# lars-uav/lars-image-processing

Hardware: AMD Instinct MI355X
Metric: Mpixels/sec NDVI+stats on 4096x4096 RGNir tiles; achieved HBM GB/s (higher is better)
Workload: dtype f32

## Files before the change

include/lars_hip.h:

```cpp
#ifndef LARS_HIP_H
#define LARS_HIP_H

#include <stddef.h>
#include <stdint.h>

#ifdef __cplusplus
extern "C" {
#endif

#define LARS_ABI_VERSION 1
#define LARS_HIST_BINS 50

typedef enum lars_status {
    LARS_OK = 0,
    LARS_ERR_INVALID = -1,
    LARS_ERR_NO_DEVICE = -2,
    LARS_ERR_HIP = -3,
    LARS_ERR_OOM = -4,
    LARS_ERR_RCCL = -5,
    LARS_ERR_UNSUPPORTED = -6
} lars_status;

#define LARS_U8  1
#define LARS_U16 2

#define LARS_NDVI  0
#define LARS_GNDVI 1
#define LARS_NDWI  2
#define LARS_MASK_NDVI  1u
#define LARS_MASK_GNDVI 2u
#define LARS_MASK_NDWI  4u
#define LARS_MASK_ALL   7u

#define LARS_F_STATS 1u
#define LARS_F_HIST  2u
#define LARS_F_SUMSQ 4u
#define LARS_F_RAW   8u

typedef struct lars_stats {
    double   sum;
    double   sumsq;
    uint64_t count;
    uint64_t above;
    uint64_t nans;
    double   min;
    double   max;
    double   threshold;
    uint32_t index_id;
    uint32_t reserved;
    uint64_t hist[LARS_HIST_BINS];
} lars_stats;

int         lars_abi_version(void);
const char *lars_last_error(void);
int         lars_device_count(int *count);
int         lars_set_device(int ordinal);
int         lars_get_device(int *ordinal);
int         lars_device_name(char *buf, size_t buflen);
int         lars_malloc(void **dptr, size_t bytes);
int         lars_free(void *dptr);
int         lars_memset(void *dptr, int value, size_t bytes, void *stream);
int         lars_memcpy_h2d(void *dst_dev, const void *src_host, size_t bytes);
int         lars_memcpy_d2h(void *dst_host, const void *src_dev, size_t bytes);
int         lars_memcpy_d2d(void *dst_dev, const void *src_dev, size_t bytes, void *stream);
int         lars_stream_create(void **stream);
int         lars_stream_destroy(void *stream);
int         lars_synchronize(void *stream);
int         lars_mem_info(size_t *free_bytes, size_t *total_bytes);
int         lars_shutdown(void);
int         lars_event_create(void **event);
int         lars_event_destroy(void *event);
int         lars_event_record(void *event, void *stream);
int         lars_event_elapsed_ms(void *start, void *stop, float *ms);
int         lars_stream_wait_event(void *stream, void *event);


int lars_d_channel_hist(const void *tiles, int64_t ntiles, int64_t npix, int channels,
                        int dtype, uint32_t *hist, void *stream);

int lars_d_wb_table(const uint32_t *hist, int64_t ntiles, int64_t npix, int dtype,
                    uint8_t *table, double *percentiles, int rgn_variant, void *stream);

size_t lars_wb_table_bytes(int dtype);

int lars_d_wb_prepare(const void *tiles, int64_t ntiles, int64_t npix, int channels, int dtype,
                      uint8_t *table, double *percentiles, int rgn_variant, void *stream);
int lars_u16_window_report(int64_t ntiles, uint32_t *flags, uint32_t *windows);

typedef struct lars_fused_args {
    const void    *tiles;
    int64_t        ntiles;
    int64_t        npix;
    int32_t        channels;
    int32_t        dtype;
    const uint8_t *wb_table;
    uint32_t       index_mask;
    uint32_t       flags;
    float         *out_index[3];
    uint8_t       *out_wb;
    uint8_t       *out_rgba[3];
    const uint8_t *cmap_lut[3];
    lars_stats    *stats;
    void          *stream;
} lars_fused_args;

int lars_d_fused(const lars_fused_args *args);
int lars_d_stats_begin(lars_stats *stats, int64_t ntiles, uint32_t index_mask, void *stream);
int lars_d_stats_end(lars_stats *stats, int64_t ntiles, uint32_t index_mask, int64_t npix, void *stream);

int lars_d_index_planes_f32(const float *red, const float *green, const float *nir,
                            int64_t n, int index_id, float *out, void *stream);

int lars_d_ndvi_f64(const void *img, int64_t npix, int channels, int dtype,
                    double *out, void *stream);

int lars_d_array_stats_f32(const float *x, int64_t n, float threshold, int want_hist,
                           lars_stats *out_dev, void *stream);
int lars_d_array_stats_f64(const double *x, int64_t n, double threshold, int want_hist,
                           lars_stats *out_dev, double *out_sumsqdev_dev, void *stream);

size_t lars_select_scratch_bytes(void);
int lars_d_median_pair_f32(const float *x, int64_t n, float *out_dev, void *scratch, void *stream);
int lars_d_median_pair_f64(const double *x, int64_t n, double *out_dev, void *scratch, void *stream);
int lars_d_median_pair_batch_f32(const float *x, int64_t n, int64_t items, int64_t stride, float *out_dev,
                                 void *scratch, void *stream);

int lars_d_quotient_select_hist(const void *tiles, int64_t ntiles, int64_t npix, int channels, int dtype,
                                const uint8_t *wb_table, uint32_t streams , int first,
                                const uint32_t bucket[4], uint64_t *hist, void *stream);
size_t lars_quotient_median_scratch_bytes(int64_t ntiles);
int lars_d_stats_medians(const lars_fused_args *a, float *out_pairs, void *scratch);
int lars_d_quotient_median_pairs(const void *tiles, int64_t ntiles, int64_t npix, int channels, int dtype,
                                 const uint8_t *wb_table, uint32_t streams ,
                                 float *out_pairs, void *scratch, void *stream);

size_t lars_joint_scratch_bytes(int64_t ntiles, int64_t npix, uint32_t index_mask);
int lars_d_stats_joint(const lars_fused_args *a, int white_balance, int rgn_variant, double *percentiles, uint32_t *hist,
                       float *out_pairs, void *scratch, size_t scratch_bytes);
int lars_joint_window_report(const void *scratch, int64_t ntiles, int64_t *windowed, int64_t *recounted);
int lars_joint_window_modes(const void *scratch, int64_t ntiles, int64_t counts[3]);

int lars_d_threshold_mask_f32(const float *x, int64_t n, float threshold, uint8_t *out_mask, void *stream);

int lars_d_colormap_f32(const float *x, int64_t n, const uint8_t *lut_rgba, uint8_t *out_rgba,
                        void *stream);
int lars_d_colormap_entry_f32(const float *x, int64_t n, uint8_t *out_entry, void *stream);

int lars_d_gray_c128(const uint8_t *img, int64_t npix, int channels, double *out_c128, void *stream);
size_t lars_phase_scratch_bytes(void);
int lars_d_phase_correlation(double *fixed_c128, double *moving_c128, int64_t h, int64_t w, int64_t *shift_dev,
                             void *scratch, void *stream);
int lars_d_shift_reflect_u8(const uint8_t *img, int64_t h, int64_t w, int channels, const int64_t *shift_dev,
                            uint8_t *out, void *stream);
int lars_d_diff_f32(const float *early, const float *late, int64_t n, float *out_diff, void *stream);
int lars_d_colormap_norm_f32(const float *x, int64_t n, float vmin, float vmax, const uint8_t *lut_rgba,
                             uint8_t *out_rgba, void *stream);

int lars_d_synth_u8(uint8_t *tiles, int64_t ntiles, int64_t first_tile, int64_t npix, int channels,
                    uint32_t seed, int profile, void *stream);

int lars_set_tuning(const char *key, int value);
int lars_get_tuning(const char *key, int *value);

#define LARS_BUILD_LAB_LAYOUT 1u
#define LARS_BUILD_IEEE_DIV 2u
#define LARS_BUILD_COUNT_MODE 4u
#define LARS_BUILD_STATS_GEOMETRY 8u
unsigned int lars_build_flags(void);

int lars_d_quot_selfcheck(uint32_t max_den, uint64_t *mismatches, uint32_t first_bad[2]);

int lars_stats_merge(const lars_stats *records, int64_t n, lars_stats *out);
int lars_d_stats_fold(const lars_stats *tile_records, int64_t ntiles, uint32_t index_mask, lars_stats *out, void *stream);


int lars_h_fix_white_balance(const void *img, int64_t h, int64_t w, int channels, int dtype,
                             int variant, uint8_t *out, double *percentiles );
int lars_h_fix_white_balance_f32(const float *img, int64_t h, int64_t w, int channels, uint8_t *out,
                                 double *percentiles );

int lars_h_calculate_index(const void *img, int64_t h, int64_t w, int channels, int dtype,
                           uint32_t index_mask, float *const out[3],
                           lars_stats *stats , int want_hist);

int lars_h_calculate_index_planes(const float *red, const float *green, const float *nir,
                                  int64_t n, int index_id, float *out);

int lars_h_ndvi_f64(const void *img, int64_t h, int64_t w, int channels, int dtype, double *out);

int lars_h_analyze_f32(const float *x, int64_t n, float threshold, int want_hist,
                       lars_stats *out, float median_pair[2]);
int lars_h_analyze_f64(const double *x, int64_t n, double threshold, int want_hist,
                       lars_stats *out, double median_pair[2], double *sumsqdev);

int lars_h_process_image(const void *img, int64_t h, int64_t w, int channels, int dtype,
                         int apply_wb, uint32_t index_mask, int want_hist,
                         uint8_t *out_wb, float *const out_index[3],
                         lars_stats *stats , float *medians ,
                         uint8_t *const out_rgba[3], const uint8_t *const cmap_lut[3]);

int lars_h_colormap_f32(const float *x, int64_t n, const uint8_t *lut_rgba, uint8_t *out_rgba);
int lars_h_threshold_mask_f32(const float *x, int64_t n, float threshold, uint8_t *out_mask);

int lars_h_resize_lanczos_u8(const uint8_t *img, int64_t h, int64_t w, int channels, int64_t new_h, int64_t new_w,
                             uint8_t *out);
int lars_h_thumbnail_u8(const uint8_t *img, int64_t h, int64_t w, int channels, int fx, int fy, const int reduce_box[4],
                        const float box[4], int64_t new_h, int64_t new_w, int vertical_first, uint8_t *out);

int lars_h_align_images(const uint8_t *fixed, const uint8_t *moving, int64_t h, int64_t w, int channels,
                        uint8_t *out_aligned, double shift[2]);
int lars_h_change_detection(const uint8_t *early, const uint8_t *late, int64_t h, int64_t w, int channels,
                            int wb_early, int wb_late, int align, int index_id,
                            float *out_early, float *out_late, float *out_diff,
                            uint8_t *out_rgba_diff, const uint8_t *lut_rgba, float vmin, float vmax,
                            uint8_t *out_aligned_late, double shift[2]);
int lars_h_colormap_norm_f32(const float *x, int64_t n, float vmin, float vmax, const uint8_t *lut_rgba,
                             uint8_t *out_rgba);

size_t lars_png_bound(int64_t h, int64_t w, int channels);
size_t lars_png_scratch_bytes(int64_t h, int64_t w, int channels);
int lars_d_encode_png_u8(const uint8_t *img, int64_t h, int64_t w, int channels, const uint8_t *palette_rgba, int palette_len,
                         uint8_t *out, size_t out_cap, int64_t *out_len_dev, void *scratch, void *stream);
int lars_h_encode_png_u8(const uint8_t *img, int64_t h, int64_t w, int channels, const uint8_t *palette_rgba, int palette_len,
                         uint8_t *out, size_t out_cap, int64_t *out_len);
int lars_h_process_image_png(const void *img, int64_t h, int64_t w, int channels, int dtype,
                             int apply_wb, uint32_t index_mask, int want_hist,
                             uint8_t *out_wb, float *const out_index[3],
                             lars_stats *stats , float *medians ,
                             const uint8_t *const cmap_lut[3], int png_mode,
                             uint8_t *const out_png[3], size_t png_cap, int64_t png_len[3]);

#define LARS_PNG_INFO_N 10
enum {
    LARS_PNG_INFO_WIDTH = 0,
    LARS_PNG_INFO_HEIGHT = 1,
    LARS_PNG_INFO_BIT_DEPTH = 2,
    LARS_PNG_INFO_COLOR_TYPE = 3,
    LARS_PNG_INFO_INTERLACE = 4,
    LARS_PNG_INFO_CHANNELS = 5,
    LARS_PNG_INFO_IDAT_BYTES = 6,
    LARS_PNG_INFO_IDAT_COUNT = 7,
    LARS_PNG_INFO_APNG = 8,
    LARS_PNG_INFO_SUPPORTED = 9
};
enum {
    LARS_PNGD_OK = 0,
    LARS_PNGD_CRC = 1,
    LARS_PNGD_ZLIB_HEADER = 2,
    LARS_PNGD_DEFLATE = 3,
    LARS_PNGD_FAR = 4,
    LARS_PNGD_SHORT = 5,
    LARS_PNGD_ADLER = 6,
    LARS_PNGD_FILTER = 7,
    LARS_PNGD_INTERNAL = 8
};
int lars_png_info(const uint8_t *file, int64_t len, int64_t info[LARS_PNG_INFO_N], int64_t *idat_table, int64_t idat_cap);
size_t lars_png_decode_scratch_bytes(int64_t h, int64_t w, int channels, int64_t idat_bytes, int64_t idat_count);
int lars_d_decode_png_u8(const uint8_t *file, const int64_t *idat_table, int64_t idat_count, int64_t idat_bytes, int64_t h,
                         int64_t w, int channels, uint8_t *out, int32_t *status_dev, void *scratch, void *stream);
int lars_h_decode_png_u8(const uint8_t *file, int64_t len, uint8_t *out, size_t out_cap);
int lars_h_thumbnail_png_u8(const uint8_t *file, int64_t len, int fx, int fy, const int reduce_box[4], const float box[4],
                            int64_t new_h, int64_t new_w, int vertical_first, uint8_t *out);

#define LARS_PNGX_PASS_N 10
enum {
    LARS_PNGX_PASS_X0 = 0,
    LARS_PNGX_PASS_Y0 = 1,
    LARS_PNGX_PASS_DX = 2,
    LARS_PNGX_PASS_DY = 3,
    LARS_PNGX_PASS_W = 4,
    LARS_PNGX_PASS_H = 5,
    LARS_PNGX_PASS_ROW_BYTES = 6,
    LARS_PNGX_PASS_OFFSET = 7,
    LARS_PNGX_PASS_BPP = 8,
    LARS_PNGX_PASS_INDEX = 9
};
int lars_png_out_format(int depth, int color_type, int *channels, int *itemsize);
int lars_png_layout(int64_t w, int64_t h, int depth, int color_type, int interlace, int64_t passes[7 * LARS_PNGX_PASS_N],
                    int64_t *npass, int64_t *need);
size_t lars_png_decode_ex_scratch_bytes(int64_t h, int64_t w, int depth, int color_type, int interlace, int64_t idat_bytes,
                                        int64_t idat_count);
int lars_d_decode_png_ex(const uint8_t *file, const int64_t *idat_table, int64_t idat_count, int64_t idat_bytes, int64_t h,
                         int64_t w, int depth, int color_type, int interlace, uint8_t *out, int32_t *status_dev, void *scratch,
                         void *stream);
int lars_h_decode_png_ex(const uint8_t *file, int64_t len, uint8_t *out, size_t out_cap);
int lars_h_thumbnail_png_ex(const uint8_t *file, int64_t len, int fx, int fy, const int reduce_box[4], const float box[4],
                            int64_t new_h, int64_t new_w, int vertical_first, uint8_t *out);

#define LARS_JPEG_INFO_N 16
#define LARS_JPEG_INFO_SAMPLING_STRIDE 2
enum {
    LARS_JPEG_INFO_WIDTH = 0,
    LARS_JPEG_INFO_HEIGHT = 1,
    LARS_JPEG_INFO_COMPONENTS = 2,
    LARS_JPEG_INFO_FRAME = 3,
    LARS_JPEG_INFO_PRECISION = 4,
    LARS_JPEG_INFO_H0 = 5,
    LARS_JPEG_INFO_V0 = 6,
    LARS_JPEG_INFO_RESTART_INTERVAL = 11,
    LARS_JPEG_INFO_ENTROPY_OFFSET = 12,
    LARS_JPEG_INFO_ENTROPY_BYTES = 13,
    LARS_JPEG_INFO_SUPPORTED = 14,
    LARS_JPEG_INFO_REASON = 15
};
enum {
    LARS_JPEG_REASON_NONE = 0,
    LARS_JPEG_REASON_PROGRESSIVE = 1,
    LARS_JPEG_REASON_FRAME = 2,
    LARS_JPEG_REASON_PRECISION = 3,
// ... 277 lines not shown
```

lars_image_processing_amd/_ffi.py:

```python
from __future__ import annotations

import contextlib
import ctypes as C
import os
import threading
from typing import NamedTuple

import numpy as np

_HERE = os.path.dirname(os.path.abspath(__file__))
LIB_PATH = os.environ.get("LARS_HIP_LIB", os.path.join(_HERE, "liblars_hip.so"))

HIST_BINS = 50
U8, U16 = 1, 2
NDVI, GNDVI, NDWI = 0, 1, 2
INDEX_IDS = {"NDVI": NDVI, "GNDVI": GNDVI, "NDWI": NDWI}
INDEX_NAMES = ("NDVI", "GNDVI", "NDWI")
F_STATS, F_HIST, F_SUMSQ, F_RAW = 1, 2, 4, 8
COMM_ID_BYTES = 128


class LarsError(RuntimeError):

    def __init__(self, code, message):
        super().__init__(f"liblars_hip error {code}: {message}")
        self.code = code


class Stats(C.Structure):
    _fields_ = [
        ("sum", C.c_double), ("sumsq", C.c_double),
        ("count", C.c_uint64), ("above", C.c_uint64), ("nans", C.c_uint64),
        ("min", C.c_double), ("max", C.c_double), ("threshold", C.c_double),
        ("index_id", C.c_uint32), ("reserved", C.c_uint32),
        ("hist", C.c_uint64 * HIST_BINS),
    ]


STATS_DTYPE = np.dtype([
    ("sum", "<f8"), ("sumsq", "<f8"), ("count", "<u8"), ("above", "<u8"), ("nans", "<u8"),
    ("min", "<f8"), ("max", "<f8"), ("threshold", "<f8"), ("index_id", "<u4"), ("reserved", "<u4"),
    ("hist", "<u8", (HIST_BINS,)),
])
assert STATS_DTYPE.itemsize == C.sizeof(Stats) == 472

REGION_DTYPE = np.dtype([("area", "<i8"), ("bbox", "<i4", (4,)), ("row_sum", "<u8"), ("col_sum", "<u8")])
assert REGION_DTYPE.itemsize == 40

RING_DTYPE = np.dtype([("label", "<i4"), ("key", "<i4"), ("start", "<i4"), ("count", "<i4"), ("area2", "<i8")])
assert RING_DTYPE.itemsize == 24


class Outlines(C.Structure):
    _fields_ = [
        ("rings", C.c_void_p), ("ring_capacity", C.c_int64), ("verts", C.c_void_p), ("vert_capacity", C.c_int64),
        ("n_rings", C.c_int64), ("n_vertices", C.c_int64), ("n_edges", C.c_int64),
    ]


class FusedArgs(C.Structure):
    _fields_ = [
        ("tiles", C.c_void_p), ("ntiles", C.c_int64), ("npix", C.c_int64),
        ("channels", C.c_int32), ("dtype", C.c_int32),
        ("wb_table", C.c_void_p), ("index_mask", C.c_uint32), ("flags", C.c_uint32),
        ("out_index", C.c_void_p * 3), ("out_wb", C.c_void_p),
        ("out_rgba", C.c_void_p * 3), ("cmap_lut", C.c_void_p * 3),
        ("stats", C.c_void_p), ("stream", C.c_void_p),
    ]


class PngInfo(NamedTuple):
    width: int
    height: int
    bit_depth: int
    color_type: int
    interlace: int
    channels: int
    idat_bytes: int
    idat_count: int
    apng: int
    supported: int

    @classmethod
    def array(cls):
        return (C.c_int64 * len(cls._fields))()


class JpegInfo(NamedTuple):
    width: int
    height: int
    components: int
    frame: int
    precision: int
    h0: int
    v0: int
    h1: int
    v1: int
    h2: int
    v2: int
    restart_interval: int
    entropy_offset: int
    entropy_bytes: int
    supported: int
    reason: int

    @classmethod
    def array(cls):
        return (C.c_int64 * len(cls._fields))()

    @property
    def sampling(self):
        return ((self.h0, self.v0), (self.h1, self.v1), (self.h2, self.v2))


class TiffInfo(NamedTuple):
    width: int
    height: int
    samples: int
    bits: int
    compression: int
    predictor: int
    planar: int
    big_endian: int
    photometric: int
    extra_samples: int
    tiled: int
    chunk_w: int
    chunk_h: int
    chunks: int
    supported: int
    reason: int

    @classmethod
    def array(cls):
        return (C.c_int64 * len(cls._fields))()


_P, _I, _I64, _U32, _SZ, _F, _D = C.c_void_p, C.c_int, C.c_int64, C.c_uint32, C.c_size_t, C.c_float, C.c_double
SIGNATURES = {
    "lars_abi_version": (_I, []),
    "lars_last_error": (C.c_char_p, []),
    "lars_device_count": (_I, [C.POINTER(_I)]),
    "lars_set_device": (_I, [_I]),
    "lars_get_device": (_I, [C.POINTER(_I)]),
    "lars_device_name": (_I, [C.c_char_p, _SZ]),
    "lars_malloc": (_I, [C.POINTER(_P), _SZ]),
    "lars_free": (_I, [_P]),
    "lars_memset": (_I, [_P, _I, _SZ, _P]),
    "lars_memcpy_h2d": (_I, [_P, _P, _SZ]),
    "lars_memcpy_d2h": (_I, [_P, _P, _SZ]),
    "lars_memcpy_d2d": (_I, [_P, _P, _SZ, _P]),
    "lars_stream_create": (_I, [C.POINTER(_P)]),
    "lars_stream_destroy": (_I, [_P]),
    "lars_synchronize": (_I, [_P]),
    "lars_shutdown": (_I, []),
    "lars_mem_info": (_I, [C.POINTER(_SZ), C.POINTER(_SZ)]),
    "lars_event_create": (_I, [C.POINTER(_P)]),
    "lars_event_destroy": (_I, [_P]),
    "lars_event_record": (_I, [_P, _P]),
    "lars_event_elapsed_ms": (_I, [_P, _P, C.POINTER(_F)]),
    "lars_stream_wait_event": (_I, [_P, _P]),
    "lars_d_channel_hist": (_I, [_P, _I64, _I64, _I, _I, _P, _P]),
    "lars_d_wb_table": (_I, [_P, _I64, _I64, _I, _P, _P, _I, _P]),
    "lars_wb_table_bytes": (_SZ, [_I]),
    "lars_d_wb_prepare": (_I, [_P, _I64, _I64, _I, _I, _P, _P, _I, _P]),
    "lars_u16_window_report": (_I, [_I64, _P, _P]),
    "lars_d_fused": (_I, [C.POINTER(FusedArgs)]),
    "lars_d_stats_begin": (_I, [_P, _I64, _U32, _P]),
    "lars_d_stats_end": (_I, [_P, _I64, _U32, _I64, _P]),
    "lars_d_index_planes_f32": (_I, [_P, _P, _P, _I64, _I, _P, _P]),
    "lars_d_ndvi_f64": (_I, [_P, _I64, _I, _I, _P, _P]),
    "lars_d_array_stats_f32": (_I, [_P, _I64, _F, _I, _P, _P]),
    "lars_d_array_stats_f64": (_I, [_P, _I64, _D, _I, _P, _P, _P]),
    "lars_select_scratch_bytes": (_SZ, []),
    "lars_d_median_pair_f32": (_I, [_P, _I64, _P, _P, _P]),
    "lars_d_median_pair_f64": (_I, [_P, _I64, _P, _P, _P]),
    "lars_d_median_pair_batch_f32": (_I, [_P, _I64, _I64, _I64, _P, _P, _P]),
    "lars_d_colormap_f32": (_I, [_P, _I64, _P, _P, _P]),
    "lars_d_colormap_entry_f32": (_I, [_P, _I64, _P, _P]),
    "lars_quotient_median_scratch_bytes": (_SZ, [_I64]),
    "lars_d_stats_medians": (_I, [C.POINTER(FusedArgs), _P, _P]),
    "lars_d_quotient_median_pairs": (_I, [_P, _I64, _I64, _I, _I, _P, _U32, _P, _P, _P]),
    "lars_joint_scratch_bytes": (_SZ, [_I64, _I64, _U32]),
    "lars_d_stats_joint": (_I, [C.POINTER(FusedArgs), _I, _I, _P, _P, _P, _P, _SZ]),
    "lars_joint_window_report": (_I, [_P, _I64, C.POINTER(_I64), C.POINTER(_I64)]),
    "lars_joint_window_modes": (_I, [_P, _I64, C.POINTER(_I64)]),
    "lars_h_tiff_lzw_decode": (_I, [_P, _I64, _P, _I64, C.POINTER(_I64)]),
    "lars_h_tiff_lzw_decode_chunks": (_I, [_P, _I64, _P, _P, _I64, _P, _I64, _P, _I]),
    "lars_d_quotient_select_hist": (_I, [_P, _I64, _I64, _I, _I, _P, _U32, _I, _P, _P, _P]),
    "lars_d_synth_u8": (_I, [_P, _I64, _I64, _I64, _I, _U32, _I, _P]),
    "lars_stats_merge": (_I, [_P, _I64, _P]),
    "lars_d_stats_fold": (_I, [_P, _I64, _U32, _P, _P]),
    "lars_build_flags": (C.c_uint, []),
    "lars_set_tuning": (_I, [C.c_char_p, _I]),
    "lars_get_tuning": (_I, [C.c_char_p, C.POINTER(_I)]),
    "lars_d_quot_selfcheck": (_I, [_U32, C.POINTER(C.c_uint64), C.POINTER(_U32 * 2)]),
    "lars_h_fix_white_balance": (_I, [_P, _I64, _I64, _I, _I, _I, _P, _P]),
    "lars_h_fix_white_balance_f32": (_I, [_P, _I64, _I64, _I, _P, _P]),
    "lars_h_calculate_index": (_I, [_P, _I64, _I64, _I, _I, _U32, C.POINTER(_P * 3), _P, _I]),
    "lars_h_calculate_index_planes": (_I, [_P, _P, _P, _I64, _I, _P]),
    "lars_h_ndvi_f64": (_I, [_P, _I64, _I64, _I, _I, _P]),
    "lars_h_analyze_f32": (_I, [_P, _I64, _F, _I, _P, _P]),
    "lars_h_analyze_f64": (_I, [_P, _I64, _D, _I, _P, _P, _P]),
    "lars_h_process_image": (_I, [_P, _I64, _I64, _I, _I, _I, _U32, _I, _P, C.POINTER(_P * 3), _P, _P,
                                  C.POINTER(_P * 3), C.POINTER(_P * 3)]),
    "lars_h_colormap_f32": (_I, [_P, _I64, _P, _P]),
    "lars_h_threshold_mask_f32": (_I, [_P, _I64, _F, _P]),
    "lars_d_threshold_mask_f32": (_I, [_P, _I64, _F, _P, _P]),
    "lars_h_colormap_norm_f32": (_I, [_P, _I64, _F, _F, _P, _P]),
    "lars_h_align_images": (_I, [_P, _P, _I64, _I64, _I, _P, _P]),
    "lars_h_change_detection": (_I, [_P, _P, _I64, _I64, _I, _I, _I, _I, _I, _P, _P, _P, _P, _P, _F, _F, _P, _P]),
    "lars_d_gray_c128": (_I, [_P, _I64, _I, _P, _P]),
    "lars_phase_scratch_bytes": (_SZ, []),
    "lars_d_phase_correlation": (_I, [_P, _P, _I64, _I64, _P, _P, _P]),
    "lars_d_shift_reflect_u8": (_I, [_P, _I64, _I64, _I, _P, _P, _P]),
    "lars_d_diff_f32": (_I, [_P, _P, _I64, _P, _P]),
    "lars_d_colormap_norm_f32": (_I, [_P, _I64, _F, _F, _P, _P, _P]),
    "lars_h_resize_lanczos_u8": (_I, [_P, _I64, _I64, _I, _I64, _I64, _P]),
    "lars_h_thumbnail_u8": (_I, [_P, _I64, _I64, _I, _I, _I, C.POINTER(_I), C.POINTER(_F), _I64, _I64, _I, _P]),
    "lars_png_bound": (_SZ, [_I64, _I64, _I]),
    "lars_png_scratch_bytes": (_SZ, [_I64, _I64, _I]),
    "lars_d_encode_png_u8": (_I, [_P, _I64, _I64, _I, _P, _I, _P, _SZ, _P, _P, _P]),
    "lars_h_encode_png_u8": (_I, [_P, _I64, _I64, _I, _P, _I, _P, _SZ, C.POINTER(_I64)]),
    "lars_h_process_image_png": (_I, [_P, _I64, _I64, _I, _I, _I, _U32, _I, _P, C.POINTER(_P * 3), _P, _P,
                                      C.POINTER(_P * 3), _I, C.POINTER(_P * 3), _SZ, _P]),
    "lars_png_info": (_I, [_P, _I64, _P, _P, _I64]),
    "lars_png_decode_scratch_bytes": (_SZ, [_I64, _I64, _I, _I64, _I64]),
    "lars_d_decode_png_u8": (_I, [_P, _P, _I64, _I64, _I64, _I64, _I, _P, _P, _P, _P]),
    "lars_h_decode_png_u8": (_I, [_P, _I64, _P, _SZ]),
    "lars_h_thumbnail_png_u8": (_I, [_P, _I64, _I, _I, C.POINTER(_I), C.POINTER(_F), _I64, _I64, _I, _P]),
    "lars_png_out_format": (_I, [_I, _I, C.POINTER(_I), C.POINTER(_I)]),
    "lars_png_layout": (_I, [_I64, _I64, _I, _I, _I, _P, C.POINTER(_I64), C.POINTER(_I64)]),
    "lars_png_decode_ex_scratch_bytes": (_SZ, [_I64, _I64, _I, _I, _I, _I64, _I64]),
    "lars_d_decode_png_ex": (_I, [_P, _P, _I64, _I64, _I64, _I64, _I, _I, _I, _P, _P, _P, _P]),
    "lars_h_decode_png_ex": (_I, [_P, _I64, _P, _SZ]),
    "lars_h_thumbnail_png_ex": (_I, [_P, _I64, _I, _I, C.POINTER(_I), C.POINTER(_F), _I64, _I64, _I, _P]),
    "lars_jpeg_info": (_I, [_P, _I64, _P]),
    "lars_jpeg_decode_scratch_bytes": (_SZ, [_P]),
    "lars_d_decode_jpeg_u8": (_I, [_P, _P, _P, _P, _P, _P, _P]),
    "lars_h_decode_jpeg_u8": (_I, [_P, _I64, _P, _SZ]),
    "lars_h_thumbnail_jpeg_u8": (_I, [_P, _I64, _I, _I, C.POINTER(_I), C.POINTER(_F), _I64, _I64, _I, _P]),
    "lars_jpeg_decode_scaled_scratch_bytes": (_SZ, [_P, _I]),
    "lars_d_decode_jpeg_scaled_u8": (_I, [_P, _P, _P, _I, _P, _P, _P, _P]),
    "lars_h_decode_jpeg_scaled_u8": (_I, [_P, _I64, _I, _P, _SZ]),
    "lars_h_thumbnail_jpeg_scaled_u8": (_I, [_P, _I64, _I, _I, _I, C.POINTER(_I), C.POINTER(_F), _I64, _I64, _I, _P]),
    "lars_tiff_info": (_I, [_P, _I64, _P, _P, _I64]),
    "lars_h_decode_tiff": (_I, [_P, _I64, _P, _SZ]),
    "lars_h_thumbnail_tiff_u8": (_I, [_P, _I64, _I, _I, C.POINTER(_I), C.POINTER(_F), _I64, _I64, _I, _P]),
    "lars_tiff_info_deflate": (_I, [_P, _I64, _P, _P, _I64]),
    "lars_h_decode_tiff_deflate": (_I, [_P, _I64, _P, _SZ]),
    "lars_h_thumbnail_tiff_deflate_u8": (_I, [_P, _I64, _I, _I, C.POINTER(_I), C.POINTER(_F), _I64, _I64, _I, _P]),
    "lars_tiff_bound": (_SZ, [_I64, _I64, _I, _I, _I64]),
    "lars_tiff_encode_scratch_bytes": (_SZ, [_I64, _I64, _I, _I, _I64]),
    "lars_d_encode_tiff": (_I, [_P, _I64, _I64, _I, _I, _I64, _I, _P, _SZ, _P, _P, _P, _P]),
    "lars_h_encode_tiff": (_I, [_P, _I64, _I64, _I, _I, _I64, _I, _P, _SZ, C.POINTER(_I64)]),
    "lars_tiff_f32_bound": (_SZ, [_I64, _I64, _I, _I64]),
    "lars_tiff_f32_encode_scratch_bytes": (_SZ, [_I64, _I64, _I, _I64]),
    "lars_d_encode_tiff_f32": (_I, [_P, _I64, _I64, _I, _I64, _I, _P, _SZ, _P, _P, _P, _P]),
    "lars_h_encode_tiff_f32": (_I, [_P, _I64, _I64, _I, _I64, _I, _P, _SZ, C.POINTER(_I64)]),
    "lars_h_process_image_tiff_f32": (_I, [_P, _I64, _I64, _I, _I, _I, _U32, _I, _P, C.POINTER(_P * 3), _P, _P,
                                           C.POINTER(_P * 3), C.POINTER(_P * 3), _I, _I64, C.POINTER(_P * 3), _SZ, _P]),
    "lars_tiff_deflate_bound": (_SZ, [_I64, _I64, _I, _I, _I64]),
    "lars_tiff_deflate_encode_scratch_bytes": (_SZ, [_I64, _I64, _I, _I, _I64]),
    "lars_d_encode_tiff_deflate": (_I, [_P, _I64, _I64, _I, _I, _I64, _I, _P, _SZ, _P, _P, _P, _P]),
    "lars_h_encode_tiff_deflate": (_I, [_P, _I64, _I64, _I, _I, _I64, _I, _P, _SZ, C.POINTER(_I64)]),
    "lars_tiff_float32_deflate_bound": (_SZ, [_I64, _I64, _I, _I64]),
    "lars_tiff_float32_deflate_encode_scratch_bytes": (_SZ, [_I64, _I64, _I, _I64]),
    "lars_d_encode_tiff_deflate_float32": (_I, [_P, _I64, _I64, _I, _I64, _I, _P, _SZ, _P, _P, _P, _P]),
    "lars_h_encode_tiff_deflate_float32": (_I, [_P, _I64, _I64, _I, _I64, _I, _P, _SZ, C.POINTER(_I64)]),
    "lars_h_process_image_tiff_float32": (_I, [_P, _I64, _I64, _I, _I, _I, _U32, _I, _P, C.POINTER(_P * 3), _P, _P,
                                                       C.POINTER(_P * 3), C.POINTER(_P * 3), _I, _I, _I64, C.POINTER(_P * 3), _SZ, _P]),
    "lars_d_valid_mask": (_I, [_P, _I64, _I, _I, _P, _I, _I, _I, _P, _P, _P]),
    "lars_d_masked_channel_hist": (_I, [_P, _I64, _I, _I, _P, _P, _P]),
    "lars_d_masked_fused": (_I, [C.POINTER(FusedArgs), _P, C.POINTER(_P * 3), _P]),
    "lars_h_valid_mask": (_I, [_P, _I64, _I64, _I, _I, _I, _I, _I, _P, C.POINTER(_I64)]),
    "lars_h_process_image_masked": (_I, [_P, _I64, _I64, _I, _I, _I, _U32, _I, _P, C.POINTER(_P * 3), _P, _P,
                                         C.POINTER(_P * 3), C.POINTER(_P * 3), _P, _I, _I, _I, C.POINTER(_I64),
                                         _I, _I, _I64, C.POINTER(_P * 3), _SZ, _P]),
    "lars_d_zone_count": (_I, [_P, _I, _P, _I64, _I64, _P, _P, _P]),
    "lars_d_zone_offsets": (_I, [_P, _I64, _P, _P, _P]),
    "lars_d_zone_scatter": (_I, [C.POINTER(_P * 3), _U32, _P, _I, _P, _I64, _I64, _P, _P, C.POINTER(_P * 3), _P]),
    "lars_d_zone_stats": (_I, [_P, _P, _P, _I64, _F, _I, _I64, _P, _P, _P]),
    "lars_h_zonal_stats_f32": (_I, [_P, _P, _I, _P, _I64, _I64, _I64, _F, _I, _P, _P, C.POINTER(_I64)]),
    "lars_h_process_image_zones": (_I, [_P, _I64, _I64, _I, _I, _I, _U32, _I, _P, C.POINTER(_P * 3), _P, _P,
                                        C.POINTER(_P * 3), C.POINTER(_P * 3), _P, _I, _I, _I, C.POINTER(_I64),
                                        _P, _I, _I64, _P, _P, C.POINTER(_I64)]),
    "lars_zone_rasterize_scratch_bytes": (_SZ, [_I64]),
    "lars_d_zone_rasterize": (_I, [_P, _I64, _P, _I64, _P, _I64, _I64, _I64, _P, _P, _P]),
    "lars_d_zone_labels_narrow": (_I, [_P, _I64, _I, _P, _P]),
    "lars_h_rasterize_zones": (_I, [_P, _I64, _P, _I64, _P, _I64, _I64, _I64, _I, _P]),
    "lars_h_zonal_stats_polygons_f32": (_I, [_P, _P, _I64, _P, _I64, _P, _I64, _P, _I64, _I64, _F, _I, _P, _P, _P, _I]),
    "lars_h_process_image_zones_polygons": (_I, [_P, _I64, _I64, _I, _I, _I, _U32, _I, _P, C.POINTER(_P * 3), _P, _P,
                                                 C.POINTER(_P * 3), C.POINTER(_P * 3), _P, _I, _I, _I, C.POINTER(_I64),
                                                 _P, _I64, _P, _I64, _P, _I64, _P, _P, _P, _I]),
    "lars_region_label_scratch_bytes": (_SZ, [_I64, _I64]),
    "lars_d_region_label": (_I, [_P, _I64, _I64, _I, _I64, _P, _P, _I64, _P, _P, _P]),
    "lars_d_region_mask_f32": (_I, [_P, _P, _P, _I64, _F, _I, _P, _P]),
    "lars_h_label_regions": (_I, [_P, _I64, _I64, _I, _I64, _I, _P, C.POINTER(_I), _P, _I64, C.POINTER(_I64)]),
    "lars_h_zonal_stats_regions_f32": (_I, [_P, _P, _I, _F, _I, _I64, _P, _I64, _I64, _F, _I, _I64, _P, _P, _P, C.POINTER(_I64), _P, _I,
                                            C.POINTER(_I)]),
    "lars_h_process_image_regions": (_I, [_P, _I64, _I64, _I, _I, _I, _U32, _I, _P, C.POINTER(_P * 3), _P, _P,
                                          C.POINTER(_P * 3), C.POINTER(_P * 3), _P, _I, _I, _I, C.POINTER(_I64),
                                          _P, _I, _I, _F, _I, _I64, _I64, _P, _P, _P, C.POINTER(_I64), _P, _I, C.POINTER(_I)]),
    "lars_region_outline_scratch_bytes": (_SZ, [_I64, _I64, _I64]),
    "lars_d_region_outline_count": (_I, [_P, _I64, _I64, _P, _P]),
    "lars_d_region_outline": (_I, [_P, _I64, _I64, _I, _I64, _I64, _P, _I64, _P, _I64, _P, _P, _P]),
    "lars_h_region_outlines": (_I, [_P, _I64, _I64, _I, _I64, _I, _P, C.POINTER(_I), _P, _I64, C.POINTER(_I64), C.POINTER(Outlines)]),
    "lars_h_zonal_stats_regions_outlines_f32": (_I, [_P, _P, _I, _F, _I, _I64, _P, _I64, _I64, _F, _I, _I64, _P, _P, _P, C.POINTER(_I64), _P, _I,
                                                     C.POINTER(_I), C.POINTER(Outlines)]),
    "lars_h_process_image_regions_outlines": (_I, [_P, _I64, _I64, _I, _I, _I, _U32, _I, _P, C.POINTER(_P * 3), _P, _P,
                                                   C.POINTER(_P * 3), C.POINTER(_P * 3), _P, _I, _I, _I, C.POINTER(_I64),
                                                   _P, _I, _I, _F, _I, _I64, _I64, _P, _P, _P, C.POINTER(_I64), _P, _I, C.POINTER(_I),
                                                   C.POINTER(Outlines)]),
    "lars_jpeg_bound": (_SZ, [_I64, _I64, _I, _I]),
    "lars_jpeg_header": (_I64, [_I64, _I64, _I, _I, _I, _P, _SZ]),
    "lars_jpeg_encode_scratch_bytes": (_SZ, [_I64, _I64, _I, _I]),
    "lars_d_encode_jpeg_u8": (_I, [_P, _I64, _I64, _I, _I, _I, _P, _SZ, _P, _P, _P]),
    "lars_h_encode_jpeg_u8": (_I, [_P, _I64, _I64, _I, _I, _I, _P, _SZ, C.POINTER(_I64)]),
    "lars_comm_available": (_I, []),
    "lars_comm_unique_id": (_I, [_P]),
# ... 158 lines not shown
```

lars_image_processing_amd/batch.py:

```python
from __future__ import annotations

import ctypes as C
import os

import numpy as np

from . import _ffi
from . import arena as _arena
from ._ffi import FusedArgs, INDEX_IDS, INDEX_NAMES, STATS_DTYPE, DeviceBuffer, DeviceSlice
from .arena import arena_placements

MAX_TILES_PER_LAUNCH = 65535


_STATS_ROUTE = os.environ.get("LARS_STATS_ROUTE", "auto")


def set_stats_route(route):
    global _STATS_ROUTE
    if route not in ("auto", "joint", "classic"):
        raise ValueError("route must be auto, joint or classic")
    _STATS_ROUTE = route


def get_stats_route():
    return _STATS_ROUTE


def index_mask(indices):
    mask = 0
    for t in indices:
        mask |= 1 << INDEX_IDS[t]
    return mask


def joint_serves(code, channels, ntiles, npix):
    return code == _ffi.U8 and channels in (3, 4) and (ntiles == 1 or npix % 4 == 0)


def plan_process(code, channels, ntiles, npix, indices, white_balance, hist, medians, sumsq, route,
                 outputs=False, wb_plane=False, reuse=False):
    if route not in ("auto", "joint", "classic"):
        raise ValueError(f"route must be auto, joint or classic, not {route!r}")
    if reuse and not outputs and route == "joint":
        raise ValueError("route='joint' derives the tables from its own counts: it cannot honour recompute_tables=False")
    one_read = route != "classic" and not reuse and joint_serves(code, channels, ntiles, npix) and bool(indices)
    if one_read and not outputs:
        return "measure" if route == "auto" and not medians and not sumsq else "one-read"
    if route == "joint" and not outputs:
        raise ValueError("route='joint' serves uint8 tiles with 3 or 4 channels (4-byte aligned) only")
    if one_read and not wb_plane and (medians or hist or select_streams(indices) in (1, 2)):
        return "one-read+planes"
    if medians and code == _ffi.U8 and channels == 3 and npix * 6 < (1 << 30) and (ntiles == 1 or npix % 4 == 0):
        return "select" if not outputs and index_mask(indices) in (1, 2, 4, 7) else "per-pixel+select"
    return "per-pixel+radix" if medians else "per-pixel"


def channels_of(indices, whole_image=False):
    if whole_image:
        return {0, 1, 2}
    need = set()
    for t in indices:
        need |= {2, 0} if t == "NDVI" else {2, 1}
    return need


def shard_range(ntiles, rank, world):
    base, rem = divmod(int(ntiles), int(world))
    start = rank * base + min(rank, rem)
    return start, start + base + (1 if rank < rem else 0)


class TileBatch:

    def __init__(self, ntiles, h, w, channels=3, dtype=np.uint8, first_tile=0):
        self.ntiles, self.h, self.w, self.channels = int(ntiles), int(h), int(w), int(channels)
        self.dtype = np.dtype(dtype)
        self.code = _ffi.dtype_code(self.dtype)
        if self.code is None:
            raise TypeError("tiles must be uint8 or uint16")
        if self.ntiles < 1 or self.ntiles > MAX_TILES_PER_LAUNCH:
            raise ValueError(f"1 <= ntiles <= {MAX_TILES_PER_LAUNCH} per batch")
        self.first_tile = int(first_tile)
        self.npix = self.h * self.w
        self.nvalues = 256 if self.code == _ffi.U8 else 65536
        self.table_bytes = int(_ffi.load().lars_wb_table_bytes(self.code))
        self.tile_bytes = self.npix * self.channels * self.dtype.itemsize
        self.tiles = DeviceBuffer(self.ntiles * self.tile_bytes)
        self.hist = None
        self.table = None
        self.percentiles = None
        self._table_channels = set()
        self._hist_channels = set()
        self._rgn_variant = 0
        self._joint_scratch = None
        self._joint_tiles = self.ntiles
        self._selq = None
        self.last_route = None

    @classmethod
    def from_host(cls, array, first_tile=0):
        arr = np.ascontiguousarray(array)
        if arr.ndim != 4 or arr.shape[3] < 3:
            raise ValueError("expected [ntiles, H, W, C>=3]")
        b = cls(arr.shape[0], arr.shape[1], arr.shape[2], arr.shape[3], arr.dtype, first_tile)
        b.tiles.upload(arr)
        return b

    @classmethod
    def synthetic(cls, ntiles, h, w, seed=1234, profile="uniform", first_tile=0, channels=3):
        b = cls(ntiles, h, w, channels, np.uint8, first_tile)
        _ffi.call("lars_d_synth_u8", C.c_void_p(b.tiles.ptr), b.ntiles, b.first_tile, b.npix, b.channels,
                  int(seed) & 0xFFFFFFFF, {"uniform": 0, "vegetation": 1}[profile], None)
        _ffi.call("lars_synchronize", None)
        return b

    def host_tiles(self, start=0, count=None):
        count = self.ntiles - start if count is None else count
        return self.tiles.download(self.dtype, (count, self.h, self.w, self.channels), start * self.tile_bytes)

    def compute_wb_tables(self, stream=None, rgn_variant=0):
        if self.table is None:
            self.table = DeviceBuffer(self.ntiles * self.table_bytes)
            self.percentiles = DeviceBuffer(self.ntiles * 3 * 2 * 8)
        if self.code == _ffi.U8:
            if self.hist is None:
                self.hist = DeviceBuffer(self.ntiles * 3 * 256 * 4)
            _ffi.call("lars_d_channel_hist", C.c_void_p(self.tiles.ptr), self.ntiles, self.npix, self.channels,
                      self.code, C.c_void_p(self.hist.ptr), stream)
            _ffi.call("lars_d_wb_table", C.c_void_p(self.hist.ptr), self.ntiles, self.npix, self.code,
                      C.c_void_p(self.table.ptr), C.c_void_p(self.percentiles.ptr), int(rgn_variant), stream)
        else:
            _ffi.call("lars_d_wb_prepare", C.c_void_p(self.tiles.ptr), self.ntiles, self.npix, self.channels,
                      self.code, C.c_void_p(self.table.ptr), C.c_void_p(self.percentiles.ptr), int(rgn_variant), stream)
        self._table_channels = {0, 1, 2}
        self._hist_channels = {0, 1, 2} if self.code == _ffi.U8 else set()
        self._rgn_variant = int(rgn_variant)
        return self

    def u16_window_report(self):
        if self.code != _ffi.U16:
            raise _ffi.LarsError(-1, "lars_u16_window_report: a uint8 batch's pre-pass does not take the value-window route")
        flags = np.zeros(self.ntiles, np.uint32)
        windows = np.zeros((self.ntiles, 3, 4), np.uint32)
        _ffi.call("lars_u16_window_report", self.ntiles, _ffi.ptr(flags), _ffi.ptr(windows))
        return flags, windows

    def _need_channels(self, partial):
        if self.table is None:
            raise RuntimeError("compute_wb_tables() first")
        if not partial and self._table_channels != {0, 1, 2}:
            missing = sorted({0, 1, 2} - self._table_channels)
            raise RuntimeError(f"white-balance tables of channel(s) {missing} are not valid: the last pass computed only the "
                               f"channels its indices read (compute_wb_tables() for all three, or partial=True)")

    def host_tables(self, partial=False):
        self._need_channels(partial)
        blob = self.table.download(np.uint8, (self.ntiles, self.table_bytes))
        return np.ascontiguousarray(blob[:, :3 * self.nvalues]).reshape(self.ntiles, 3, self.nvalues)

    def host_percentiles(self, partial=False):
        self._need_channels(partial)
        return self.percentiles.download(np.float64, (self.ntiles, 3, 2))

    def host_hist(self, partial=False):
        self._need_channels(partial)
        if self.hist is None or (not partial and self._hist_channels != {0, 1, 2}):
            missing = sorted({0, 1, 2} - self._hist_channels)
            raise RuntimeError(f"channel histograms of channel(s) {missing} are not valid: the last one-read pass was not asked for them "
                               f"(compute_wb_tables(), or run_joint(..., channel_hist=True); partial=True hands out what there is)")
        return self.hist.download(np.uint32, (self.ntiles, 3, 256))

    def make_outputs(self, indices=INDEX_NAMES, index=False, wb=False, rgba=False, ring=None, placement_trials=None, arena="auto",
                     pick="fastest"):
        outs = BatchOutputs(self, indices, index, wb, rgba, ring, allocate=False)
        nplanes = len(outs._index_ids) + len(outs._rgba_ids)
        plan = _arena.plan_arena(nplanes, outs.plane_bytes, outs.slots * self.npix * 4, arena, placement_trials, pick)
        if plan.kind != "search":
            if plan.kind == "packed":
                outs.adopt_arena(DeviceBuffer(nplanes * outs.plane_bytes))
            outs.arena_report = _arena.unsearched_report(plan)
            return outs

        def free_bytes():
            free_b, total_b = C.c_size_t(), C.c_size_t()
            _ffi.call("lars_mem_info", C.byref(free_b), C.byref(total_b))
            return free_b.value

        stats = self.new_stats()
        try:
            found = _arena.search(outs, plan, pick, alloc=DeviceBuffer, free_bytes=free_bytes,
                                  probe=lambda placement, warm_ms: self._probe_arena(outs, indices, stats, warm_ms),
                                  synchronize=lambda: _ffi.call("lars_synchronize", None))
        finally:
            stats.free()
        outs.placement_ms, outs.arena_report = _arena.report(found)
        return outs

    def _probe_arena(self, outs, indices, stats, warm_ms=_arena.ARENA_WARM_MS):
        count = min(outs.slots, self.ntiles)
        starts = list(range(0, self.ntiles, count))
        if len(starts) > 16:
            starts = [starts[int(round(i * (len(starts) - 1) / 15.0))] for i in range(16)]
        mask = index_mask(indices)
        wb_on = self.table is not None
        launches = [self.fused_args(indices, wb_on, stats, False, outs, None, st, min(count, self.ntiles - st), raw=True) for st in starts]
        while len(launches) < 4:
            launches = launches + launches
        ev = [C.c_void_p(), C.c_void_p()]
        for e in ev:
            _ffi.call("lars_event_create", C.byref(e))
        ms = C.c_float(0)

        def one_pass():
            _ffi.call("lars_event_record", ev[0], None)
            for a in launches:
                self.run_fused(a)
            _ffi.call("lars_event_record", ev[1], None)
            _ffi.call("lars_event_elapsed_ms", ev[0], ev[1], C.byref(ms))
            return float(ms.value)

        try:
            _ffi.call("lars_d_stats_begin", C.c_void_p(stats.ptr), self.ntiles, mask, None)
            warmed, passes = 0.0, 0
            while warmed < warm_ms and passes < 8:
                warmed += one_pass()
                passes += 1
            timed = one_pass()
            _ffi.call("lars_d_stats_end", C.c_void_p(stats.ptr), self.ntiles, mask, self.npix, None)
            _ffi.call("lars_synchronize", None)
        finally:
            for e in ev:
                _ffi.call("lars_event_destroy", e)
        return timed / len(launches)

    def fused_args(self, indices=INDEX_NAMES, white_balance=True, stats=None, hist=False, outputs=None,
                   stream=None, tile_start=0, tile_count=None, sumsq=False, raw=False):
        tile_count = self.ntiles - tile_start if tile_count is None else tile_count
        a = FusedArgs()
        a.tiles = self.tiles.ptr + tile_start * self.tile_bytes
        a.ntiles, a.npix, a.channels, a.dtype = tile_count, self.npix, self.channels, self.code
        if white_balance:
            if self.table is None:
                raise RuntimeError("compute_wb_tables() first")
            a.wb_table = self.table.ptr + tile_start * self.table_bytes
        a.index_mask = index_mask(indices)
        a.flags = ((_ffi.F_STATS if stats is not None else 0) | (_ffi.F_HIST if (stats is not None and hist) else 0) |
                   (_ffi.F_SUMSQ if (stats is not None and sumsq) else 0) | (_ffi.F_RAW if (stats is not None and raw) else 0))
        if stats is not None:
            a.stats = stats.ptr + tile_start * 3 * STATS_DTYPE.itemsize
        if outputs is not None:
            slot = tile_start % outputs.slots
            if slot + tile_count > outputs.slots:
                raise ValueError("tile range wraps the output ring")
            for k in range(3):
                if outputs.index[k] is not None:
                    a.out_index[k] = outputs.index[k].ptr + slot * self.npix * 4
                if outputs.rgba[k] is not None:
                    a.out_rgba[k] = outputs.rgba[k].ptr + slot * self.npix * 4
                    a.cmap_lut[k] = outputs.luts[k].ptr
            if outputs.wb is not None:
                a.out_wb = outputs.wb.ptr + slot * self.npix * self.channels
        a.stream = stream
        return a

    def new_stats(self):
        return DeviceBuffer(self.ntiles * 3 * STATS_DTYPE.itemsize)

    def fold_stats(self, stats, indices=INDEX_NAMES, out=None, stream=None):
        if out is None:
            out = DeviceBuffer(3 * STATS_DTYPE.itemsize)
            out.zero(stream)
        _ffi.call("lars_d_stats_fold", C.c_void_p(stats.ptr), self.ntiles, index_mask(indices), C.c_void_p(out.ptr), stream)
        return out

    def run_fused_chunks(self, indices, white_balance, stats, hist, outputs, stream=None, sumsq=False, launch_events=None):
        chunk = self.ntiles if outputs is None else outputs.slots
        if chunk >= self.ntiles:
            if launch_events:
                _ffi.call("lars_event_record", launch_events[0], stream)
            self.run_fused(self.fused_args(indices, white_balance, stats, hist, outputs, stream, sumsq=sumsq))
            if launch_events and len(launch_events) > 1:
                _ffi.call("lars_event_record", launch_events[1], stream)
            return 1
        mask = index_mask(indices)
        if stats is not None:
            _ffi.call("lars_d_stats_begin", C.c_void_p(stats.ptr), self.ntiles, mask, stream)
        launches = 0
        if launch_events:
            _ffi.call("lars_event_record", launch_events[0], stream)
        for start in range(0, self.ntiles, chunk):
            count = min(chunk, self.ntiles - start)
            self.run_fused(self.fused_args(indices, white_balance, stats, hist, outputs, stream, start, count, sumsq=sumsq,
                                           raw=stats is not None))
            launches += 1
            if launch_events and launches < len(launch_events):
                _ffi.call("lars_event_record", launch_events[launches], stream)
        if stats is not None:
            _ffi.call("lars_d_stats_end", C.c_void_p(stats.ptr), self.ntiles, mask, self.npix, stream)
        return launches

    def run_fused(self, args):
        _ffi.call("lars_d_fused", C.byref(args))

    def can_joint(self):
        return joint_serves(self.code, self.channels, self.ntiles, self.npix)

    def run_joint(self, indices, white_balance, stats, hist=False, sumsq=False, pairs=None, stream=None, rgn_variant=0,
                  tile_count=None, channel_hist=False):
        mask = index_mask(indices)
        need = int(_ffi.load().lars_joint_scratch_bytes(self.ntiles, self.npix, mask))
        if self._joint_scratch is None or self._joint_scratch.nbytes < need:
            if self._joint_scratch is not None:
                _ffi.call("lars_synchronize", stream)
                self._joint_scratch.free()
            self._joint_scratch = DeviceBuffer(need)
        if white_balance:
            if self.table is None:
                self.table = DeviceBuffer(self.ntiles * self.table_bytes)
                self.percentiles = DeviceBuffer(self.ntiles * 3 * 2 * 8)
                self.table.zero(stream)
                self.percentiles.zero(stream)
            if channel_hist and self.hist is None:
                self.hist = DeviceBuffer(self.ntiles * 3 * 256 * 4)
                self.hist.zero(stream)
                self._hist_channels = set()
            if tile_count is None or int(tile_count) == self.ntiles:
                keep = self._table_channels if int(rgn_variant) == self._rgn_variant else set()
                self._table_channels = keep | channels_of(indices)
                self._rgn_variant = int(rgn_variant)
                if channel_hist:
                    self._hist_channels = self._hist_channels | channels_of(indices)
            else:
                self._table_channels = set()
                self._hist_channels = set()
        a = FusedArgs()
        a.tiles = self.tiles.ptr
        a.ntiles, a.npix, a.channels, a.dtype = (self.ntiles if tile_count is None else int(tile_count)), self.npix, self.channels, self.code
        a.wb_table = self.table.ptr if white_balance else None
        a.index_mask = mask
        a.flags = _ffi.F_STATS | (_ffi.F_HIST if hist else 0) | (_ffi.F_SUMSQ if sumsq else 0)
        a.stats = stats.ptr
        a.stream = stream
        self._joint_tiles = int(a.ntiles)
        _ffi.call("lars_d_stats_joint", C.byref(a), 1 if white_balance else 0, int(rgn_variant),
                  C.c_void_p(self.percentiles.ptr) if white_balance else None,
                  C.c_void_p(self.hist.ptr) if white_balance and channel_hist else None,
                  C.c_void_p(pairs.ptr) if pairs is not None else None, C.c_void_p(self._joint_scratch.ptr), self._joint_scratch.nbytes)

    def joint_window_report(self):
        w, r = C.c_int64(0), C.c_int64(0)
        if self._joint_scratch is None:
            return 0, 0
        _ffi.call("lars_joint_window_report", C.c_void_p(self._joint_scratch.ptr), self._joint_tiles, C.byref(w), C.byref(r))
        return int(w.value), int(r.value)

    def joint_window_modes(self):
        if self._joint_scratch is None:
            return 0, 0, 0
        counts = (C.c_int64 * 3)()
        _ffi.call("lars_joint_window_modes", C.c_void_p(self._joint_scratch.ptr), self._joint_tiles, counts)
        return int(counts[0]), int(counts[1]), int(counts[2])

    def check_joint(self, stream=None):
        _ffi.call("lars_synchronize", stream)
        if self._joint_scratch is not None and int(self._joint_scratch.download(np.uint32, (1,))[0]):
            raise RuntimeError("lars_d_stats_joint: a workgroup's hand-over list overflowed (a chunk of more than 2^24 pixels?)")

    def pick_stats_route(self, indices, white_balance=True, sample=256, min_pixels=1 << 29):
        key = (tuple(sorted(INDEX_IDS[t] for t in indices)), bool(white_balance))
        cache = self.__dict__.setdefault("_route_cache", {})
        if key in cache:
            return cache[key]
        sample = min(int(sample), self.ntiles)
        if sample * self.npix < int(min_pixels) or self.channels != 3:
            cache[key] = "joint"
            return "joint"
        saved = (self.table, self.percentiles, self.hist, set(self._table_channels), self._rgn_variant, set(self._hist_channels))
        self.table = self.percentiles = self.hist = None
        self._table_channels = set()
        self._hist_channels = set()
        ev = [C.c_void_p() for _ in range(3)]
        for e in ev:
            _ffi.call("lars_event_create", C.byref(e))
        stats = self.new_stats()
        ms = {}
        try:
            for _ in range(2):
                _ffi.call("lars_event_record", ev[0], None)
                self.run_joint(indices, white_balance, stats, tile_count=sample)
                _ffi.call("lars_event_record", ev[1], None)
                if white_balance:
                    if self.hist is None:
                        self.hist = DeviceBuffer(self.ntiles * 3 * 256 * 4)
                    _ffi.call("lars_d_channel_hist", C.c_void_p(self.tiles.ptr), sample, self.npix, self.channels, self.code,
                              C.c_void_p(self.hist.ptr), None)
                    _ffi.call("lars_d_wb_table", C.c_void_p(self.hist.ptr), sample, self.npix, self.code, C.c_void_p(self.table.ptr),
                              C.c_void_p(self.percentiles.ptr), 0, None)
                self.run_fused(self.fused_args(indices, white_balance, stats, False, None, None, 0, sample))
                _ffi.call("lars_event_record", ev[2], None)
                t = C.c_float(0)
                _ffi.call("lars_event_elapsed_ms", ev[0], ev[1], C.byref(t)); ms["joint"] = t.value
                _ffi.call("lars_event_elapsed_ms", ev[1], ev[2], C.byref(t)); ms["classic"] = t.value
            self.check_joint()
        finally:
            _ffi.call("lars_synchronize", None)
            for e in ev:
                _ffi.call("lars_event_destroy", e)
            stats.free()
            for buf in (self.table, self.percentiles, self.hist):
                if buf is not None:
                    buf.free()
            self.table, self.percentiles, self.hist, self._table_channels, self._rgn_variant, self._hist_channels = saved
        cache[key] = "joint" if ms["joint"] <= ms["classic"] else "classic"
        self._route_ms = dict(ms)
        return cache[key]

    def process(self, indices=INDEX_NAMES, white_balance=True, hist=False, outputs=None, stream=None,
                recompute_tables=True, medians=False, sumsq=False, route=None, rgn_variant=None, channel_hist=False):
        route = _STATS_ROUTE if route is None else route
        variant = 0 if rgn_variant is None else int(rgn_variant)
        wb_plane = outputs is not None and outputs.wb is not None
        reuse = (white_balance and not recompute_tables and self.table is not None
                 and channels_of(indices, wb_plane) <= self._table_channels and (rgn_variant is None or variant == self._rgn_variant))

        def plan(r):
            return plan_process(self.code, self.channels, self.ntiles, self.npix, indices, white_balance, hist, medians, sumsq, r,
                                outputs is not None, wb_plane, reuse)

        taken = plan(route)
        if taken == "measure":
            taken = plan(self.pick_stats_route(indices, white_balance))
        self.last_route = taken
        if taken in ("one-read", "one-read+planes"):
            return self._run_one_read(indices, white_balance, hist, sumsq, medians, outputs, stream, variant, channel_hist)
        if white_balance and not reuse:
            self.compute_wb_tables(stream, rgn_variant=variant)
        stats = self.new_stats()
        stats.zero(stream)
        run = {"select": self._run_select, "per-pixel+select": self._run_fused_select, "per-pixel": self._run_fused,
               "per-pixel+radix": self._run_fused_radix}[taken]
        return run(indices, white_balance, stats, hist, sumsq, outputs, stream)

    def _records(self, stats):
        rec = stats.download(STATS_DTYPE, (self.ntiles, 3))
        stats.free()
        return rec

    def _run_one_read(self, indices, white_balance, hist, sumsq, medians, outputs, stream, variant, channel_hist):
        stats = self.new_stats()
        stats.zero(stream)
        pairs = DeviceBuffer(self.ntiles * 4 * 4) if medians else None
        self.run_joint(indices, white_balance, stats, hist, sumsq, pairs, stream, rgn_variant=variant, channel_hist=channel_hist)
        if outputs is not None:
            self.run_fused_chunks(indices, white_balance, None, False, outputs, stream)
        self.check_joint(stream)
        rec = self._records(stats)
        if not medians:
            return rec
        med = self._medians_from_pairs(pairs.download(np.float32, (self.ntiles, 2, 2)), indices)
        pairs.free()
        return rec, med

    def _run_select(self, indices, white_balance, stats, hist, sumsq, outputs, stream):
        args = self.fused_args(indices, white_balance, stats, hist, None, stream, sumsq=sumsq)
        med = self._per_tile_select(indices, stream, lambda pairs, scratch: _ffi.call("lars_d_stats_medians", C.byref(args), pairs, scratch))
        return self._records(stats), med

    def _run_fused_select(self, indices, white_balance, stats, hist, sumsq, outputs, stream):
        self.run_fused_chunks(indices, white_balance, stats, hist, outputs, stream, sumsq)
        med = self.tile_medians(indices, white_balance, stream)
        return self._records(stats), med

    def _run_fused(self, indices, white_balance, stats, hist, sumsq, outputs, stream):
        self.run_fused_chunks(indices, white_balance, stats, hist, outputs, stream, sumsq)
        _ffi.call("lars_synchronize", stream)
        return self._records(stats)

    def _run_fused_radix(self, indices, white_balance, stats, hist, sumsq, outputs, stream):
        own_outputs = None
        if outputs is None or any(outputs.index[INDEX_IDS[t]] is None for t in indices):
            own_outputs = outputs = self.make_outputs(indices=indices, index=True, ring=min(self.ntiles, 16), arena="plain")
        pairs = DeviceBuffer(self.ntiles * 3 * 2 * 4)
        pairs.zero(stream)
        sel = DeviceBuffer(outputs.slots * int(_ffi.load().lars_select_scratch_bytes()))
        for start in range(0, self.ntiles, outputs.slots):
            count = min(outputs.slots, self.ntiles - start)
            self.run_fused(self.fused_args(indices, white_balance, stats, hist, outputs, stream, start, count, sumsq=sumsq))
            for t in indices:
                k = INDEX_IDS[t]
                _ffi.call("lars_d_median_pair_batch_f32", C.c_void_p(outputs.index[k].ptr), self.npix, count, self.npix,
                          C.c_void_p(pairs.ptr + (k * self.ntiles + start) * 8), C.c_void_p(sel.ptr), stream)
        _ffi.call("lars_synchronize", stream)
        rec = self._records(stats)
        med = pair_medians(pairs.download(np.float32, (3, self.ntiles, 2)), indices, per_index=True)
        pairs.free()
        sel.free()
        if own_outputs is not None:
            own_outputs.free()
        return rec, med

    def free(self):
        for b in (self.tiles, self.hist, self.table, self.percentiles, self._joint_scratch, self._selq):
            if b is not None:
                b.free()

    def tile_medians(self, indices=INDEX_NAMES, white_balance=True, stream=None):
        if white_balance and (self.table is None or not channels_of(indices) <= self._table_channels):
            raise RuntimeError("compute_wb_tables() first")
        return self._per_tile_select(indices, stream, lambda pairs, scratch: _ffi.call(
            "lars_d_quotient_median_pairs", C.c_void_p(self.tiles.ptr), self.ntiles, self.npix, self.channels, self.code,
            C.c_void_p(self.table.ptr) if white_balance else None, select_streams(indices), pairs, scratch, stream))

    def _per_tile_select(self, indices, stream, launch):
        pairs = DeviceBuffer(self.ntiles * 4 * 4)
        scratch = DeviceBuffer(int(_ffi.load().lars_quotient_median_scratch_bytes(self.ntiles)))
        launch(C.c_void_p(pairs.ptr), C.c_void_p(scratch.ptr))
        _ffi.call("lars_synchronize", stream)
        med = self._medians_from_pairs(pairs.download(np.float32, (self.ntiles, 2, 2)), indices)
        pairs.free()
        scratch.free()
        return med

    def _medians_from_pairs(self, pairs, indices):
        med = pair_medians(pairs, indices)
        if any(np.isnan(med[:, INDEX_IDS[t]]).any() for t in indices):
            raise RuntimeError("exact median select did not settle (values outside the uint8 quotient domain?)")
        return med

    def select_histogram(self, first, buckets, white_balance=True, stream=None, streams=3):
        if self.code != _ffi.U8 or self.channels != 3:
            raise TypeError("exact batch medians need uint8 tiles with 3 channels")
        if white_balance and self.table is None:
            raise RuntimeError("compute_wb_tables() first")
        if self._selq is None:
            self._selq = DeviceBuffer(2 * 2 * SELECT_BINS * 8)
        self._selq.zero(stream)
        b = np.ascontiguousarray(np.asarray(buckets, dtype=np.int64) & 0xFFFFFFFF, dtype=np.uint32).reshape(4)
        _ffi.call("lars_d_quotient_select_hist", C.c_void_p(self.tiles.ptr), self.ntiles, self.npix, self.channels, self.code,
                  C.c_void_p(self.table.ptr) if white_balance else None, int(streams), int(first), _ffi.ptr(b),
                  C.c_void_p(self._selq.ptr), stream)
        _ffi.call("lars_synchronize", stream)
        return self._selq.download(np.uint64, (2, 2, SELECT_BINS))

    def global_medians(self, indices=INDEX_NAMES, white_balance=True, comm=None, recompute_tables=False):
        if white_balance and (recompute_tables or self.table is None or not channels_of(indices) <= self._table_channels):
            self.compute_wb_tables()
        n_local = self.ntiles * self.npix
        streams = select_streams(indices)
        values = select_order_statistics(lambda first, buckets: self.select_histogram(first, buckets, white_balance, None, streams),
                                         n_local, comm, streams)
        return medians_from_pairs(values, indices)


class BatchOutputs:

    def __init__(self, batch, indices, index, wb, rgba, ring=None, allocate=True):
        from .api import colormap_lut, _colormap_for
        self.slots = batch.ntiles if not ring else min(int(ring), batch.ntiles)
        self.index, self.rgba, self.luts = [None] * 3, [None] * 3, [None] * 3
        self.batch = batch
        self.plane_bytes = (self.slots * batch.npix * 4 + 255) & ~255
        self._index_ids = sorted(INDEX_IDS[t] for t in indices) if index else []
        self._rgba_ids = sorted(INDEX_IDS[t] for t in indices) if rgba else []
        self.arena = None
        self.arena2 = None
        self.arena_report = None
        if allocate and (self._index_ids or self._rgba_ids):
            self.adopt_arena(DeviceBuffer((len(self._index_ids) + len(self._rgba_ids)) * self.plane_bytes))
        for t in indices:
            k = INDEX_IDS[t]
            if rgba:
                self.luts[k] = DeviceBuffer(1024)
                self.luts[k].upload(colormap_lut(_colormap_for(t)))
        self.wb = DeviceBuffer(self.slots * batch.npix * batch.channels) if wb else None

    def adopt(self, buffers, placement):
        placement = tuple((int(i), int(o)) for i, o in placement)
        assert len(placement) == len(self._index_ids) + len(self._rgba_ids)
        used = list(dict.fromkeys(i for i, _ in placement))
        assert len(used) <= 2
        for i in used:
            inside = sorted(o for a, o in placement if a == i)
            assert all(o % 256 == 0 and o + self.plane_bytes <= buffers[i].nbytes for o in inside)
            assert all(b - a >= self.plane_bytes for a, b in zip(inside, inside[1:])), "planes overlap"
        self.arena = buffers[used[0]] if used else None
        self.arena2 = buffers[used[1]] if len(used) > 1 else None
        self.plane_offsets = tuple(o for _, o in placement)
        slices = [DeviceSlice(buffers[i], o, self.plane_bytes) for i, o in placement]
        for j, k in enumerate(self._index_ids):
            self.index[k] = slices[j]
        for j, k in enumerate(self._rgba_ids):
            self.rgba[k] = slices[len(self._index_ids) + j]

    def adopt_arena(self, arena, offsets=None):
        if offsets is None:
            offsets = _arena.packed(len(self._index_ids) + len(self._rgba_ids), self.plane_bytes)
        self.adopt([arena], [(0, o) for o in offsets])

    def adopt_two_arenas(self, arena, offsets, arena2, offsets2):
        self.adopt([arena, arena2], [(0, o) for o in offsets] + [(1, o) for o in offsets2])

    def forget_planes(self):
        self.index, self.rgba, self.arena, self.arena2 = [None] * 3, [None] * 3, None, None

    def host_index(self, index_type, slot=0, count=1):
        k = INDEX_IDS[index_type]
        b = self.batch
        return self.index[k].download(np.float32, (count, b.h, b.w), slot * b.npix * 4)

    def host_rgba(self, index_type, slot=0, count=1):
        k = INDEX_IDS[index_type]
        b = self.batch
        return self.rgba[k].download(np.uint8, (count, b.h, b.w, 4), slot * b.npix * 4)

    def host_wb(self, slot=0, count=1):
        b = self.batch
        return self.wb.download(np.uint8, (count, b.h, b.w, b.channels), slot * b.npix * b.channels)

    def free(self):
        for b in self.index + self.rgba + self.luts + [self.wb, self.arena, self.arena2]:
            if b is not None:
                b.free()
        self.forget_planes()


def merge_records(records):
    rec = np.ascontiguousarray(records, dtype=STATS_DTYPE).reshape(-1)
    out = np.zeros(1, dtype=STATS_DTYPE)
    _ffi.call("lars_stats_merge", _ffi.ptr(rec), rec.size, _ffi.ptr(out))
    return out[0]


def summarize(record):
    count = int(record["count"])
    mean = float(record["sum"]) / count
    sumsq = float(record["sumsq"])
    have_sq = sumsq != 0.0 or (float(record["min"]) == 0.0 and float(record["max"]) == 0.0)
    var = max(sumsq / count - mean * mean, 0.0)
    return {
        "count": count,
        "mean": mean,
        "std": var ** 0.5 if have_sq else None,
        "min": float(record["min"]),
        "max": float(record["max"]),
        "coverage": int(record["above"]) / count * 100.0,
        "hist": np.array(record["hist"], dtype=np.int64),
    }


def local_fold(tile_records, indices=INDEX_NAMES):
    out = np.zeros(3, dtype=STATS_DTYPE)
    for t in indices:
        k = INDEX_IDS[t]
        out[k] = merge_records(tile_records[:, k])
    return out
# ... 166 lines not shown
```

lars_image_processing_amd/csrc/common.h:

```cpp
#pragma once
#include <hip/hip_runtime.h>
#include <stdint.h>
#include <stdio.h>
#include <string>

#include "host_common.h"

namespace lars {


#define LARS_HIP_TRY(expr)                                                          \
    do {                                                                            \
        hipError_t _e = (expr);                                                     \
        if (_e != hipSuccess)                                                       \
            return ::lars::fail(_e == hipErrorOutOfMemory ? LARS_ERR_OOM : LARS_ERR_HIP, \
                                "%s failed: %s (%s:%d)", #expr, hipGetErrorString(_e), \
                                __FILE__, __LINE__);                                \
    } while (0)

struct ThreadCtx {
    int device = -1;
    hipStream_t stream = nullptr;
    void *ws = nullptr;
    size_t ws_bytes = 0;
    void *scratch = nullptr;
    size_t scratch_bytes = 0;
    void *outline = nullptr;
    size_t outline_bytes = 0;
    int64_t u16_win_tiles = 0;
};

int ensure_ctx(ThreadCtx **out);
int ws_reserve(ThreadCtx *c, size_t bytes);
int scratch_reserve(ThreadCtx *c, size_t bytes);
int outline_reserve(ThreadCtx *c, size_t bytes);

struct Carver {
    char *base;
    size_t off = 0;
    explicit Carver(void *b) : base(static_cast<char *>(b)) {}
    template <typename T>
    T *take(size_t count)
    {
        off = (off + 255) & ~(size_t)255;
        T *p = base ? reinterpret_cast<T *>(base + off) : nullptr;
        off += count * sizeof(T);
        return p;
    }
    size_t bytes() const { return (off + 255) & ~(size_t)255; }
};

template <typename Plan>
int ws_plan(ThreadCtx *c, Plan &&plan)
{
    Carver size(nullptr);
    plan(size);
    LARS_TRY(ws_reserve(c, size.bytes() + 256));
    Carver cv(c->ws);
    plan(cv);
    return LARS_OK;
}
inline hipStream_t pick_stream(ThreadCtx *c, void *stream) {
    return stream ? reinterpret_cast<hipStream_t>(stream) : c->stream;
}

#define LARS_FX_SCALE 4294967296.0
#define LARS_FX_INV (1.0 / 4294967296.0)

struct StatsAccView {
    unsigned long long sum_fx;
    unsigned long long sumsq_fx;
    unsigned long long count;
    unsigned long long above;
    unsigned long long nans;
    unsigned long long min_key;
    unsigned long long max_key;
    double threshold;
    unsigned int index_id;
    unsigned int reserved;
    unsigned long long hist[LARS_HIST_BINS];
};
static_assert(sizeof(StatsAccView) == sizeof(lars_stats), "accumulator view must alias lars_stats");

__host__ __device__ inline unsigned int f32_key(float x) {
    unsigned int b = __builtin_bit_cast(unsigned int, x);
    return (b & 0x80000000u) ? ~b : (b | 0x80000000u);
}
__host__ __device__ inline float key_f32(unsigned int k) {
    unsigned int b = (k & 0x80000000u) ? (k & 0x7FFFFFFFu) : ~k;
    return __builtin_bit_cast(float, b);
}
__host__ __device__ inline unsigned long long f64_key(double x) {
    unsigned long long b = __builtin_bit_cast(unsigned long long, x);
    return (b >> 63) ? ~b : (b | 0x8000000000000000ull);
}
__host__ __device__ inline double key_f64(unsigned long long k) {
    unsigned long long b = (k >> 63) ? (k & 0x7FFFFFFFFFFFFFFFull) : ~k;
    return __builtin_bit_cast(double, b);
}

__host__ __device__ inline double hist_edge_f64(int i) {
    return i >= LARS_HIST_BINS ? 1.0 : (double)i * (2.0 / 50.0) + (-1.0);
}

#define LARS_U16_THR_OFFSET 196608
#define LARS_U16_PAR_OFFSET (196608 + 3 * 260 * 4)
#define LARS_U16_BLOB_BYTES (196608 + 4096)

int launch_check(const char *what);
void align_release();

struct Tuning {
    int fused_impl = 0;
    int hist_impl = 2;
    int nt_stores = 0;
    int blocks_per_tile = 0;
    int load_policy = 0;
    int selq_window = 1;
    int selq_list_wgs = 0;
    int last_fused_kernel = 0;
    int u16_hist_impl = 5;
    int out_stride_planes = 0;
    int joint_depth = 6;
    int joint_win_depth = 15;
    int jpeg_subseq_bits = 512;
    int jpeg_last_rounds = 0;
    int tiff_strip_bytes = 65536;
    int deflate_matching = 0;
    int joint_window = 1;
    int zone_split_pixels = 131072;
};
Tuning &tuning();
inline bool stream_loads_nt(bool kernel_default_nt)
{
    const int k = tuning().load_policy;
    return k == 0 ? kernel_default_nt : k == 2;
}

struct FusedParams;
#ifndef LARS_V2_STATS_THREADS
#define LARS_V2_STATS_THREADS 1024
#endif
#ifndef LARS_V2_STATS_WAVES
#define LARS_V2_STATS_WAVES 8
#endif
int fused_v2_threads(bool any_out);
void fused_v2_launch(unsigned mask, bool wb, int stats, bool nt, dim3 grid, hipStream_t s, const FusedParams &P);
void chan_hist_v2_launch(const uint8_t *tiles, long long npix, unsigned int *hist, dim3 grid, hipStream_t s, int channels = 3);
int selq_pass_launch(const uint8_t *tiles, const uint8_t *wb_table, long long ntiles, long long npix, int first,
                     const unsigned int bucket[4], unsigned long long *hist, hipStream_t s, unsigned streams);
size_t selq_tile_scratch_bytes(long long ntiles);
int selq_tile_medians_launch(const uint8_t *tiles, const uint8_t *wb_table, long long ntiles, long long npix, float *out_pairs,
                             void *scratch, hipStream_t s, bool first_pass_done, unsigned streams, bool windowed = false);
int selq_tile_prepare(void *scratch, long long ntiles, long long npix, hipStream_t s, unsigned int streams);
unsigned int *selq_tile_hist32(void *scratch, long long ntiles);
void fused_v2_sel_launch(unsigned mask, bool wb, int stats, dim3 grid, hipStream_t s, const FusedParams &P);
int blocks_per_tile(long long work_items, long long ntiles, int threads = 256, long long target_total = 8192);
void stats_init_launch(lars_stats *stats, long long nrec, unsigned int mask, hipStream_t s);
void stats_finalize_launch(lars_stats *stats, long long nrec, unsigned int mask, long long npix, hipStream_t s);
int quot_check_launch(unsigned int max_den, unsigned long long *mismatches_dev, unsigned int *first_bad_dev, hipStream_t s);

}
```

lars_image_processing_amd/csrc/device_common.h:

```cpp
#pragma once
#include "common.h"
#include "stream_load.h"

namespace lars {

struct FusedParams {
    const void *tiles;
    long long npix;
    int channels;
    const uint8_t *wb_table;
    float *out_index[3];
    uint8_t *out_wb;
    uint8_t *out_rgba[3];
    const uint8_t *cmap_lut[3];
    lars_stats *stats;
    unsigned int mask;
    unsigned int flags;
    unsigned int *sel_hist;
    const unsigned int *sel_win;
    unsigned int *sel_win_hist;
    unsigned int *sel_below;
#ifdef LARS_LAB_LAYOUT
    long long out_tile_stride;
#endif
};

struct Acc {
    float mn, mx;
    double sum, sumsq;
    unsigned int above;
};
__device__ inline void acc_init(Acc &a) { a.mn = __builtin_inff(); a.mx = -__builtin_inff(); a.sum = 0; a.sumsq = 0; a.above = 0; }

__device__ inline float norm_diff(float a, float b)
{
    const float s = a + b;
    const float d = a - b;
#ifdef LARS_IEEE_DIV
    return d / (s == 0.0f ? 1.0f : s);
#else
    const float den = fmaxf(s, 1.0f);
    const float r = __builtin_amdgcn_rcpf(den);
    const float q0 = d * r;
    const float e = __builtin_fmaf(-q0, den, d);
    return __builtin_fmaf(e, r, q0);
#endif
}

#define LARS_HIST_CELLS 65
template <typename T>
struct HistCell {
    T edge;
    long long base;
};
template <>
struct HistCell<float> {
    float edge;
    int base;
};
template <typename T>
__device__ inline void hist_cells_init(HistCell<T> *cells, int tid)
{
    if (tid < LARS_HIST_CELLS) {
        const T lo = (T)tid / (T)32 - (T)1, hi = (T)(tid + 1) / (T)32 - (T)1;
        int below = 0;
        T inside = (T)__builtin_inf();
        for (int i = 0; i < LARS_HIST_BINS; ++i) {
            const T e = (T)hist_edge_f64(i);
            if (e < lo) ++below;
            else if (e < hi) inside = e;
        }
        cells[tid].edge = inside;
        cells[tid].base = below - 1;
    }
}
template <typename T>
__device__ inline int hist_bin_cell(T x, const HistCell<T> *cells)
{
    const int c = (int)__builtin_fma(x, (T)32, (T)32);
    const HistCell<T> e = cells[c];
    return (int)e.base + (x >= e.edge ? 1 : 0);
}
__device__ inline int hist_bin_f32(float x, const HistCell<float> *cells)
{
    const int c = (int)__builtin_fmaf(x, 32.0f, 32.0f);
    const HistCell<float> e = cells[c];
    return e.base + (x >= e.edge ? 1 : 0);
}

__device__ inline unsigned int cmap_index(float x)
{
    const float s = (x + 1.0f) * 128.0f;
    int i = (int)s;
    i = i < 0 ? 0 : (i > 255 ? 255 : i);
    return (unsigned)i;
}


__device__ inline unsigned int wb_level(int v, double p_lo, double p_hi, int rgn_variant)
{
    double x = (double)v;
    if (rgn_variant) x = fmin(fmax(x, p_lo), p_hi);
    double y = (x - p_lo) / (p_hi - p_lo) * 255.0;
    if (y != y) return 0u;
    y = y < 0.0 ? 0.0 : (y > 255.0 ? 255.0 : y);
    return rgn_variant ? (unsigned int)(int)y : (unsigned int)(int)(float)y;
}

__device__ inline void u16_fill_blob(uint8_t *blob, int c, double p_lo, double p_hi, int rgn_variant,
                                     unsigned int *s_thr, int tid)
{
    for (int k = tid; k < 260; k += 256) s_thr[k] = 65536u;
    __syncthreads();
    uint8_t *out = blob + (long long)c * 65536;
    unsigned int prev = tid == 0 ? 0u : wb_level(tid * 256 - 1, p_lo, p_hi, rgn_variant);
    for (int j = 0; j < 256; ++j) {
        const int v = tid * 256 + j;
        const unsigned int o = wb_level(v, p_lo, p_hi, rgn_variant);
        out[v] = (uint8_t)o;
        for (unsigned int k = prev + 1; k <= o; ++k) s_thr[k] = (unsigned)v;
        prev = o > prev ? o : prev;
    }
    __syncthreads();
    unsigned int *thr = reinterpret_cast<unsigned int *>(blob + LARS_U16_THR_OFFSET) + c * 260;
    for (int k = tid; k < 260; k += 256) thr[k] = k == 0 ? 0u : (k >= 256 ? 65536u : s_thr[k]);
    if (tid == 0) {
        double *par = reinterpret_cast<double *>(blob + LARS_U16_PAR_OFFSET) + c * 2;
        const double span = p_hi - p_lo;
        par[0] = p_lo;
        par[1] = span > 0.0 ? 255.0 / span : 1e300;
    }
}

}
```

lars_image_processing_amd/csrc/fused.hip:

```cpp
#include <string.h>

#include "common.h"
#include "device_common.h"
#include "fused_device.h"
#include "wg_device.h"

namespace lars {

__global__ __launch_bounds__(256) void k_chan_hist_u8c3(const uint8_t *__restrict__ tiles,
                                                        long long npix, unsigned int *__restrict__ hist)
{
    __shared__ unsigned int s_h[4][3 * 256];
    const int tid = threadIdx.x;
    const int wave = tid >> 6;
    for (int i = tid; i < 4 * 768; i += 256) (&s_h[0][0])[i] = 0;
    __syncthreads();

    const long long tile = blockIdx.y;
    const uint8_t *base = tiles + tile * npix * 3;
    const long long nquads = npix >> 2;
    unsigned int *h = s_h[wave];
    for (long long q = (long long)blockIdx.x * 256 + tid; q < nquads; q += (long long)gridDim.x * 256) {
        const unsigned int *p = reinterpret_cast<const unsigned int *>(base + q * 12);
        unsigned int w0 = p[0], w1 = p[1], w2 = p[2];
        atomicAdd(&h[0 * 256 + (w0 & 0xFF)], 1u);
        atomicAdd(&h[1 * 256 + ((w0 >> 8) & 0xFF)], 1u);
        atomicAdd(&h[2 * 256 + ((w0 >> 16) & 0xFF)], 1u);
        atomicAdd(&h[0 * 256 + (w0 >> 24)], 1u);
        atomicAdd(&h[1 * 256 + (w1 & 0xFF)], 1u);
        atomicAdd(&h[2 * 256 + ((w1 >> 8) & 0xFF)], 1u);
        atomicAdd(&h[0 * 256 + ((w1 >> 16) & 0xFF)], 1u);
        atomicAdd(&h[1 * 256 + (w1 >> 24)], 1u);
        atomicAdd(&h[2 * 256 + (w2 & 0xFF)], 1u);
        atomicAdd(&h[0 * 256 + ((w2 >> 8) & 0xFF)], 1u);
        atomicAdd(&h[1 * 256 + ((w2 >> 16) & 0xFF)], 1u);
        atomicAdd(&h[2 * 256 + (w2 >> 24)], 1u);
    }
    if (blockIdx.x == 0 && tid < (int)(npix & 3)) {
        const uint8_t *p = base + (nquads * 4 + tid) * 3;
        atomicAdd(&h[p[0]], 1u);
        atomicAdd(&h[256 + p[1]], 1u);
        atomicAdd(&h[512 + p[2]], 1u);
    }
    __syncthreads();
    unsigned int *gh = hist + tile * 768;
    for (int i = tid; i < 768; i += 256) {
        unsigned int v = s_h[0][i] + s_h[1][i] + s_h[2][i] + s_h[3][i];
        if (v) atomicAdd(&gh[i], v);
    }
}

template <typename PIX, int NVAL>
__global__ __launch_bounds__(256) void k_chan_hist_generic(const PIX *__restrict__ tiles, long long npix,
                                                           int channels, unsigned int *__restrict__ hist)
{
    const long long tile = blockIdx.y;
    const PIX *base = tiles + tile * npix * channels;
    unsigned int *gh = hist + tile * 3 * (long long)NVAL;
    if (NVAL == 256) {
        __shared__ unsigned int s_h[3 * 256];
        for (int i = threadIdx.x; i < 768; i += 256) s_h[i] = 0;
        __syncthreads();
        for (long long i = (long long)blockIdx.x * 256 + threadIdx.x; i < npix; i += (long long)gridDim.x * 256) {
            const PIX *p = base + i * channels;
            atomicAdd(&s_h[(unsigned)p[0]], 1u);
            atomicAdd(&s_h[256 + (unsigned)p[1]], 1u);
            atomicAdd(&s_h[512 + (unsigned)p[2]], 1u);
        }
        __syncthreads();
        for (int i = threadIdx.x; i < 768; i += 256)
            if (s_h[i]) atomicAdd(&gh[i], s_h[i]);
    } else {
        for (long long i = (long long)blockIdx.x * 256 + threadIdx.x; i < npix; i += (long long)gridDim.x * 256) {
            const PIX *p = base + i * channels;
            atomicAdd(&gh[(unsigned)p[0]], 1u);
            atomicAdd(&gh[NVAL + (unsigned)p[1]], 1u);
            atomicAdd(&gh[2 * NVAL + (unsigned)p[2]], 1u);
        }
    }
}

template <int NVAL>
__global__ __launch_bounds__(256) void k_wb_table(const unsigned int *__restrict__ hist, long long npix,
                                                  uint8_t *__restrict__ table, double *__restrict__ pcts,
                                                  int rgn_variant)
{
    constexpr int PER = NVAL / 256;
    __shared__ unsigned long long s_scan[4];
    __shared__ double s_val[4];
    __shared__ double s_p[2];
    __shared__ unsigned int s_thr[NVAL == 256 ? 4 : 260];

    const int tid = threadIdx.x;
    const long long slot = (long long)blockIdx.y * 3 + blockIdx.x;
    const unsigned int *h = hist + slot * NVAL;

    unsigned long long local = 0;
    for (int j = 0; j < PER; ++j) local += h[tid * PER + j];
    const unsigned long long before = wg_exscan<256>(local, s_scan);

    const double nm1 = (double)(npix - 1);
    double tq[2];
    long long rank[4];
    for (int k = 0; k < 2; ++k) {
        const double q = (k == 0 ? 2.0 : 98.0) / 100.0;
        const double vi = nm1 * q;
        const double fl = floor(vi);
        long long lo = (long long)fl;
        long long hi = lo + 1;
        if (hi > npix - 1) hi = npix - 1;
        rank[2 * k] = lo;
        rank[2 * k + 1] = hi;
        tq[k] = vi - fl;
    }
    unsigned long long cum = before;
    for (int j = 0; j < PER; ++j) {
        const unsigned long long c = h[tid * PER + j];
        if (c) {
            for (int r = 0; r < 4; ++r)
                if ((unsigned long long)rank[r] >= cum && (unsigned long long)rank[r] < cum + c)
                    s_val[r] = (double)(tid * PER + j);
        }
        cum += c;
    }
    __syncthreads();
    if (tid < 2) {
        const double a = s_val[2 * tid], b = s_val[2 * tid + 1], t = tq[tid];
        const double d = b - a;
        double r = a + d * t;
        if (t >= 0.5) r = b - d * (1.0 - t);
        s_p[tid] = r;
        if (pcts) pcts[slot * 2 + tid] = r;
    }
    __syncthreads();
    const double p_lo = s_p[0], p_hi = s_p[1];
    if (NVAL == 256) {
        uint8_t *out = table + slot * 256;
        out[tid] = (uint8_t)wb_level(tid, p_lo, p_hi, rgn_variant);
    } else {
        u16_fill_blob(table + (long long)blockIdx.y * LARS_U16_BLOB_BYTES, (int)blockIdx.x, p_lo, p_hi, rgn_variant, s_thr, tid);
    }
}

__global__ void k_stats_init(lars_stats *stats, long long nrec, unsigned int mask)
{
    const long long i = (long long)blockIdx.x * blockDim.x + threadIdx.x;
    if (i >= nrec) return;
    const int k = (int)(i % 3);
    if (!((mask >> k) & 1u)) return;
    StatsAccView *a = reinterpret_cast<StatsAccView *>(stats + i);
    a->sum_fx = 0; a->sumsq_fx = 0; a->count = 0; a->above = 0; a->nans = 0;
    a->min_key = ~0ull; a->max_key = 0ull;
    a->threshold = (k == LARS_NDWI) ? 0.0 : (double)0.2f;
    a->index_id = (unsigned)k; a->reserved = 0;
    for (int b = 0; b < LARS_HIST_BINS; ++b) a->hist[b] = 0;
}

__global__ void k_stats_finalize(lars_stats *stats, long long nrec, unsigned int mask, long long npix)
{
    const long long i = (long long)blockIdx.x * blockDim.x + threadIdx.x;
    if (i >= nrec) return;
    const int k = (int)(i % 3);
    if (!((mask >> k) & 1u)) return;
    StatsAccView *a = reinterpret_cast<StatsAccView *>(stats + i);
    const long long s = (long long)a->sum_fx, s2 = (long long)a->sumsq_fx;
    const unsigned long long mnk = a->min_key, mxk = a->max_key;
    lars_stats *o = stats + i;
    o->sum = (double)s * LARS_FX_INV;
    o->sumsq = (double)s2 * LARS_FX_INV;
    o->count = (uint64_t)npix;
    o->min = key_f64(mnk);
    o->max = key_f64(mxk);
}

__global__ __launch_bounds__(256) void k_stats_fold(const lars_stats *__restrict__ rec, long long ntiles, unsigned int mask,
                                                    lars_stats *__restrict__ out)
{
    const int k = blockIdx.x;
    if (!((mask >> k) & 1u)) return;
    __shared__ double s_sum[256], s_sq[256];
    __shared__ double s_mn[4], s_mx[4];
    __shared__ unsigned long long s_cnt[4][3];
    const int tid = threadIdx.x;
    double sum = 0.0, sq = 0.0;
    double mn = __builtin_inf(), mx = -__builtin_inf();
    unsigned long long cnt = 0, above = 0, nans = 0;
    __shared__ unsigned long long s_hist[LARS_HIST_BINS];
    if (tid < LARS_HIST_BINS) s_hist[tid] = 0ull;
    __syncthreads();
    for (long long t = tid; t < ntiles; t += 256) {
        const unsigned long long *h = reinterpret_cast<const unsigned long long *>(rec[t * 3 + k].hist);
        unsigned long long v[LARS_HIST_BINS];
#pragma unroll
        for (int b = 0; b < LARS_HIST_BINS; ++b) v[b] = h[b];
#pragma unroll
        for (int b = 0; b < LARS_HIST_BINS; ++b)
            if (v[b]) atomicAdd(&s_hist[b], v[b]);
    }
    for (long long base = 0; base < ntiles; base += 256) {
        const long long t = base + tid;
        if (t < ntiles) {
            const lars_stats *r = rec + t * 3 + k;
            s_sum[tid] = r->sum; s_sq[tid] = r->sumsq;
            cnt += r->count; above += r->above; nans += r->nans;
            mn = fmin(mn, r->min); mx = fmax(mx, r->max);
        }
        __syncthreads();
        const int n = (int)(ntiles - base < 256 ? ntiles - base : 256);
        if (tid == 0) {
            int i = 0;
            if (base == 0) { sum = s_sum[0]; sq = s_sq[0]; i = 1; }
            for (; i < n && (i & 7); ++i) { sum += s_sum[i]; sq += s_sq[i]; }
            for (; i + 8 <= n; i += 8) {
                double a[8], b[8];
#pragma unroll
                for (int j = 0; j < 8; ++j) { a[j] = s_sum[i + j]; b[j] = s_sq[i + j]; }
#pragma unroll
                for (int j = 0; j < 8; ++j) { sum += a[j]; sq += b[j]; }
            }
            for (; i < n; ++i) { sum += s_sum[i]; sq += s_sq[i]; }
        }
        __syncthreads();
    }
    for (int off = 32; off >= 1; off >>= 1) {
        cnt += __shfl_xor(cnt, off); above += __shfl_xor(above, off); nans += __shfl_xor(nans, off);
        mn = fmin(mn, __shfl_xor(mn, off)); mx = fmax(mx, __shfl_xor(mx, off));
    }
    if ((tid & 63) == 0) {
        const int w = tid >> 6;
        s_cnt[w][0] = cnt; s_cnt[w][1] = above; s_cnt[w][2] = nans; s_mn[w] = mn; s_mx[w] = mx;
    }
    __syncthreads();
    lars_stats *o = out + k;
    if (tid == 0) {
        o->sum = sum; o->sumsq = sq;
        o->count = s_cnt[0][0] + s_cnt[1][0] + s_cnt[2][0] + s_cnt[3][0];
        o->above = s_cnt[0][1] + s_cnt[1][1] + s_cnt[2][1] + s_cnt[3][1];
        o->nans = s_cnt[0][2] + s_cnt[1][2] + s_cnt[2][2] + s_cnt[3][2];
        o->min = fmin(fmin(s_mn[0], s_mn[1]), fmin(s_mn[2], s_mn[3]));
        o->max = fmax(fmax(s_mx[0], s_mx[1]), fmax(s_mx[2], s_mx[3]));
        o->threshold = rec[k].threshold; o->index_id = rec[k].index_id; o->reserved = rec[k].reserved;
    }
    if (tid < LARS_HIST_BINS) o->hist[tid] = s_hist[tid];
}

__device__ inline void acc_flush(Acc a, StatsAccView *rec, double (*s_red)[4], int tid)
{
    for (int off = 32; off >= 1; off >>= 1) {
        a.mn = fminf(a.mn, __shfl_xor(a.mn, off));
        a.mx = fmaxf(a.mx, __shfl_xor(a.mx, off));
        a.sum += __shfl_xor(a.sum, off);
        a.sumsq += __shfl_xor(a.sumsq, off);
        a.above += __shfl_xor(a.above, off);
    }
    const int wave = tid >> 6, lane = tid & 63;
    __syncthreads();
    if (lane == 0) {
        s_red[0][wave] = a.sum;
        s_red[1][wave] = a.sumsq;
        s_red[2][wave] = (double)a.above;
        s_red[3][wave] = __builtin_bit_cast(double, ((unsigned long long)f32_key(a.mx) << 32) | f32_key(a.mn));
    }
    __syncthreads();
    if (tid == 0) {
        double sum = 0, sumsq = 0, above = 0;
        unsigned int mnk = 0xFFFFFFFFu, mxk = 0;
        for (int w = 0; w < 4; ++w) {
            sum += s_red[0][w];
            sumsq += s_red[1][w];
            above += s_red[2][w];
            const unsigned long long kk = __builtin_bit_cast(unsigned long long, s_red[3][w]);
            const unsigned int kmn = (unsigned int)kk, kmx = (unsigned int)(kk >> 32);
            mnk = kmn < mnk ? kmn : mnk;
            mxk = kmx > mxk ? kmx : mxk;
        }
        atomicAdd(&rec->sum_fx, (unsigned long long)__double2ll_rn(sum * LARS_FX_SCALE));
        atomicAdd(&rec->sumsq_fx, (unsigned long long)__double2ll_rn(sumsq * LARS_FX_SCALE));
        atomicAdd(&rec->above, (unsigned long long)above);
        atomicMin(&rec->min_key, f64_key((double)key_f32(mnk)));
        atomicMax(&rec->max_key, f64_key((double)key_f32(mxk)));
    }
}


template <typename PIX, unsigned MASK, bool WB, int STATS, int CH = 3, int POLICY = LOAD_PLAIN>
__global__ __launch_bounds__(256)
__attribute__((amdgpu_waves_per_eu(1, (sizeof(PIX) == 1 && CH == 3 && MASK != 0u && STATS <= 1) ? 3 : 8))) void k_fused_u8c3(FusedParams P)
{
    constexpr bool U16 = sizeof(PIX) == 2;
    static_assert(CH == 3 || (CH == 4 && !U16), "4-channel fast path: uint8 tiles");
    __shared__ uint8_t s_lut[U16 ? 16 : 3 * 256];
    __shared__ unsigned int s_thr[U16 ? 3 * 260 : 4];
    __shared__ double s_par[U16 ? 6 : 1];
    constexpr int HIST_COPIES = 16;
    __shared__ unsigned int s_hist_all[HIST_COPIES * 3 * LARS_HIST_BINS];
    __shared__ HistCell<float> s_edges[LARS_HIST_CELLS];
    __shared__ double s_red[4][4];

    const int tid = threadIdx.x;
    unsigned int *const s_hist = s_hist_all + (tid & (HIST_COPIES - 1));
    const unsigned int bx = blockIdx.x, gx = gridDim.x;
    const long long tile = blockIdx.y;
    const long long npix = P.npix;
    const PIX *base = static_cast<const PIX *>(P.tiles) + tile * npix * CH;

    if (WB) {
        if (U16) {
            const uint8_t *blob = P.wb_table + tile * LARS_U16_BLOB_BYTES;
            const unsigned int *thr = reinterpret_cast<const unsigned int *>(blob + LARS_U16_THR_OFFSET);
            const double *par = reinterpret_cast<const double *>(blob + LARS_U16_PAR_OFFSET);
            for (int i = tid; i < 3 * 260; i += 256) s_thr[i] = thr[i];
            if (tid < 6) s_par[tid] = par[tid];
        } else {
            const uint8_t *t = P.wb_table + tile * 768;
            for (int i = tid; i < 768; i += 256) s_lut[i] = t[i];
        }
    }
    if (STATS >= 2) {
        for (int i = tid; i < HIST_COPIES * 3 * LARS_HIST_BINS; i += 256) s_hist_all[i] = 0;
        hist_cells_init<float>(s_edges, tid);
    }
    if (WB || STATS >= 2) __syncthreads();

    auto wb_map = [&](unsigned int v, int c) -> unsigned int {
        if (!U16) return s_lut[c * 256 + v];
        const double y = ((double)v - s_par[2 * c]) * s_par[2 * c + 1];
        int g = (int)y;
        g = g < 0 ? 0 : (g > 255 ? 255 : g);
        const unsigned int *t = s_thr + c * 260;
        g += (v >= t[g + 1] ? 1 : 0) - (v < t[g] ? 1 : 0);
        return (unsigned int)g;
    };

    Acc acc[3];
    acc_init(acc[0]); acc_init(acc[1]); acc_init(acc[2]);

#ifdef LARS_LAB_LAYOUT
    const long long ots = P.out_tile_stride;
#else
    const long long ots = npix;
#endif
    float *const oi0 = P.out_index[0] ? P.out_index[0] + tile * ots : nullptr;
    float *const oi1 = P.out_index[1] ? P.out_index[1] + tile * ots : nullptr;
    float *const oi2 = P.out_index[2] ? P.out_index[2] + tile * ots : nullptr;
    uint8_t *const owb = P.out_wb ? P.out_wb + tile * npix * CH : nullptr;
    uint8_t *const oc0 = P.out_rgba[0] ? P.out_rgba[0] + tile * npix * 4 : nullptr;
    uint8_t *const oc1 = P.out_rgba[1] ? P.out_rgba[1] + tile * npix * 4 : nullptr;
    uint8_t *const oc2 = P.out_rgba[2] ? P.out_rgba[2] + tile * npix * 4 : nullptr;
    const unsigned int *lut0 = reinterpret_cast<const unsigned int *>(P.cmap_lut[0]);
    const unsigned int *lut1 = reinterpret_cast<const unsigned int *>(P.cmap_lut[1]);
    const unsigned int *lut2 = reinterpret_cast<const unsigned int *>(P.cmap_lut[2]);

    const long long nquads = npix >> 2;
    const bool nt_st = (P.flags & 0x20000000u) != 0;
    __amdgpu_buffer_rsrc_t rsrc16;
    if (U16) rsrc16 = __builtin_amdgcn_make_buffer_rsrc(const_cast<PIX *>(base), 0, (int)(nquads * 24), 0x00020000);
    constexpr int NW = U16 ? 6 : 3;

    auto load_quad = [&](long long q, unsigned int (&w)[NW]) {
        if (U16) {
            const unsigned int off = (unsigned int)q * 24u;
            const fu32x4 a4 = stream_load_b128<POLICY>(rsrc16, off, 0);
            const fu32x2 a2 = stream_load_b64<POLICY>(rsrc16, off + 16u, 0);
            w[0] = a4.x; w[1] = a4.y; w[2] = a4.z; w[NW - 3] = a4.w; w[NW - 2] = a2.x; w[NW - 1] = a2.y;
        } else if (CH == 4) {
            const sl_u32x3 a = rgba_quad_to_rgb(
                stream_load_ptr<POLICY>(reinterpret_cast<const sl_u32x4 *>(reinterpret_cast<const uint8_t *>(base) + q * 16)));
            w[0] = a.x; w[1] = a.y; w[2] = a.z;
        } else {
            const unsigned int *p = reinterpret_cast<const unsigned int *>(reinterpret_cast<const uint8_t *>(base) + q * 12);
            w[0] = stream_load_ptr<POLICY>(p); w[1] = stream_load_ptr<POLICY>(p + 1); w[2] = stream_load_ptr<POLICY>(p + 2);
        }
    };
    auto do_quad = [&](long long q, const unsigned int (&w)[NW]) {
        unsigned int b[12];
        if (U16) {
#pragma unroll
            for (int i = 0; i < 6; ++i) { b[2 * i] = w[i % NW] & 0xFFFFu; b[2 * i + 1] = w[i % NW] >> 16; }
        } else {
            const unsigned int w0 = w[0], w1 = w[1], w2 = w[2];
            const unsigned int t[12] = {w0 & 0xFF, (w0 >> 8) & 0xFF, (w0 >> 16) & 0xFF, w0 >> 24,
                                        w1 & 0xFF, (w1 >> 8) & 0xFF, (w1 >> 16) & 0xFF, w1 >> 24,
                                        w2 & 0xFF, (w2 >> 8) & 0xFF, (w2 >> 16) & 0xFF, w2 >> 24};
#pragma unroll
            for (int i = 0; i < 12; ++i) b[i] = t[i];
        }
        if (WB) {
            const bool need_r = (MASK & 1u) || owb, need_g = (MASK & 6u) || owb;
#pragma unroll
            for (int i = 0; i < 12; ++i)
                if (i % 3 == 2 || (i % 3 == 0 && need_r) || (i % 3 == 1 && need_g)) b[i] = wb_map(b[i], i % 3);
            if (owb && CH == 4) {
                *reinterpret_cast<uint4 *>(owb + q * 16) = make_uint4(b[0] | (b[1] << 8) | (b[2] << 16), b[3] | (b[4] << 8) | (b[5] << 16),
                                                                      b[6] | (b[7] << 8) | (b[8] << 16), b[9] | (b[10] << 8) | (b[11] << 16));
            } else if (owb) {
                unsigned int *o = reinterpret_cast<unsigned int *>(owb + q * 12);
                o[0] = b[0] | (b[1] << 8) | (b[2] << 16) | (b[3] << 24);
                o[1] = b[4] | (b[5] << 8) | (b[6] << 16) | (b[7] << 24);
                o[2] = b[8] | (b[9] << 8) | (b[10] << 16) | (b[11] << 24);
            }
        }
        float v0[4], v1[4], v2[4];
#pragma unroll
        for (int px = 0; px < 4; ++px) {
            v0[px] = v1[px] = v2[px] = 0.0f;
            pixel_math<MASK, STATS, false, !U16, HIST_COPIES>((float)b[3 * px], (float)b[3 * px + 1], (float)b[3 * px + 2], 0u,
                                                            v0[px], v1[px], v2[px], acc, s_hist, s_edges);
        }
        if ((MASK & 1u) && oi0) store_plane4(oi0 + q * 4, v0, nt_st);
        if ((MASK & 2u) && oi1) store_plane4(oi1 + q * 4, v1, nt_st);
        if ((MASK & 4u) && oi2) store_plane4(oi2 + q * 4, v2, nt_st);
        if ((MASK & 1u) && oc0)
            *reinterpret_cast<uint4 *>(oc0 + q * 16) = make_uint4(lut0[cmap_index(v0[0])], lut0[cmap_index(v0[1])],
                                                                  lut0[cmap_index(v0[2])], lut0[cmap_index(v0[3])]);
        if ((MASK & 2u) && oc1)
            *reinterpret_cast<uint4 *>(oc1 + q * 16) = make_uint4(lut1[cmap_index(v1[0])], lut1[cmap_index(v1[1])],
                                                                  lut1[cmap_index(v1[2])], lut1[cmap_index(v1[3])]);
        if ((MASK & 4u) && oc2)
            *reinterpret_cast<uint4 *>(oc2 + q * 16) = make_uint4(lut2[cmap_index(v2[0])], lut2[cmap_index(v2[1])],
                                                                  lut2[cmap_index(v2[2])], lut2[cmap_index(v2[3])]);
    };

    constexpr int RUN = (!U16 && CH == 3 && MASK == 7u && STATS == 1) ? 16 : (U16 && MASK == 1u && STATS <= 1) ? 8 : 4;
    const long long nsteps = (nquads + 64 * RUN - 1) / (64 * RUN);
    const long long wstride = (long long)gx * 4;
    const unsigned int lane = (unsigned int)tid & 63u;
    for (long long st = (long long)bx * 4 + (tid >> 6); st < nsteps; st += wstride) {
        const long long q0 = st * (64 * RUN) + lane;
        unsigned int w[RUN][NW];
        if (st * (64 * RUN) + 64 * RUN <= nquads) {
#pragma unroll
            for (int j = 0; j < RUN; ++j) load_quad(q0 + 64 * j, w[j]);
            __builtin_amdgcn_sched_barrier(0);
#pragma unroll
            for (int j = 0; j < RUN; ++j) {
                do_quad(q0 + 64 * j, w[j]);
                __builtin_amdgcn_sched_barrier(0);
            }
        } else {
            for (int j = 0; j < RUN; ++j) {
                const long long q = q0 + 64 * j;
                if (q < nquads) { load_quad(q, w[0]); do_quad(q, w[0]); }
            }
        }
    }
    if (bx == 0 && tid < (int)(npix & 3)) {
        const long long i = nquads * 4 + tid;
        unsigned int r = base[i * CH], g = base[i * CH + 1], n = base[i * CH + 2];
        if (WB) { r = wb_map(r, 0); g = wb_map(g, 1); n = wb_map(n, 2); }
        if (WB && owb) {
            owb[i * CH] = (uint8_t)r; owb[i * CH + 1] = (uint8_t)g; owb[i * CH + 2] = (uint8_t)n;
            if (CH == 4) owb[i * CH + 3] = 0;
        }
        float a = 0, bq = 0, c = 0;
        pixel_math<MASK, STATS, false, !U16, HIST_COPIES>((float)r, (float)g, (float)n, 0u, a, bq, c, acc, s_hist, s_edges);
        if ((MASK & 1u) && oi0) oi0[i] = a;
        if ((MASK & 2u) && oi1) oi1[i] = bq;
        if ((MASK & 4u) && oi2) oi2[i] = c;
        if ((MASK & 1u) && oc0) reinterpret_cast<unsigned int *>(oc0)[i] = lut0[cmap_index(a)];
        if ((MASK & 2u) && oc1) reinterpret_cast<unsigned int *>(oc1)[i] = lut1[cmap_index(bq)];
        if ((MASK & 4u) && oc2) reinterpret_cast<unsigned int *>(oc2)[i] = lut2[cmap_index(c)];
    }

    if (STATS >= 1) {
        StatsAccView *rec = reinterpret_cast<StatsAccView *>(P.stats + tile * 3);
#pragma unroll
        for (int k = 0; k < 3; ++k)
            if ((MASK & (1u << k)) && (P.mask & (1u << k))) acc_flush(acc[k], rec + k, s_red, tid);
        if (STATS >= 2) {
            __syncthreads();
            for (int i = tid; i < 3 * LARS_HIST_BINS; i += 256) {
                const int k = i / LARS_HIST_BINS;
                unsigned int v = 0;
#pragma unroll
                for (int c = 0; c < HIST_COPIES; ++c) v += s_hist_all[i * HIST_COPIES + ((c + i) & (HIST_COPIES - 1))];
                if ((MASK & (1u << k)) && (P.mask & (1u << k)) && v) atomicAdd(&rec[k].hist[i - k * LARS_HIST_BINS], (unsigned long long)v);
            }
        }
    }
}

template <typename PIX, int NVAL>
__global__ __launch_bounds__(256) void k_fused_generic(FusedParams P)
{
    __shared__ unsigned int s_hist[3 * LARS_HIST_BINS];
    __shared__ HistCell<float> s_edges[LARS_HIST_CELLS];
    __shared__ double s_red[4][4];

    const int tid = threadIdx.x;
    const long long tile = blockIdx.y;
    const long long npix = P.npix;
    const int C = P.channels;
    const unsigned mask = P.mask;
    const bool stats = P.flags & (LARS_F_STATS | LARS_F_HIST | LARS_F_SUMSQ);
    const bool hist = P.flags & (LARS_F_HIST | LARS_F_SUMSQ);
    const bool sumsq = P.flags & LARS_F_SUMSQ;
    const PIX *base = static_cast<const PIX *>(P.tiles) + tile * npix * C;
    const uint8_t *tab = P.wb_table ? P.wb_table + tile * (NVAL == 256 ? 768ll : (long long)LARS_U16_BLOB_BYTES) : nullptr;

    for (int i = tid; i < 3 * LARS_HIST_BINS; i += 256) s_hist[i] = 0;
    hist_cells_init<float>(s_edges, tid);
    __syncthreads();

    Acc acc[3];
    acc_init(acc[0]); acc_init(acc[1]); acc_init(acc[2]);
    float *const oi0 = P.out_index[0] ? P.out_index[0] + tile * npix : nullptr;
    float *const oi1 = P.out_index[1] ? P.out_index[1] + tile * npix : nullptr;
    float *const oi2 = P.out_index[2] ? P.out_index[2] + tile * npix : nullptr;
    uint8_t *const owb = P.out_wb ? P.out_wb + tile * npix * C : nullptr;
    unsigned int *const oc0 = P.out_rgba[0] ? reinterpret_cast<unsigned int *>(P.out_rgba[0]) + tile * npix : nullptr;
    unsigned int *const oc1 = P.out_rgba[1] ? reinterpret_cast<unsigned int *>(P.out_rgba[1]) + tile * npix : nullptr;
    unsigned int *const oc2 = P.out_rgba[2] ? reinterpret_cast<unsigned int *>(P.out_rgba[2]) + tile * npix : nullptr;
    const unsigned int *lut0 = reinterpret_cast<const unsigned int *>(P.cmap_lut[0]);
    const unsigned int *lut1 = reinterpret_cast<const unsigned int *>(P.cmap_lut[1]);
    const unsigned int *lut2 = reinterpret_cast<const unsigned int *>(P.cmap_lut[2]);

    for (long long i = (long long)blockIdx.x * 256 + tid; i < npix; i += (long long)gridDim.x * 256) {
        const PIX *p = base + i * C;
        unsigned int r = p[0], g = p[1], n = p[2];
        if (tab) {
            r = tab[r]; g = tab[NVAL + g]; n = tab[2 * NVAL + n];
            if (owb) {
                uint8_t *o = owb + i * C;
                o[0] = (uint8_t)r; o[1] = (uint8_t)g; o[2] = (uint8_t)n;
                for (int c = 3; c < C; ++c) o[c] = 0;
            }
        }
        float a = 0, b = 0, c = 0;
        if (stats) {
            if (sumsq) pixel_math<7u, 3, true>((float)r, (float)g, (float)n, mask, a, b, c, acc, s_hist, s_edges);
            else if (hist) pixel_math<7u, 2, true>((float)r, (float)g, (float)n, mask, a, b, c, acc, s_hist, s_edges);
            else pixel_math<7u, 1, true>((float)r, (float)g, (float)n, mask, a, b, c, acc, s_hist, s_edges);
        } else {
            pixel_math<7u, 0, true>((float)r, (float)g, (float)n, mask, a, b, c, acc, s_hist, s_edges);
        }
        if ((mask & 1u) && oi0) oi0[i] = a;
        if ((mask & 2u) && oi1) oi1[i] = b;
        if ((mask & 4u) && oi2) oi2[i] = c;
        if ((mask & 1u) && oc0) oc0[i] = lut0[cmap_index(a)];
        if ((mask & 2u) && oc1) oc1[i] = lut1[cmap_index(b)];
        if ((mask & 4u) && oc2) oc2[i] = lut2[cmap_index(c)];
    }
    if (stats) {
        StatsAccView *rec = reinterpret_cast<StatsAccView *>(P.stats + tile * 3);
        for (int k = 0; k < 3; ++k)
            if (mask & (1u << k)) acc_flush(acc[k], rec + k, s_red, tid);
        if (hist) {
            __syncthreads();
            for (int i = tid; i < 3 * LARS_HIST_BINS; i += 256) {
                const int k = i / LARS_HIST_BINS;
                if ((mask & (1u << k)) && s_hist[i])
                    atomicAdd(&rec[k].hist[i - k * LARS_HIST_BINS], (unsigned long long)s_hist[i]);
            }
        }
    }
}

__device__ inline unsigned int mix32(unsigned int x)
{
    x ^= x >> 16; x *= 0x7FEB352Du; x ^= x >> 15; x *= 0x846CA68Bu; x ^= x >> 16;
    return x;
}
__device__ inline unsigned int veg_byte(unsigned int v, int ch)
{
    return ch == 0 ? 20u + (v * 3u) / 8u : ch == 1 ? 40u + v / 2u : ch == 2 ? 60u + (v * 3u) / 4u : v;
}

__global__ __launch_bounds__(256) void k_synth_u8(uint8_t *tiles, long long first_tile, long long nbytes,
                                                  int channels, unsigned int seed, int profile)
{
    const long long tile_local = blockIdx.y;
    const unsigned int salt = (unsigned int)(first_tile + tile_local) * 0x9E3779B9u;
    uint8_t *base = tiles + tile_local * nbytes;
    const long long nwords = (nbytes + 3) >> 2;
    for (long long k = (long long)blockIdx.x * 256 + threadIdx.x; k < nwords; k += (long long)gridDim.x * 256) {
        unsigned int w = mix32(mix32((unsigned int)k + seed) ^ salt);
        if (profile == 1) {
            unsigned int o = 0;
            for (int j = 0; j < 4; ++j) {
                const int ch = (int)((k * 4 + j) % channels);
                o |= (veg_byte((w >> (8 * j)) & 0xFF, ch) & 0xFF) << (8 * j);
            }
            w = o;
        }
        const long long off = k * 4;
        if (off + 4 <= nbytes && ((reinterpret_cast<uintptr_t>(base + off) & 3) == 0)) {
            *reinterpret_cast<unsigned int *>(base + off) = w;
        } else {
            for (int j = 0; j < 4 && off + j < nbytes; ++j) base[off + j] = (uint8_t)(w >> (8 * j));
        }
    }
}

}

using namespace lars;

namespace lars {
int blocks_per_tile(long long work_items, long long ntiles, int threads, long long target_total)
{
    long long want = (target_total * 256 / threads + ntiles - 1) / ntiles;
    if (tuning().blocks_per_tile > 0) want = tuning().blocks_per_tile;
    long long cap = work_items / ((long long)threads * 16);
    if (cap < 1) cap = 1;
    if (want > cap && tuning().blocks_per_tile <= 0) want = cap;
    const long long hard = (work_items + threads - 1) / threads;
    if (want > hard) want = hard;
    if (want < 1) want = 1;
    if (want > 65535) want = 65535;
    return (int)want;
}
}

extern "C" int lars_d_channel_hist(const void *tiles, int64_t ntiles, int64_t npix, int channels, int dtype,
                                   uint32_t *hist, void *stream)
{
    ThreadCtx *c;
    LARS_TRY(ensure_ctx(&c));
    if (!tiles || !hist || ntiles <= 0 || npix <= 0 || channels < 3)
        return fail(LARS_ERR_INVALID, "lars_d_channel_hist: bad arguments");
    if (ntiles > 65535) return fail(LARS_ERR_INVALID, "lars_d_channel_hist: ntiles > 65535 per call");
    hipStream_t s = pick_stream(c, stream);
    const int nval = dtype == LARS_U8 ? 256 : 65536;
    if (dtype != LARS_U8 && dtype != LARS_U16) return fail(LARS_ERR_INVALID, "lars_d_channel_hist: dtype");
    LARS_HIP_TRY(hipMemsetAsync(hist, 0, (size_t)ntiles * 3 * nval * sizeof(uint32_t), s));
    const bool fast = dtype == LARS_U8 && channels == 3 && (ntiles == 1 || (npix & 3) == 0) &&
                      ((reinterpret_cast<uintptr_t>(tiles) & 3) == 0);
    const bool fast4 = dtype == LARS_U8 && channels == 4 && (reinterpret_cast<uintptr_t>(tiles) & 15) == 0 &&
                       (ntiles == 1 || (npix & 3) == 0) && (long long)npix * 4 < (1ll << 30);
    if ((fast && tuning().hist_impl != 1 && (long long)npix * 3 < (1ll << 30)) || fast4) {
        long long want = tuning().blocks_per_tile > 0 ? tuning().blocks_per_tile : (1024 + ntiles - 1) / ntiles;
        const long long cap = (npix / 4 + 1023) / 1024;
        if (want > cap) want = cap;
        if (want < 1) want = 1;
        dim3 grid((unsigned)want, (unsigned)ntiles);
        chan_hist_v2_launch(static_cast<const uint8_t *>(tiles), (long long)npix, hist, grid, s, channels);
    } else if (fast) {
        dim3 grid(blocks_per_tile(npix / 4 + 1, ntiles), (unsigned)ntiles);
        hipLaunchKernelGGL(k_chan_hist_u8c3, grid, dim3(256), 0, s, static_cast<const uint8_t *>(tiles),
                           (long long)npix, hist);
    } else if (dtype == LARS_U8) {
        dim3 grid(blocks_per_tile(npix, ntiles), (unsigned)ntiles);
        hipLaunchKernelGGL((k_chan_hist_generic<uint8_t, 256>), grid, dim3(256), 0, s,
                           static_cast<const uint8_t *>(tiles), (long long)npix, channels, hist);
    } else {
        dim3 grid(blocks_per_tile(npix, ntiles), (unsigned)ntiles);
        hipLaunchKernelGGL((k_chan_hist_generic<uint16_t, 65536>), grid, dim3(256), 0, s,
                           static_cast<const uint16_t *>(tiles), (long long)npix, channels, hist);
    }
    return launch_check("lars_d_channel_hist");
}

extern "C" int lars_d_wb_table(const uint32_t *hist, int64_t ntiles, int64_t npix, int dtype, uint8_t *table,
                               double *percentiles, int rgn_variant, void *stream)
{
    ThreadCtx *c;
    LARS_TRY(ensure_ctx(&c));
    if (!hist || !table || ntiles <= 0 || npix <= 0) return fail(LARS_ERR_INVALID, "lars_d_wb_table: bad arguments");
    if (ntiles > 65535) return fail(LARS_ERR_INVALID, "lars_d_wb_table: ntiles > 65535 per call");
    hipStream_t s = pick_stream(c, stream);
    dim3 grid(3, (unsigned)ntiles);
    if (dtype == LARS_U8)
        hipLaunchKernelGGL((k_wb_table<256>), grid, dim3(256), 0, s, hist, (long long)npix, table, percentiles, rgn_variant);
    else if (dtype == LARS_U16)
        hipLaunchKernelGGL((k_wb_table<65536>), grid, dim3(256), 0, s, hist, (long long)npix, table, percentiles, rgn_variant);
    else
        return fail(LARS_ERR_INVALID, "lars_d_wb_table: dtype");
    return launch_check("lars_d_wb_table");
}

template <typename PIX, unsigned MASK, bool WB, int CH, int POLICY>
static void launch_fast_stats(int stats_mode, dim3 grid, hipStream_t s, const FusedParams &P)
{
    if (stats_mode == 0) hipLaunchKernelGGL((k_fused_u8c3<PIX, MASK, WB, 0, CH, POLICY>), grid, dim3(256), 0, s, P);
    else if (stats_mode == 1) hipLaunchKernelGGL((k_fused_u8c3<PIX, MASK, WB, 1, CH, POLICY>), grid, dim3(256), 0, s, P);
    else if (stats_mode == 3) hipLaunchKernelGGL((k_fused_u8c3<PIX, MASK, WB, 3, CH, POLICY>), grid, dim3(256), 0, s, P);
    else hipLaunchKernelGGL((k_fused_u8c3<PIX, MASK, WB, 2, CH, POLICY>), grid, dim3(256), 0, s, P);
}
template <typename PIX, unsigned MASK, int CH, int POLICY>
static void launch_fast_wb(bool wb, int stats_mode, dim3 grid, hipStream_t s, const FusedParams &P)
{
    if (wb) launch_fast_stats<PIX, MASK, true, CH, POLICY>(stats_mode, grid, s, P);
    else launch_fast_stats<PIX, MASK, false, CH, POLICY>(stats_mode, grid, s, P);
}
template <typename PIX, int CH, int POLICY>
static void launch_fast_policy(unsigned mask, bool wb, int stats_mode, dim3 grid, hipStream_t s, const FusedParams &P)
{
    switch (mask) {
    case 0u: hipLaunchKernelGGL((k_fused_u8c3<PIX, 0u, true, 0, CH, POLICY>), grid, dim3(256), 0, s, P); break;
    case 1u: launch_fast_wb<PIX, 1u, CH, POLICY>(wb, stats_mode, grid, s, P); break;
    case 2u: launch_fast_wb<PIX, 2u, CH, POLICY>(wb, stats_mode, grid, s, P); break;
    case 4u: launch_fast_wb<PIX, 4u, CH, POLICY>(wb, stats_mode, grid, s, P); break;
    default: launch_fast_wb<PIX, 7u, CH, POLICY>(wb, stats_mode, grid, s, P); break;
    }
}
template <typename PIX, int CH = 3>
static void launch_fast(unsigned mask, bool wb, int stats_mode, dim3 grid, hipStream_t s, const FusedParams &P, bool default_nt = false)
{
    if (stream_loads_nt(default_nt)) launch_fast_policy<PIX, CH, LOAD_NT>(mask, wb, stats_mode, grid, s, P);
    else launch_fast_policy<PIX, CH, LOAD_PLAIN>(mask, wb, stats_mode, grid, s, P);
}

extern "C" int lars_d_fused(const lars_fused_args *a)
{
    ThreadCtx *c;
    LARS_TRY(ensure_ctx(&c));
    if (!a || !a->tiles || a->ntiles <= 0 || a->npix <= 0 || a->channels < 3)
        return fail(LARS_ERR_INVALID, "lars_d_fused: bad arguments");
    if (a->ntiles > 65535) return fail(LARS_ERR_INVALID, "lars_d_fused: ntiles > 65535 per call");
    if (a->dtype != LARS_U8 && a->dtype != LARS_U16) return fail(LARS_ERR_INVALID, "lars_d_fused: dtype");
    const unsigned mask = a->index_mask & LARS_MASK_ALL;
    if (a->index_mask & ~LARS_MASK_ALL) return fail(LARS_ERR_INVALID, "lars_d_fused: unknown index bits in mask");
    const int stats_mode = (a->flags & LARS_F_SUMSQ) ? 3 : (a->flags & LARS_F_HIST) ? 2 : (a->flags & LARS_F_STATS) ? 1 : 0;
    if (stats_mode && !a->stats) return fail(LARS_ERR_INVALID, "lars_d_fused: stats requested but stats == NULL");
    if (a->out_wb && !a->wb_table) return fail(LARS_ERR_INVALID, "lars_d_fused: out_wb needs wb_table");
    for (int k = 0; k < 3; ++k)
        if (a->out_rgba[k] && !a->cmap_lut[k]) return fail(LARS_ERR_INVALID, "lars_d_fused: out_rgba needs cmap_lut");
    if (mask == 0 && !a->out_wb) return fail(LARS_ERR_INVALID, "lars_d_fused: nothing to do");
    hipStream_t s = pick_stream(c, a->stream);

    FusedParams P;
    P.tiles = a->tiles; P.npix = a->npix; P.channels = a->channels; P.wb_table = a->wb_table;
    for (int k = 0; k < 3; ++k) {
        const bool on = (mask >> k) & 1u;
        P.out_index[k] = on ? a->out_index[k] : nullptr;
        P.out_rgba[k] = on ? a->out_rgba[k] : nullptr;
        P.cmap_lut[k] = a->cmap_lut[k];
    }
    P.out_wb = a->out_wb; P.stats = a->stats; P.mask = mask; P.sel_hist = nullptr; P.sel_win = nullptr; P.sel_win_hist = nullptr; P.sel_below = nullptr;
    P.flags = (a->flags & 7u) | (tuning().nt_stores ? 0x20000000u : 0u);
#ifdef LARS_LAB_LAYOUT
    P.out_tile_stride = a->npix * (tuning().out_stride_planes > 1 ? tuning().out_stride_planes : 1);
#endif

    const long long nrec = a->ntiles * 3;
    const bool raw = (a->flags & LARS_F_RAW) != 0;
    if (stats_mode && !raw)
        hipLaunchKernelGGL(k_stats_init, dim3((unsigned)((nrec + 255) / 256)), dim3(256), 0, s, a->stats, nrec, mask);

    const bool aligned = (reinterpret_cast<uintptr_t>(a->tiles) & 3) == 0 &&
                         (!a->out_wb || (reinterpret_cast<uintptr_t>(a->out_wb) & 3) == 0) &&
                         (!P.out_index[0] || (reinterpret_cast<uintptr_t>(P.out_index[0]) & 15) == 0) &&
                         (!P.out_index[1] || (reinterpret_cast<uintptr_t>(P.out_index[1]) & 15) == 0) &&
                         (!P.out_index[2] || (reinterpret_cast<uintptr_t>(P.out_index[2]) & 15) == 0) &&
                         (!P.out_rgba[0] || (reinterpret_cast<uintptr_t>(P.out_rgba[0]) & 15) == 0) &&
                         (!P.out_rgba[1] || (reinterpret_cast<uintptr_t>(P.out_rgba[1]) & 15) == 0) &&
                         (!P.out_rgba[2] || (reinterpret_cast<uintptr_t>(P.out_rgba[2]) & 15) == 0);
    const unsigned tmask = (mask == 3u || mask == 5u || mask == 6u) ? 7u : mask;
    const bool ch_ok = a->channels == 3 || (a->channels == 4 && a->dtype == LARS_U8 && (reinterpret_cast<uintptr_t>(a->tiles) & 15) == 0 &&
                                            (!a->out_wb || (reinterpret_cast<uintptr_t>(a->out_wb) & 15) == 0));
    const bool fast = ch_ok && aligned && (a->ntiles == 1 || (a->npix & 3) == 0);
    const bool any_out = P.out_wb || P.out_index[0] || P.out_index[1] || P.out_index[2] || P.out_rgba[0] ||
                         P.out_rgba[1] || P.out_rgba[2];
    int impl = tuning().fused_impl;
    if (impl == 0) impl = (any_out && mask != 0u) ? 1 : 2;
    const bool small_tile = (long long)a->npix * 6 < (1ll << 30);
    int &ran = tuning().last_fused_kernel;
    if (fast && a->dtype == LARS_U8 && a->channels == 3 && impl >= 2 && small_tile) {
        dim3 grid(blocks_per_tile(a->npix / 4 + 1, a->ntiles, fused_v2_threads(any_out || mask == 0u)), (unsigned)a->ntiles);
        fused_v2_launch(tmask, a->wb_table != nullptr, stats_mode, tuning().nt_stores != 0, grid, s, P);
        ran = 2;
    } else if (fast && a->dtype == LARS_U8 && a->channels == 4) {
        dim3 grid(blocks_per_tile(a->npix / 4 + 1, a->ntiles, 256, 32768), (unsigned)a->ntiles);
        launch_fast<uint8_t, 4>(tmask, a->wb_table != nullptr, stats_mode, grid, s, P);
        ran = 5;
    } else if (fast && a->dtype == LARS_U8) {
        dim3 grid(blocks_per_tile(a->npix / 4 + 1, a->ntiles, 256, 32768), (unsigned)a->ntiles);
        const bool three_planes_stats = tmask == 7u && stats_mode == 1 && a->wb_table && P.out_index[0] && P.out_index[1] && P.out_index[2];
        launch_fast<uint8_t>(tmask, a->wb_table != nullptr, stats_mode, grid, s, P, three_planes_stats);
        ran = 1;
    } else if (fast && a->dtype == LARS_U16 && small_tile) {
        dim3 grid(blocks_per_tile(a->npix / 4 + 1, a->ntiles, 256, 32768), (unsigned)a->ntiles);
        launch_fast<uint16_t>(tmask, a->wb_table != nullptr, stats_mode, grid, s, P);
        ran = 3;
    } else {
        dim3 grid(blocks_per_tile(a->npix, a->ntiles), (unsigned)a->ntiles);
        if (a->dtype == LARS_U8) hipLaunchKernelGGL((k_fused_generic<uint8_t, 256>), grid, dim3(256), 0, s, P);
        else hipLaunchKernelGGL((k_fused_generic<uint16_t, 65536>), grid, dim3(256), 0, s, P);
        ran = 4;
    }
    if (stats_mode && !raw)
        hipLaunchKernelGGL(k_stats_finalize, dim3((unsigned)((nrec + 255) / 256)), dim3(256), 0, s, a->stats, nrec, mask,
                           (long long)a->npix);
    return launch_check("lars_d_fused");
}

extern "C" int lars_d_stats_begin(lars_stats *stats, int64_t ntiles, uint32_t index_mask, void *stream)
{
    ThreadCtx *c;
    LARS_TRY(ensure_ctx(&c));
    if (!stats || ntiles <= 0 || (index_mask & ~LARS_MASK_ALL)) return fail(LARS_ERR_INVALID, "lars_d_stats_begin: bad arguments");
    stats_init_launch(stats, ntiles * 3, index_mask & LARS_MASK_ALL, pick_stream(c, stream));
    return launch_check("lars_d_stats_begin");
}
extern "C" int lars_d_stats_end(lars_stats *stats, int64_t ntiles, uint32_t index_mask, int64_t npix, void *stream)
{
    ThreadCtx *c;
    LARS_TRY(ensure_ctx(&c));
    if (!stats || ntiles <= 0 || npix <= 0 || (index_mask & ~LARS_MASK_ALL)) return fail(LARS_ERR_INVALID, "lars_d_stats_end: bad arguments");
    stats_finalize_launch(stats, ntiles * 3, index_mask & LARS_MASK_ALL, (long long)npix, pick_stream(c, stream));
    return launch_check("lars_d_stats_end");
}

extern "C" int lars_d_stats_fold(const lars_stats *tile_records, int64_t ntiles, uint32_t index_mask, lars_stats *out, void *stream)
{
    ThreadCtx *c;
    LARS_TRY(ensure_ctx(&c));
    if (!tile_records || !out || ntiles <= 0 || !(index_mask & LARS_MASK_ALL) || (index_mask & ~LARS_MASK_ALL))
        return fail(LARS_ERR_INVALID, "lars_d_stats_fold: bad arguments");
    hipLaunchKernelGGL(k_stats_fold, dim3(3), dim3(256), 0, pick_stream(c, stream), tile_records, (long long)ntiles,
                       index_mask & LARS_MASK_ALL, out);
    return launch_check("lars_d_stats_fold");
}

extern "C" int lars_d_synth_u8(uint8_t *tiles, int64_t ntiles, int64_t first_tile, int64_t npix, int channels,
                               uint32_t seed, int profile, void *stream)
{
    ThreadCtx *c;
    LARS_TRY(ensure_ctx(&c));
    if (!tiles || ntiles <= 0 || npix <= 0 || channels < 1 || ntiles > 65535)
        return fail(LARS_ERR_INVALID, "lars_d_synth_u8: bad arguments");
    hipStream_t s = pick_stream(c, stream);
    const long long nbytes = (long long)npix * channels;
    dim3 grid(blocks_per_tile((nbytes + 3) / 4, ntiles), (unsigned)ntiles);
    hipLaunchKernelGGL(k_synth_u8, grid, dim3(256), 0, s, tiles, (long long)first_tile, nbytes, channels, seed, profile);
    return launch_check("lars_d_synth_u8");
}

namespace lars {
void stats_init_launch(lars_stats *stats, long long nrec, unsigned int mask, hipStream_t s)
{
    hipLaunchKernelGGL(k_stats_init, dim3((unsigned)((nrec + 255) / 256)), dim3(256), 0, s, stats, nrec, mask);
}
void stats_finalize_launch(lars_stats *stats, long long nrec, unsigned int mask, long long npix, hipStream_t s)
{
    hipLaunchKernelGGL(k_stats_finalize, dim3((unsigned)((nrec + 255) / 256)), dim3(256), 0, s, stats, nrec, mask, npix);
}
}
```

lars_image_processing_amd/csrc/fused_v2.hip:

```cpp
#include <string.h>

#include <type_traits>

#include "v2_device.h"

namespace lars {

__global__ __launch_bounds__(256) void k_quot_check(unsigned int max_den, unsigned long long *mismatches,
                                                    unsigned int *first_bad)
{
    unsigned long long bad = 0;
    for (unsigned int den = blockIdx.x + 1; den <= max_den; den += gridDim.x) {
        const float fd = (float)den;
        for (long long num = -(long long)den + threadIdx.x; num <= (long long)den; num += 256) {
            const float fn = (float)num;
            const float want = fn / fd;
            const float got = exact_quot(fn, fd);
            if (__builtin_bit_cast(unsigned int, want) != __builtin_bit_cast(unsigned int, got)) {
                if (!bad) { first_bad[0] = den; first_bad[1] = (unsigned int)(int)num; }
                ++bad;
            }
        }
    }
    if (bad) atomicAdd(mismatches, bad);
}

template <int CH, int POLICY = LOAD_PLAIN>
__global__ __launch_bounds__(1024) void k_chan_hist_u8c3_v2(const uint8_t *__restrict__ tiles, long long npix,
                                                            unsigned int *__restrict__ hist)
{
    __shared__ unsigned int s_h[3 * 256 * 32];
    const int tid = threadIdx.x;
    for (int i = tid; i < 3 * 256 * 32; i += 1024) s_h[i] = 0;
    __syncthreads();

    const long long tile = blockIdx.y;
    const uint8_t *base = tiles + tile * npix * CH;
    const long long nquads = npix >> 2;
    const unsigned int lane_off = (tid & 31) << 2;
    char *hb = reinterpret_cast<char *>(s_h);
#define HADD(word, shift, ch)                                                                          \
    atomicAdd(reinterpret_cast<unsigned int *>(hb + (ch) * 32768 + ((((word) >> (shift)) & 0xFFu) << 7) + lane_off), 1u)
    const long long step = (long long)gridDim.x * 1024;
    const long long q0 = (long long)blockIdx.x * 1024 + tid;
    const long long niter = (nquads + step - 1) / step;
#define HQUAD(a0, a1, a2)                                                                              \
    HADD(a0, 0, 0); HADD(a0, 8, 1); HADD(a0, 16, 2); HADD(a0, 24, 0);                                 \
    HADD(a1, 0, 1); HADD(a1, 8, 2); HADD(a1, 16, 0); HADD(a1, 24, 1);                                 \
    HADD(a2, 0, 2); HADD(a2, 8, 0); HADD(a2, 16, 1); HADD(a2, 24, 2);
    if (niter > 0 && CH == 4) {
        const __amdgpu_buffer_rsrc_t rsrc =
            __builtin_amdgcn_make_buffer_rsrc(const_cast<uint8_t *>(base), 0, (int)(nquads * 16), 0x00020000);
        const unsigned int voff = (unsigned int)q0 * 16u;
        const unsigned int step_b = (unsigned int)step * 16u;
        sl_u32x4 w[4];
#define HQUAD4(p)                                                                                       \
        {                                                                                               \
            const u32x3 a = rgba_quad_to_rgb(p);                                                        \
            HQUAD(a.x, a.y, a.z)                                                                        \
        }
#pragma unroll
        for (int k = 0; k < 4; ++k) w[k] = stream_load_b128<POLICY>(rsrc, voff, (unsigned)k * step_b);
        long long it = 0;
        unsigned int soff = 4u * step_b;
        for (; it + 4 <= niter - 1; it += 4) {
#pragma unroll
            for (int k = 0; k < 4; ++k) {
                HQUAD4(w[k])
                __builtin_amdgcn_sched_barrier(0);
                w[k] = stream_load_b128<POLICY>(rsrc, voff, soff + (unsigned)k * step_b);
                __builtin_amdgcn_sched_barrier(0);
            }
            soff += 4u * step_b;
        }
#pragma unroll
        for (int k = 0; k < 4; ++k) {
            if (it + k < niter && q0 + (it + k) * step < nquads) { HQUAD4(w[k]) }
        }
#undef HQUAD4
    } else if (niter > 0) {
        const __amdgpu_buffer_rsrc_t rsrc =
            __builtin_amdgcn_make_buffer_rsrc(const_cast<uint8_t *>(base), 0, (int)(nquads * 12), 0x00020000);
        const unsigned int voff = (unsigned int)q0 * 12u;
        const unsigned int step_b = (unsigned int)step * 12u;
        u32x3 w[4];
#pragma unroll
        for (int k = 0; k < 4; ++k) w[k] = stream_load_b96<POLICY>(rsrc, voff, (unsigned)k * step_b);
        long long it = 0;
        unsigned int soff = 4u * step_b;
        for (; it + 4 <= niter - 1; it += 4) {
#pragma unroll
            for (int k = 0; k < 4; ++k) {
                HQUAD(w[k].x, w[k].y, w[k].z)
                __builtin_amdgcn_sched_barrier(0);
                w[k] = stream_load_b96<POLICY>(rsrc, voff, soff + (unsigned)k * step_b);
                __builtin_amdgcn_sched_barrier(0);
            }
            soff += 4u * step_b;
        }
#pragma unroll
        for (int k = 0; k < 4; ++k) {
            if (it + k < niter && q0 + (it + k) * step < nquads) { HQUAD(w[k].x, w[k].y, w[k].z) }
        }
    }
#undef HQUAD
    if (blockIdx.x == 0 && tid < (int)(npix & 3)) {
        const uint8_t *p = base + (nquads * 4 + tid) * CH;
        HADD((unsigned)p[0], 0, 0); HADD((unsigned)p[1], 0, 1); HADD((unsigned)p[2], 0, 2);
    }
#undef HADD
    __syncthreads();
    if (tid < 768) {
        const unsigned int *row = s_h + tid * 32;
        unsigned int v = 0;
        for (int j = 0; j < 32; ++j) v += row[(j + tid) & 31];
        if (v) atomicAdd(&hist[tile * 768 + tid], v);
    }
}

typedef float f32x4 __attribute__((ext_vector_type(4)));
template <bool NT>
__device__ inline void store4(float *dst, float a, float b, float c, float d)
{
    f32x4 v = {a, b, c, d};
    if (NT) __builtin_nontemporal_store(v, reinterpret_cast<f32x4 *>(dst));
    else *reinterpret_cast<f32x4 *>(dst) = v;
}

struct WaveAcc {
    float mn, mx;
    double sum, sumsq;
};

#define V2_HIST_COPIES 16
#define V2_HIST_SHIFT 6
#define V2_HIST_ROWS 51
#define V2_HIST_WORDS (3 * V2_HIST_ROWS * V2_HIST_COPIES)
#define V2_WIN_ROW (64 + SELQ_WIN_SLOTS + 64)

__device__ inline void count_gt(unsigned int &counter, float x, float thr)
{
    unsigned int c;
    asm volatile("v_cmp_lt_f32 vcc, %1, %2\n\ts_bcnt1_i32_b64 %0, vcc" : "=s"(c) : "s"(thr), "v"(x) : "vcc", "scc");
    counter += c;
}
__device__ inline void count_lt(unsigned int &counter, float x, float thr)
{
    unsigned int c;
    asm volatile("v_cmp_gt_f32 vcc, %1, %2\n\ts_bcnt1_i32_b64 %0, vcc" : "=s"(c) : "s"(thr), "v"(x) : "vcc", "scc");
    counter += c;
}

__device__ inline void count4_gt(unsigned int &counter, const float (&x)[4], float thr)
{
    unsigned int c;
    asm volatile("v_cmp_lt_f32 vcc, %1, %2\n\ts_bcnt1_i32_b64 %0, vcc\n\t"
                 "v_cmp_lt_f32 vcc, %1, %3\n\ts_bcnt1_i32_b64 vcc_lo, vcc\n\ts_add_u32 %0, %0, vcc_lo\n\t"
                 "v_cmp_lt_f32 vcc, %1, %4\n\ts_bcnt1_i32_b64 vcc_lo, vcc\n\ts_add_u32 %0, %0, vcc_lo\n\t"
                 "v_cmp_lt_f32 vcc, %1, %5\n\ts_bcnt1_i32_b64 vcc_lo, vcc\n\ts_add_u32 %0, %0, vcc_lo"
                 : "=&s"(c) : "s"(thr), "v"(x[0]), "v"(x[1]), "v"(x[2]), "v"(x[3]) : "vcc", "scc");
    counter += c;
}
__device__ inline void count4_lt(unsigned int &counter, const float (&x)[4], float thr)
{
    unsigned int c;
    asm volatile("v_cmp_gt_f32 vcc, %1, %2\n\ts_bcnt1_i32_b64 %0, vcc\n\t"
                 "v_cmp_gt_f32 vcc, %1, %3\n\ts_bcnt1_i32_b64 vcc_lo, vcc\n\ts_add_u32 %0, %0, vcc_lo\n\t"
                 "v_cmp_gt_f32 vcc, %1, %4\n\ts_bcnt1_i32_b64 vcc_lo, vcc\n\ts_add_u32 %0, %0, vcc_lo\n\t"
                 "v_cmp_gt_f32 vcc, %1, %5\n\ts_bcnt1_i32_b64 vcc_lo, vcc\n\ts_add_u32 %0, %0, vcc_lo"
                 : "=&s"(c) : "s"(thr), "v"(x[0]), "v"(x[1]), "v"(x[2]), "v"(x[3]) : "vcc", "scc");
    counter += c;
}

template <int STATS, bool COUNT = true>
__device__ inline void push(WaveAcc &a, unsigned int &above, float x, float thr)
{
    a.mn = fminf(a.mn, x);
    a.mx = fmaxf(a.mx, x);
    const double xd = (double)x;
    a.sum += xd;
    if (STATS >= 3) a.sumsq += xd * xd;
    if (COUNT) count_gt(above, x, thr);
}
// ... 180 lines not shown
                if (STATS >= 2) hist_add(x, 1.0f, hb1);
                if (oi1) oi1[i] = x;
                if (oc1) reinterpret_cast<unsigned int *>(oc1)[i] = lut1[cmap_index(x)];
            }
            if (WANT_NDWI) {
                const float w = 0.0f - x;
                if (STATS >= 2) hist_add(x, -1.0f, hb2);
                if (oi2) oi2[i] = w;
                if (oc2) reinterpret_cast<unsigned int *>(oc2)[i] = lut2[cmap_index(w)];
            }
        }
    }

    if (STATS >= 2 || SEL) asm volatile("s_waitcnt lgkmcnt(0)" ::: "memory");
    if (RED_ALIASES_TABLE) __syncthreads();
    if (STATS >= 1) {
        for (int off = 32; off >= 1; off >>= 1) {
            if (WANT_NDVI) {
                acc_v.mn = fminf(acc_v.mn, __shfl_xor(acc_v.mn, off)); acc_v.mx = fmaxf(acc_v.mx, __shfl_xor(acc_v.mx, off));
                acc_v.sum += __shfl_xor(acc_v.sum, off);
                if (STATS >= 3) acc_v.sumsq += __shfl_xor(acc_v.sumsq, off);
            }
            if (NEED_G) {
                acc_g.mn = fminf(acc_g.mn, __shfl_xor(acc_g.mn, off)); acc_g.mx = fmaxf(acc_g.mx, __shfl_xor(acc_g.mx, off));
                acc_g.sum += __shfl_xor(acc_g.sum, off);
                if (STATS >= 3) acc_g.sumsq += __shfl_xor(acc_g.sumsq, off);
            }
        }
        const int wave = tid >> 6;
        double *row = s_red + wave * 16;
        if (lane == 0) {
            row[0] = acc_v.sum; row[1] = acc_v.sumsq; row[2] = (double)acc_v.mn; row[3] = (double)acc_v.mx; row[4] = (double)above_v;
            row[5] = acc_g.sum; row[6] = acc_g.sumsq; row[7] = (double)acc_g.mn; row[8] = (double)acc_g.mx;
            row[9] = (double)above_g; row[10] = (double)above_w;
        }
        __syncthreads();
        if (tid < 11) {
            const bool is_min = tid == 2 || tid == 7, is_max = tid == 3 || tid == 8;
            double t = s_red[tid];
#pragma unroll 1
            for (int w = 1; w < NWAVES; ++w) {
                const double o = s_red[w * 16 + tid];
                t = is_min ? fmin(t, o) : is_max ? fmax(t, o) : t + o;
            }
            s_red[tid] = t;
        }
        __syncthreads();
        if (tid == 0) {
            double t[11];
            for (int j = 0; j < 11; ++j) t[j] = s_red[j];
            StatsAccView *rec = reinterpret_cast<StatsAccView *>(P.stats + tile * 3);
            if (WANT_NDVI && (P.mask & 1u)) {
                atomicAdd(&rec[0].sum_fx, (unsigned long long)__double2ll_rn(t[0] * LARS_FX_SCALE));
                if (STATS >= 3) atomicAdd(&rec[0].sumsq_fx, (unsigned long long)__double2ll_rn(t[1] * LARS_FX_SCALE));
                atomicAdd(&rec[0].above, (unsigned long long)t[4]);
                atomicMin(&rec[0].min_key, f64_key(t[2]));
                atomicMax(&rec[0].max_key, f64_key(t[3]));
            }
            if (WANT_GNDVI && (P.mask & 2u)) {
                atomicAdd(&rec[1].sum_fx, (unsigned long long)__double2ll_rn(t[5] * LARS_FX_SCALE));
                if (STATS >= 3) atomicAdd(&rec[1].sumsq_fx, (unsigned long long)__double2ll_rn(t[6] * LARS_FX_SCALE));
                atomicAdd(&rec[1].above, (unsigned long long)t[9]);
                atomicMin(&rec[1].min_key, f64_key(t[7]));
                atomicMax(&rec[1].max_key, f64_key(t[8]));
            }
            if (WANT_NDWI && (P.mask & 4u)) {
                atomicAdd(&rec[2].sum_fx, (unsigned long long)__double2ll_rn((0.0 - t[5]) * LARS_FX_SCALE));
                if (STATS >= 3) atomicAdd(&rec[2].sumsq_fx, (unsigned long long)__double2ll_rn(t[6] * LARS_FX_SCALE));
                atomicAdd(&rec[2].above, (unsigned long long)t[10]);
                atomicMin(&rec[2].min_key, f64_key(0.0 - t[8]));
                atomicMax(&rec[2].max_key, f64_key(0.0 - t[7]));
            }
        }
        if (STATS >= 2) {
            __syncthreads();
            StatsAccView *rec = reinterpret_cast<StatsAccView *>(P.stats + tile * 3);
            if (tid < 3 * LARS_HIST_BINS) {
                const int k = tid / LARS_HIST_BINS;
                if ((MASK & (1u << k)) && (P.mask & (1u << k))) {
                    const int b = tid - k * LARS_HIST_BINS;
                    const unsigned int *rowh = s_hist + (k * V2_HIST_ROWS + b) * V2_HIST_COPIES;
                    unsigned int v = 0;
                    const int nwords = (b == LARS_HIST_BINS - 1) ? 2 * V2_HIST_COPIES : V2_HIST_COPIES;
                    for (int j = 0; j < nwords; ++j) v += rowh[j];
                    if (v) atomicAdd(&rec[k].hist[b], (unsigned long long)v);
                }
            }
        }
        if (SEL == 1) {
            unsigned int *h = P.sel_hist + tile * (4 * SELQ_BINS);
            for (int i = tid; i < 2 * SELQ_BINS; i += NTHR) {
                const unsigned int v = s_sel[i];
                if (v) atomicAdd(&h[(i >> 11) * (2 * SELQ_BINS) + (i & (SELQ_BINS - 1))], v);
            }
        }
        if (SEL == 2) {
            for (int i = tid; i < 2 * V2_WIN_ROW; i += NTHR) {
                const unsigned int v = s_win[i];
                if (!v) continue;
                const int stream = i / V2_WIN_ROW, w = i % V2_WIN_ROW;
                if (w < 64) atomicAdd(&P.sel_below[tile * 2 + stream], v);
                else if (w < 64 + SELQ_WIN_SLOTS) atomicAdd(&P.sel_win_hist[(tile * 2 + stream) * SELQ_WIN_SLOTS + (w - 64)], v);
            }
        }
    }
}


}

using namespace lars;

namespace lars {


void fused_v2_sel_launch(unsigned mask, bool wb, int stats, dim3 grid, hipStream_t s, const FusedParams &P)
{
    const int what = (P.sel_win && stats == 1) ? 0 : stats >= 3 ? 3 : stats == 2 ? 2 : 1;
    with_constant<1u, 2u, 4u, 7u>((int)mask, [&](auto M) {
        with_constant<false, true>(wb, [&](auto W) {
            with_constant<0, 1, 2, 3>(what, [&](auto X) {
                constexpr int STATS = decltype(X)::value ? decltype(X)::value : 1, SEL = decltype(X)::value ? 1 : 2;
                hipLaunchKernelGGL((k_fused_v2<decltype(M)::value, decltype(W)::value, STATS, false, false, SEL>), grid,
                                   dim3(V2Block<false>::threads), 0, s, P);
            });
        });
    });
}

int fused_v2_threads(bool any_out) { return any_out ? V2Block<true>::threads : V2Block<false>::threads; }

void fused_v2_launch(unsigned mask, bool wb, int stats, bool nt, dim3 grid, hipStream_t s, const FusedParams &P)
{
    const bool out = P.out_wb || P.out_index[0] || P.out_index[1] || P.out_index[2] || P.out_rgba[0] || P.out_rgba[1] ||
                     P.out_rgba[2];
    if (mask == 0u) {
        hipLaunchKernelGGL((k_fused_v2<0u, true, 0, true, false>), grid, dim3(V2Block<true>::threads), 0, s, P);
        return;
    }
    const int planes = !out ? 0 : nt ? 2 : 1;
    with_constant<1u, 2u, 4u, 7u>((int)mask, [&](auto M) {
        with_constant<false, true>(wb, [&](auto W) {
            with_constant<0, 1, 2, 3>(stats, [&](auto S) {
                with_constant<0, 1, 2>(planes, [&](auto O) {
                    constexpr bool OUT = decltype(O)::value != 0, NT = decltype(O)::value == 2;
                    hipLaunchKernelGGL((k_fused_v2<decltype(M)::value, decltype(W)::value, decltype(S)::value, OUT, NT>), grid,
                                       dim3(V2Block<OUT>::threads), 0, s, P);
                });
            });
        });
    });
}

void chan_hist_v2_launch(const uint8_t *tiles, long long npix, unsigned int *hist, dim3 grid, hipStream_t s, int channels)
{
    const bool nt = stream_loads_nt(true);
    if (channels == 4 && nt) hipLaunchKernelGGL((k_chan_hist_u8c3_v2<4, LOAD_NT>), grid, dim3(1024), 0, s, tiles, npix, hist);
    else if (channels == 4) hipLaunchKernelGGL((k_chan_hist_u8c3_v2<4, LOAD_PLAIN>), grid, dim3(1024), 0, s, tiles, npix, hist);
    else if (nt) hipLaunchKernelGGL((k_chan_hist_u8c3_v2<3, LOAD_NT>), grid, dim3(1024), 0, s, tiles, npix, hist);
    else hipLaunchKernelGGL((k_chan_hist_u8c3_v2<3, LOAD_PLAIN>), grid, dim3(1024), 0, s, tiles, npix, hist);
}

int quot_check_launch(unsigned int max_den, unsigned long long *mismatches_dev, unsigned int *first_bad_dev, hipStream_t s)
{
    hipLaunchKernelGGL(k_quot_check, dim3(2048), dim3(256), 0, s, max_den, mismatches_dev, first_bad_dev);
    return launch_check("k_quot_check");
}

}
```

lars_image_processing_amd/csrc/runtime.cpp:

```cpp
#include <stdarg.h>
#include <stdlib.h>
#include <string.h>
#include <cmath>

#include "common.h"

namespace lars {

static thread_local ThreadCtx g_ctx;

static void release_ctx(ThreadCtx *c)
{
    if (c->device < 0) return;
    if (hipSetDevice(c->device) != hipSuccess) { c->device = -1; return; }
    align_release();
    if (c->stream) { hipStreamSynchronize(c->stream); hipStreamDestroy(c->stream); c->stream = nullptr; }
    if (c->ws) { hipFree(c->ws); c->ws = nullptr; c->ws_bytes = 0; }
    if (c->scratch) { hipFree(c->scratch); c->scratch = nullptr; c->scratch_bytes = 0; }
    if (c->outline) { hipFree(c->outline); c->outline = nullptr; c->outline_bytes = 0; }
    c->u16_win_tiles = 0;
    c->device = -1;
}
struct CtxGuard {
    ~CtxGuard() { release_ctx(&g_ctx); }
};
static thread_local CtxGuard g_ctx_guard;

static int bind_device(ThreadCtx *c, int ordinal)
{
    int count = 0;
    hipError_t e = hipGetDeviceCount(&count);
    if (e != hipSuccess || count <= 0)
        return fail(LARS_ERR_NO_DEVICE, "no HIP device available (%s); liblars_hip has no CPU fallback",
                    e == hipSuccess ? "device count 0" : hipGetErrorString(e));
    if (ordinal < 0 || ordinal >= count) return fail(LARS_ERR_INVALID, "device ordinal %d out of range [0,%d)", ordinal, count);
    hipDeviceProp_t prop;
    LARS_HIP_TRY(hipGetDeviceProperties(&prop, ordinal));
    if (strncmp(prop.gcnArchName, "gfx950", 6) != 0)
        return fail(LARS_ERR_NO_DEVICE, "device %d is %s; liblars_hip is built for gfx950 (MI355X) only", ordinal,
                    prop.gcnArchName);
    LARS_HIP_TRY(hipSetDevice(ordinal));
    if (c->stream) { hipStreamDestroy(c->stream); c->stream = nullptr; }
    if (c->ws) { hipFree(c->ws); c->ws = nullptr; c->ws_bytes = 0; }
    if (c->scratch) { hipFree(c->scratch); c->scratch = nullptr; c->scratch_bytes = 0; }
    if (c->outline) { hipFree(c->outline); c->outline = nullptr; c->outline_bytes = 0; }
    c->u16_win_tiles = 0;
    LARS_HIP_TRY(hipStreamCreateWithFlags(&c->stream, hipStreamNonBlocking));
    c->device = ordinal;
    (void)&g_ctx_guard;
    return LARS_OK;
}

int ensure_ctx(ThreadCtx **out)
{
    ThreadCtx *c = &g_ctx;
    if (c->device < 0) LARS_TRY(bind_device(c, 0));
    else LARS_HIP_TRY(hipSetDevice(c->device));
    *out = c;
    return LARS_OK;
}

static int reserve(void **p, size_t *have, size_t bytes, hipStream_t s)
{
    if (bytes <= *have) return LARS_OK;
    if (*p) {
        LARS_HIP_TRY(hipStreamSynchronize(s));
        LARS_HIP_TRY(hipFree(*p));
        *p = nullptr; *have = 0;
    }
    size_t want = bytes + (bytes >> 3);
    want = (want + 0xFFFFF) & ~(size_t)0xFFFFF;
    hipError_t e = hipMalloc(p, want);
    if (e != hipSuccess) {
        *p = nullptr;
        return fail(LARS_ERR_OOM, "hipMalloc(%zu) for the library workspace failed: %s", want, hipGetErrorString(e));
    }
    *have = want;
    return LARS_OK;
}
int ws_reserve(ThreadCtx *c, size_t bytes) { return reserve(&c->ws, &c->ws_bytes, bytes, c->stream); }
int scratch_reserve(ThreadCtx *c, size_t bytes)
{
    c->u16_win_tiles = 0;
    return reserve(&c->scratch, &c->scratch_bytes, bytes, c->stream);
}

int outline_reserve(ThreadCtx *c, size_t bytes) { return reserve(&c->outline, &c->outline_bytes, bytes, c->stream); }

static Tuning g_tuning;
Tuning &tuning() { return g_tuning; }

struct Knob {
    const char *name;
    int Tuning::*field;
    enum Access { SET, READ_ONLY, LAB_LAYOUT } access;
    bool (*allowed)(int);
    const char *domain;
};
#ifdef LARS_LAB_LAYOUT
static const bool kLabLayout = true;
#else
static const bool kLabLayout = false;
#endif
static const Knob KNOBS[] = {
    {"fused_impl", &Tuning::fused_impl, Knob::SET, nullptr, nullptr},
    {"hist_impl", &Tuning::hist_impl, Knob::SET, nullptr, nullptr},
    {"nt_stores", &Tuning::nt_stores, Knob::SET, nullptr, nullptr},
    {"blocks_per_tile", &Tuning::blocks_per_tile, Knob::SET, nullptr, nullptr},
    {"load_policy", &Tuning::load_policy, Knob::SET, [](int v) { return v >= 0 && v <= 2; }, "0 .. 2"},
    {"selq_window", &Tuning::selq_window, Knob::SET, nullptr, nullptr},
    {"selq_list_wgs", &Tuning::selq_list_wgs, Knob::SET, nullptr, nullptr},
    {"joint_depth", &Tuning::joint_depth, Knob::SET, [](int v) { return v == 4 || v == 6 || v == 8 || v == 12; }, "4, 6, 8 or 12"},
    {"joint_window", &Tuning::joint_window, Knob::SET, [](int v) { return v >= 0 && v <= 5; }, "0 .. 5"},
    {"joint_win_depth", &Tuning::joint_win_depth, Knob::SET, [](int v) { return v == 4 || v == 5 || v == 6 || v == 12 || v == 15; }, "4, 5, 6, 12 or 15"},
    {"out_stride_planes", &Tuning::out_stride_planes, Knob::LAB_LAYOUT, nullptr, nullptr},
    {"u16_hist_impl", &Tuning::u16_hist_impl, Knob::SET, [](int v) { return v == 5 || v == 1 || v == 3; }, "5, 1 or 3"},
    {"jpeg_subseq_bits", &Tuning::jpeg_subseq_bits, Knob::SET, [](int v) { return v >= 32 && v <= 65536; }, "32 .. 65536"},
    {"tiff_strip_bytes", &Tuning::tiff_strip_bytes, Knob::SET, [](int v) { return v >= 1 && v <= (1 << 30); }, "1 .. 1073741824"},
    {"deflate_matching", &Tuning::deflate_matching, Knob::SET, [](int v) { return v == 0 || v == 1; }, "0 or 1"},
    {"zone_split_pixels", &Tuning::zone_split_pixels, Knob::SET, [](int v) { return v >= 64 && v <= (1 << 30); }, "64 .. 1073741824"},
    {"last_fused_kernel", &Tuning::last_fused_kernel, Knob::READ_ONLY, nullptr, nullptr},
    {"jpeg_last_rounds", &Tuning::jpeg_last_rounds, Knob::READ_ONLY, nullptr, nullptr},
};
static const Knob *find_knob(const char *key)
{
    for (const Knob &k : KNOBS)
        if (!strcmp(key, k.name)) return &k;
    return nullptr;
}

int launch_check(const char *what)
{
    hipError_t e = hipGetLastError();
    if (e != hipSuccess) return fail(LARS_ERR_HIP, "%s: kernel launch failed: %s", what, hipGetErrorString(e));
    return LARS_OK;
}

}

using namespace lars;

extern "C" {


int lars_device_count(int *count)
{
    if (!count) return fail(LARS_ERR_INVALID, "lars_device_count: NULL");
    int n = 0;
    hipError_t e = hipGetDeviceCount(&n);
    if (e != hipSuccess) { *count = 0; return fail(LARS_ERR_NO_DEVICE, "hipGetDeviceCount: %s", hipGetErrorString(e)); }
    *count = n;
    return LARS_OK;
}

int lars_set_device(int ordinal) { return bind_device(&g_ctx, ordinal); }

int lars_get_device(int *ordinal)
{
    ThreadCtx *c;
    LARS_TRY(ensure_ctx(&c));
    if (ordinal) *ordinal = c->device;
    return LARS_OK;
}

int lars_device_name(char *buf, size_t buflen)
{
    ThreadCtx *c;
    LARS_TRY(ensure_ctx(&c));
    hipDeviceProp_t prop;
    LARS_HIP_TRY(hipGetDeviceProperties(&prop, c->device));
    snprintf(buf, buflen, "%s (%s, %d CUs, %.1f GiB)", prop.name, prop.gcnArchName, prop.multiProcessorCount,
             (double)prop.totalGlobalMem / (1024.0 * 1024.0 * 1024.0));
    return LARS_OK;
}

int lars_malloc(void **dptr, size_t bytes)
{
    ThreadCtx *c;
    LARS_TRY(ensure_ctx(&c));
    if (!dptr) return fail(LARS_ERR_INVALID, "lars_malloc: NULL");
    const hipError_t e = hipMalloc(dptr, bytes ? bytes : 1);
    if (e != hipSuccess) { *dptr = nullptr; return fail(LARS_ERR_OOM, "hipMalloc(%zu): %s", bytes, hipGetErrorString(e)); }
    return LARS_OK;
}
int lars_free(void *dptr)
{
    if (!dptr) return LARS_OK;
    ThreadCtx *c;
    LARS_TRY(ensure_ctx(&c));
    LARS_HIP_TRY(hipFree(dptr));
    return LARS_OK;
}
int lars_memset(void *dptr, int value, size_t bytes, void *stream)
{
    ThreadCtx *c;
    LARS_TRY(ensure_ctx(&c));
    LARS_HIP_TRY(hipMemsetAsync(dptr, value, bytes, pick_stream(c, stream)));
    return LARS_OK;
}
int lars_memcpy_h2d(void *dst, const void *src, size_t bytes)
{
    ThreadCtx *c;
    LARS_TRY(ensure_ctx(&c));
    LARS_HIP_TRY(hipMemcpyAsync(dst, src, bytes, hipMemcpyHostToDevice, c->stream));
    LARS_HIP_TRY(hipStreamSynchronize(c->stream));
    return LARS_OK;
}
int lars_memcpy_d2h(void *dst, const void *src, size_t bytes)
{
    ThreadCtx *c;
    LARS_TRY(ensure_ctx(&c));
    LARS_HIP_TRY(hipMemcpyAsync(dst, src, bytes, hipMemcpyDeviceToHost, c->stream));
    LARS_HIP_TRY(hipStreamSynchronize(c->stream));
    return LARS_OK;
}
int lars_memcpy_d2d(void *dst, const void *src, size_t bytes, void *stream)
{
    ThreadCtx *c;
    LARS_TRY(ensure_ctx(&c));
    LARS_HIP_TRY(hipMemcpyAsync(dst, src, bytes, hipMemcpyDeviceToDevice, pick_stream(c, stream)));
    return LARS_OK;
}
int lars_stream_create(void **stream)
{
    ThreadCtx *c;
    LARS_TRY(ensure_ctx(&c));
    hipStream_t s;
    LARS_HIP_TRY(hipStreamCreateWithFlags(&s, hipStreamNonBlocking));
    *stream = s;
    return LARS_OK;
}
int lars_stream_destroy(void *stream)
{
    if (stream) LARS_HIP_TRY(hipStreamDestroy(reinterpret_cast<hipStream_t>(stream)));
    return LARS_OK;
}
int lars_synchronize(void *stream)
{
    ThreadCtx *c;
    LARS_TRY(ensure_ctx(&c));
    LARS_HIP_TRY(hipStreamSynchronize(pick_stream(c, stream)));
    return LARS_OK;
}
int lars_shutdown(void)
{
    release_ctx(&g_ctx);
    return LARS_OK;
}

int lars_mem_info(size_t *free_bytes, size_t *total_bytes)
{
    ThreadCtx *c;
    LARS_TRY(ensure_ctx(&c));
    size_t f = 0, t = 0;
    LARS_HIP_TRY(hipMemGetInfo(&f, &t));
    if (free_bytes) *free_bytes = f;
    if (total_bytes) *total_bytes = t;
    return LARS_OK;
}

int lars_event_create(void **event)
{
    ThreadCtx *c;
    LARS_TRY(ensure_ctx(&c));
    hipEvent_t e;
    LARS_HIP_TRY(hipEventCreate(&e));
    *event = e;
    return LARS_OK;
}
int lars_event_destroy(void *event)
{
    if (event) LARS_HIP_TRY(hipEventDestroy(reinterpret_cast<hipEvent_t>(event)));
// ... 79 lines not shown
```

Before: 361,000.

## Predict white-balance percentiles from sampled histogram and verify during fused pass

```diff
diff --git a/include/lars_hip.h b/include/lars_hip.h
--- a/include/lars_hip.h
+++ b/include/lars_hip.h
@@ -155,6 +155,14 @@
 int lars_d_diff_f32(const float *early, const float *late, int64_t n, float *out_diff, void *stream);
 int lars_d_colormap_norm_f32(const float *x, int64_t n, float vmin, float vmax, const uint8_t *lut_rgba,
                              uint8_t *out_rgba, void *stream);
+
+size_t lars_wb_predict_bytes(int64_t ntiles);
+int64_t lars_wb_predict_floor_pixels(void);
+int64_t lars_wb_predict_sample_segment(int64_t npix, int frac_log2, int64_t s);
+int lars_d_wb_predict(const void *tiles, int64_t ntiles, int64_t npix, int frac_log2, double ksigma, int rgn_variant,
+                      uint32_t *sample_hist, uint32_t *pred, uint32_t *hist, uint8_t *table, double *percentiles, void *stream);
+int lars_d_fused_checked(const lars_fused_args *args, uint32_t *pred, uint32_t *hist, double *percentiles, int rgn_variant);
+int lars_wb_predict_report(const uint32_t *pred, int64_t ntiles, uint32_t *states, uint32_t *marks);
 
 int lars_d_synth_u8(uint8_t *tiles, int64_t ntiles, int64_t first_tile, int64_t npix, int channels,
                     uint32_t seed, int profile, void *stream);
diff --git a/lars_image_processing_amd/_ffi.py b/lars_image_processing_amd/_ffi.py
--- a/lars_image_processing_amd/_ffi.py
+++ b/lars_image_processing_amd/_ffi.py
@@ -166,6 +166,12 @@
     "lars_d_wb_prepare": (_I, [_P, _I64, _I64, _I, _I, _P, _P, _I, _P]),
     "lars_u16_window_report": (_I, [_I64, _P, _P]),
     "lars_d_fused": (_I, [C.POINTER(FusedArgs)]),
+    "lars_wb_predict_bytes": (_SZ, [_I64]),
+    "lars_wb_predict_floor_pixels": (_I64, []),
+    "lars_wb_predict_sample_segment": (_I64, [_I64, _I, _I64]),
+    "lars_d_wb_predict": (_I, [_P, _I64, _I64, _I, _D, _I, _P, _P, _P, _P, _P, _P]),
+    "lars_d_fused_checked": (_I, [C.POINTER(FusedArgs), _P, _P, _P, _I]),
+    "lars_wb_predict_report": (_I, [_P, _I64, _P, _P]),
     "lars_d_stats_begin": (_I, [_P, _I64, _U32, _P]),
     "lars_d_stats_end": (_I, [_P, _I64, _U32, _I64, _P]),
     "lars_d_index_planes_f32": (_I, [_P, _P, _P, _I64, _I, _P, _P]),
diff --git a/lars_image_processing_amd/batch.py b/lars_image_processing_amd/batch.py
--- a/lars_image_processing_amd/batch.py
+++ b/lars_image_processing_amd/batch.py
@@ -11,6 +11,16 @@
 from .arena import arena_placements
 
 MAX_TILES_PER_LAUNCH = 65535
+
+WB_PREDICT_FRACTION_LOG2 = 4
+WB_PREDICT_KSIGMA = 1.0
+
+
+def _knob(name):
+    v = C.c_int(0)
+    if _ffi.load().lars_get_tuning(name.encode(), C.byref(v)) != 0:
+        raise _ffi.LarsError(-1, f"lars_get_tuning: {name}")
+    return v.value
 
 
 _STATS_ROUTE = os.environ.get("LARS_STATS_ROUTE", "auto")
@@ -97,6 +107,54 @@
         self._joint_tiles = self.ntiles
         self._selq = None
         self.last_route = None
+        self._pred = None
+        self._sample_hist = None
+
+    _EXACT, _PENDING, _CHECKED = "exact", "pending", "checked"
+
+    def _settle(self, also_checked):
+        state = self.__dict__.get("_wb_state", self._EXACT)
+        if state == self._PENDING or (also_checked and state == self._CHECKED):
+            self.__dict__["_wb_state"] = self._EXACT
+            d = self.__dict__
+            _ffi.call("lars_d_channel_hist", C.c_void_p(self.tiles.ptr), self.ntiles, self.npix, self.channels, self.code,
+                      C.c_void_p(d["_hist"].ptr), d.get("_wb_stream"))
+            _ffi.call("lars_d_wb_table", C.c_void_p(d["_hist"].ptr), self.ntiles, self.npix, self.code, C.c_void_p(d["_table"].ptr),
+                      C.c_void_p(d["_percentiles"].ptr), self._rgn_variant, d.get("_wb_stream"))
+            self._pred.zero(d.get("_wb_stream"))
+            self._hist_channels = {0, 1, 2}
+
+    def _wb_buffer(name, also_checked=False):
+        def get(self):
+            self._settle(also_checked)
+            return self.__dict__.get(name)
+
+        def put(self, value):
+            self.__dict__[name] = value
+            self.__dict__["_wb_state"] = self._EXACT
+
+        return property(get, put)
+
+    table = _wb_buffer("_table")
+    percentiles = _wb_buffer("_percentiles")
+    hist = _wb_buffer("_hist", also_checked=True)
+    del _wb_buffer
+
+    def can_predict_wb(self):
+        if not (self.code == _ffi.U8 and self.channels == 3 and (self.ntiles == 1 or self.npix % 4 == 0) and self.tiles.ptr % 4 == 0
+                and self.npix * 3 < (1 << 30)):
+            return False
+        knob = _knob("wb_predict")
+        if knob == 0 or _knob("hist_impl") == 1 or _knob("fused_impl") >= 2:
+            return False
+        return knob >= 2 or self.npix >= int(_ffi.load().lars_wb_predict_floor_pixels())
+
+    def wb_predict_report(self):
+        states = np.zeros(self.ntiles, np.uint32)
+        marks = np.zeros((self.ntiles, 3, 2), np.uint32)
+        if self._pred is not None:
+            _ffi.call("lars_wb_predict_report", C.c_void_p(self._pred.ptr), self.ntiles, _ffi.ptr(states), _ffi.ptr(marks))
+        return states, marks
 
     @classmethod
     def from_host(cls, array, first_tile=0):
@@ -120,12 +178,27 @@
         return self.tiles.download(self.dtype, (count, self.h, self.w, self.channels), start * self.tile_bytes)
 
     def compute_wb_tables(self, stream=None, rgn_variant=0):
+        self.__dict__["_wb_state"] = self._EXACT
         if self.table is None:
             self.table = DeviceBuffer(self.ntiles * self.table_bytes)
             self.percentiles = DeviceBuffer(self.ntiles * 3 * 2 * 8)
+        if self.code == _ffi.U8 and self.hist is None:
+            self.hist = DeviceBuffer(self.ntiles * 3 * 256 * 4)
+        if self.can_predict_wb():
+            if self._pred is None:
+                self._pred = DeviceBuffer(int(_ffi.load().lars_wb_predict_bytes(self.ntiles)))
+                self._sample_hist = DeviceBuffer(self.ntiles * 3 * 256 * 4)
+            _ffi.call("lars_d_wb_predict", C.c_void_p(self.tiles.ptr), self.ntiles, self.npix, WB_PREDICT_FRACTION_LOG2, WB_PREDICT_KSIGMA,
+                      int(rgn_variant), C.c_void_p(self._sample_hist.ptr), C.c_void_p(self._pred.ptr), C.c_void_p(self._hist.ptr),
+                      C.c_void_p(self._table.ptr), C.c_void_p(self._percentiles.ptr), stream)
+            self._wb_state, self._wb_stream = self._PENDING, stream
+            self._table_channels = {0, 1, 2}
+            self._hist_channels = set()
+            self._rgn_variant = int(rgn_variant)
+            return self
+        if self._pred is not None:
+            self._pred.zero(stream)
         if self.code == _ffi.U8:
-            if self.hist is None:
-                self.hist = DeviceBuffer(self.ntiles * 3 * 256 * 4)
             _ffi.call("lars_d_channel_hist", C.c_void_p(self.tiles.ptr), self.ntiles, self.npix, self.channels,
                       self.code, C.c_void_p(self.hist.ptr), stream)
             _ffi.call("lars_d_wb_table", C.c_void_p(self.hist.ptr), self.ntiles, self.npix, self.code,
@@ -164,6 +237,7 @@
         return self.percentiles.download(np.float64, (self.ntiles, 3, 2))
 
     def host_hist(self, partial=False):
+        self._settle(True)
         self._need_channels(partial)
         if self.hist is None or (not partial and self._hist_channels != {0, 1, 2}):
             missing = sorted({0, 1, 2} - self._hist_channels)
@@ -235,15 +309,16 @@
         return timed / len(launches)
 
     def fused_args(self, indices=INDEX_NAMES, white_balance=True, stats=None, hist=False, outputs=None,
-                   stream=None, tile_start=0, tile_count=None, sumsq=False, raw=False):
+                   stream=None, tile_start=0, tile_count=None, sumsq=False, raw=False, checked=False):
         tile_count = self.ntiles - tile_start if tile_count is None else tile_count
         a = FusedArgs()
         a.tiles = self.tiles.ptr + tile_start * self.tile_bytes
         a.ntiles, a.npix, a.channels, a.dtype = tile_count, self.npix, self.channels, self.code
         if white_balance:
-            if self.table is None:
+            table = self._table if checked else self.table
+            if table is None:
                 raise RuntimeError("compute_wb_tables() first")
-            a.wb_table = self.table.ptr + tile_start * self.table_bytes
+            a.wb_table = table.ptr + tile_start * self.table_bytes
         a.index_mask = index_mask(indices)
         a.flags = ((_ffi.F_STATS if stats is not None else 0) | (_ffi.F_HIST if (stats is not None and hist) else 0) |
                    (_ffi.F_SUMSQ if (stats is not None and sumsq) else 0) | (_ffi.F_RAW if (stats is not None and raw) else 0))
@@ -276,32 +351,47 @@
 
     def run_fused_chunks(self, indices, white_balance, stats, hist, outputs, stream=None, sumsq=False, launch_events=None):
         chunk = self.ntiles if outputs is None else outputs.slots
+        mask = index_mask(indices)
+        checked = (self.__dict__.get("_wb_state") == self._PENDING and white_balance and stats is not None and not hist and not sumsq
+                   and mask == 7 and outputs is not None and all(p is not None for p in outputs.index)
+                   and outputs.wb is None and all(p is None for p in outputs.rgba)
+                   and all(p.ptr % 16 == 0 for p in outputs.index)
+                   and _knob("fused_impl") < 2 and _knob("hist_impl") != 1)
+        if checked:
+            self._wb_stream = stream
         if chunk >= self.ntiles:
             if launch_events:
                 _ffi.call("lars_event_record", launch_events[0], stream)
-            self.run_fused(self.fused_args(indices, white_balance, stats, hist, outputs, stream, sumsq=sumsq))
+            self.run_fused(self.fused_args(indices, white_balance, stats, hist, outputs, stream, sumsq=sumsq, checked=checked), 0, checked)
             if launch_events and len(launch_events) > 1:
                 _ffi.call("lars_event_record", launch_events[1], stream)
-            return 1
-        mask = index_mask(indices)
-        if stats is not None:
-            _ffi.call("lars_d_stats_begin", C.c_void_p(stats.ptr), self.ntiles, mask, stream)
-        launches = 0
-        if launch_events:
-            _ffi.call("lars_event_record", launch_events[0], stream)
-        for start in range(0, self.ntiles, chunk):
-            count = min(chunk, self.ntiles - start)
-            self.run_fused(self.fused_args(indices, white_balance, stats, hist, outputs, stream, start, count, sumsq=sumsq,
-                                           raw=stats is not None))
-            launches += 1
-            if launch_events and launches < len(launch_events):
-                _ffi.call("lars_event_record", launch_events[launches], stream)
-        if stats is not None:
-            _ffi.call("lars_d_stats_end", C.c_void_p(stats.ptr), self.ntiles, mask, self.npix, stream)
+            launches = 1
+        else:
+            if stats is not None:
+                _ffi.call("lars_d_stats_begin", C.c_void_p(stats.ptr), self.ntiles, mask, stream)
+            launches = 0
+            if launch_events:
+                _ffi.call("lars_event_record", launch_events[0], stream)
+            for start in range(0, self.ntiles, chunk):
+                count = min(chunk, self.ntiles - start)
+                self.run_fused(self.fused_args(indices, white_balance, stats, hist, outputs, stream, start, count, sumsq=sumsq,
+                                               raw=stats is not None, checked=checked), start, checked)
+                launches += 1
+                if launch_events and launches < len(launch_events):
+                    _ffi.call("lars_event_record", launch_events[launches], stream)
+            if stats is not None:
+                _ffi.call("lars_d_stats_end", C.c_void_p(stats.ptr), self.ntiles, mask, self.npix, stream)
+        if checked:
+            self._wb_state = self._CHECKED
         return launches
 
-    def run_fused(self, args):
-        _ffi.call("lars_d_fused", C.byref(args))
+    def run_fused(self, args, tile_start=0, checked=False):
+        if not checked:
+            _ffi.call("lars_d_fused", C.byref(args))
+            return
+        _ffi.call("lars_d_fused_checked", C.byref(args), C.c_void_p(self._pred.ptr + tile_start * (self._pred.nbytes // self.ntiles)),
+                  C.c_void_p(self._hist.ptr + tile_start * 3 * 256 * 4), C.c_void_p(self._percentiles.ptr + tile_start * 3 * 2 * 8),
+                  self._rgn_variant)
 
     def can_joint(self):
         return joint_serves(self.code, self.channels, self.ntiles, self.npix)
@@ -501,7 +591,9 @@
         return rec, med
 
     def free(self):
-        for b in (self.tiles, self.hist, self.table, self.percentiles, self._joint_scratch, self._selq):
+        d = self.__dict__
+        for b in (self.tiles, d.get("_hist"), d.get("_table"), d.get("_percentiles"), self._joint_scratch, self._selq, self._pred,
+                  self._sample_hist):
             if b is not None:
                 b.free()
 
diff --git a/lars_image_processing_amd/csrc/common.h b/lars_image_processing_amd/csrc/common.h
--- a/lars_image_processing_amd/csrc/common.h
+++ b/lars_image_processing_amd/csrc/common.h
@@ -128,9 +128,11 @@
     int tiff_strip_bytes = 65536;
     int deflate_matching = 0;
     int joint_window = 1;
+    int wb_predict = 1;
     int zone_split_pixels = 131072;
 };
 Tuning &tuning();
+#define LARS_WB_PREDICT_FLOOR_PIXELS (1 << 20)
 inline bool stream_loads_nt(bool kernel_default_nt)
 {
     const int k = tuning().load_policy;
@@ -146,7 +148,11 @@
 #endif
 int fused_v2_threads(bool any_out);
 void fused_v2_launch(unsigned mask, bool wb, int stats, bool nt, dim3 grid, hipStream_t s, const FusedParams &P);
-void chan_hist_v2_launch(const uint8_t *tiles, long long npix, unsigned int *hist, dim3 grid, hipStream_t s, int channels = 3);
+void chan_hist_v2_launch(const uint8_t *tiles, long long npix, unsigned int *hist, dim3 grid, hipStream_t s, int channels = 3,
+                         const unsigned int *gate = nullptr, unsigned int gate_mask = 0u);
+void wb_exact_gated_launch(const uint8_t *tiles, long long ntiles, long long npix, unsigned int *hist, uint8_t *table, double *pcts,
+                           int rgn_variant, const unsigned int *pred, unsigned int gate_mask, int blocks, hipStream_t s);
+void wb_check_launch(unsigned int *pred, long long ntiles, long long npix, lars_stats *stats, hipStream_t s);
 int selq_pass_launch(const uint8_t *tiles, const uint8_t *wb_table, long long ntiles, long long npix, int first,
                      const unsigned int bucket[4], unsigned long long *hist, hipStream_t s, unsigned streams);
 size_t selq_tile_scratch_bytes(long long ntiles);
diff --git a/lars_image_processing_amd/csrc/device_common.h b/lars_image_processing_amd/csrc/device_common.h
--- a/lars_image_processing_amd/csrc/device_common.h
+++ b/lars_image_processing_amd/csrc/device_common.h
@@ -20,6 +20,7 @@
     const unsigned int *sel_win;
     unsigned int *sel_win_hist;
     unsigned int *sel_below;
+    unsigned int *pred;
 #ifdef LARS_LAB_LAYOUT
     long long out_tile_stride;
 #endif
@@ -107,6 +108,47 @@
     return rgn_variant ? (unsigned int)(int)y : (unsigned int)(int)(float)y;
 }
 
+__device__ inline void wb_mark_ranks(long long n, int k, long long &lo, long long &hi, double &t)
+{
+    const double q = (k == 0 ? 2.0 : 98.0) / 100.0;
+    const double vi = (double)(n - 1) * q;
+    const double fl = floor(vi);
+    lo = (long long)fl;
+    hi = lo + 1;
+    if (hi > n - 1) hi = n - 1;
+    t = vi - fl;
+}
+__device__ inline double wb_mark_lerp(double a, double b, double t)
+{
+    const double d = b - a;
+    return t >= 0.5 ? b - d * (1.0 - t) : a + d * t;
+}
+__device__ inline void wb_table_row_u8(uint8_t *row, int tid, double p_lo, double p_hi, int rgn_variant)
+{
+    row[tid] = (uint8_t)wb_level(tid, p_lo, p_hi, rgn_variant);
+}
+
+#define LARS_PRED_EXACT 0u
+#define LARS_PRED_PREDICTED 1u
+#define LARS_PRED_CONFIRMED 2u
+#define LARS_PRED_REPAIRED 3u
+#define LARS_PRED_WORDS 20
+#define LARS_PRED_MARKS 1
+#define LARS_PRED_COUNTS 8
+__device__ inline bool pred_gate(const unsigned int *gate, long long tile, unsigned int mask)
+{
+    return !gate || ((1u << gate[tile * LARS_PRED_WORDS]) & mask);
+}
+
+__device__ inline void stats_rec_init(StatsAccView *a, int k)
+{
+    a->sum_fx = 0; a->sumsq_fx = 0; a->count = 0; a->above = 0; a->nans = 0;
+    a->min_key = ~0ull; a->max_key = 0ull;
+    a->threshold = (k == LARS_NDWI) ? 0.0 : (double)0.2f;
+    a->index_id = (unsigned)k; a->reserved = 0;
+    for (int b = 0; b < LARS_HIST_BINS; ++b) a->hist[b] = 0;
+}
+
 __device__ inline void u16_fill_blob(uint8_t *blob, int c, double p_lo, double p_hi, int rgn_variant,
                                      unsigned int *s_thr, int tid)
 {
diff --git a/lars_image_processing_amd/csrc/fused.hip b/lars_image_processing_amd/csrc/fused.hip
--- a/lars_image_processing_amd/csrc/fused.hip
+++ b/lars_image_processing_amd/csrc/fused.hip
@@ -83,8 +83,10 @@
 template <int NVAL>
 __global__ __launch_bounds__(256) void k_wb_table(const unsigned int *__restrict__ hist, long long npix,
                                                   uint8_t *__restrict__ table, double *__restrict__ pcts,
-                                                  int rgn_variant)
-{
+                                                  int rgn_variant, const unsigned int *__restrict__ gate = nullptr,
+                                                  unsigned int gate_mask = 0u)
+{
+    if (!pred_gate(gate, blockIdx.y, gate_mask)) return;
     constexpr int PER = NVAL / 256;
     __shared__ unsigned long long s_scan[4];
     __shared__ double s_val[4];
@@ -99,20 +101,9 @@
     for (int j = 0; j < PER; ++j) local += h[tid * PER + j];
     const unsigned long long before = wg_exscan<256>(local, s_scan);
 
-    const double nm1 = (double)(npix - 1);
     double tq[2];
     long long rank[4];
-    for (int k = 0; k < 2; ++k) {
-        const double q = (k == 0 ? 2.0 : 98.0) / 100.0;
-        const double vi = nm1 * q;
-        const double fl = floor(vi);
-        long long lo = (long long)fl;
-        long long hi = lo + 1;
-        if (hi > npix - 1) hi = npix - 1;
-        rank[2 * k] = lo;
-        rank[2 * k + 1] = hi;
-        tq[k] = vi - fl;
-    }
+    for (int k = 0; k < 2; ++k) wb_mark_ranks(npix, k, rank[2 * k], rank[2 * k + 1], tq[k]);
     unsigned long long cum = before;
     for (int j = 0; j < PER; ++j) {
         const unsigned long long c = h[tid * PER + j];
@@ -125,18 +116,14 @@
     }
     __syncthreads();
     if (tid < 2) {
-        const double a = s_val[2 * tid], b = s_val[2 * tid + 1], t = tq[tid];
-        const double d = b - a;
-        double r = a + d * t;
-        if (t >= 0.5) r = b - d * (1.0 - t);
+        const double r = wb_mark_lerp(s_val[2 * tid], s_val[2 * tid + 1], tq[tid]);
         s_p[tid] = r;
         if (pcts) pcts[slot * 2 + tid] = r;
     }
     __syncthreads();
     const double p_lo = s_p[0], p_hi = s_p[1];
     if (NVAL == 256) {
-        uint8_t *out = table + slot * 256;
-        out[tid] = (uint8_t)wb_level(tid, p_lo, p_hi, rgn_variant);
+        wb_table_row_u8(table + slot * 256, tid, p_lo, p_hi, rgn_variant);
     } else {
         u16_fill_blob(table + (long long)blockIdx.y * LARS_U16_BLOB_BYTES, (int)blockIdx.x, p_lo, p_hi, rgn_variant, s_thr, tid);
     }
@@ -148,12 +135,7 @@
     if (i >= nrec) return;
     const int k = (int)(i % 3);
     if (!((mask >> k) & 1u)) return;
-    StatsAccView *a = reinterpret_cast<StatsAccView *>(stats + i);
-    a->sum_fx = 0; a->sumsq_fx = 0; a->count = 0; a->above = 0; a->nans = 0;
-    a->min_key = ~0ull; a->max_key = 0ull;
-    a->threshold = (k == LARS_NDWI) ? 0.0 : (double)0.2f;
-    a->index_id = (unsigned)k; a->reserved = 0;
-    for (int b = 0; b < LARS_HIST_BINS; ++b) a->hist[b] = 0;
+    stats_rec_init(reinterpret_cast<StatsAccView *>(stats + i), k);
 }
 
 __global__ void k_stats_finalize(lars_stats *stats, long long nrec, unsigned int mask, long long npix)
@@ -283,13 +265,23 @@
 }
 
 
-template <typename PIX, unsigned MASK, bool WB, int STATS, int CH = 3, int POLICY = LOAD_PLAIN>
+template <typename PIX, unsigned MASK, bool WB, int STATS, int CH = 3, int CHECK = 0, int POLICY = LOAD_PLAIN>
 __global__ __launch_bounds__(256)
-__attribute__((amdgpu_waves_per_eu(1, (sizeof(PIX) == 1 && CH == 3 && MASK != 0u && STATS <= 1) ? 3 : 8))) void k_fused_u8c3(FusedParams P)
+__attribute__((amdgpu_waves_per_eu(CHECK == 1 ? 2 : 1, (sizeof(PIX) == 1 && CH == 3 && MASK != 0u && STATS <= 1) ? 3 : 8))) void k_fused_u8c3(FusedParams P)
 {
     constexpr bool U16 = sizeof(PIX) == 2;
+    constexpr bool CK = CHECK == 1;
     static_assert(CH == 3 || (CH == 4 && !U16), "4-channel fast path: uint8 tiles");
-    __shared__ uint8_t s_lut[U16 ? 16 : 3 * 256];
+    static_assert(CHECK == 0 || (!U16 && WB), "predicted tables: uint8 tiles with white balance");
+    if (CHECK != 0) {
+        const unsigned int st = P.pred[(long long)blockIdx.y * LARS_PRED_WORDS];
+        if (CK ? st != LARS_PRED_PREDICTED : (st != LARS_PRED_EXACT && st != LARS_PRED_REPAIRED)) return;
+    }
+    constexpr int CK_COPIES = 64;
+    __shared__ unsigned int s_lutw[CK ? 3 * 256 : 1];
+    __shared__ unsigned int s_ck[CK ? 12 * CK_COPIES : 1];
+    unsigned int ck[3] = {0u, 0u, 0u};
+    __shared__ uint8_t s_lut[(U16 || CK) ? 16 : 3 * 256];
     __shared__ unsigned int s_thr[U16 ? 3 * 260 : 4];
     __shared__ double s_par[U16 ? 6 : 1];
     constexpr int HIST_COPIES = 16;
@@ -311,6 +303,15 @@
             const double *par = reinterpret_cast<const double *>(blob + LARS_U16_PAR_OFFSET);
             for (int i = tid; i < 3 * 260; i += 256) s_thr[i] = thr[i];
             if (tid < 6) s_par[tid] = par[tid];
+        } else if (CK) {
+            const uint8_t *t = P.wb_table + tile * 768;
+            const unsigned int *mk = P.pred + tile * LARS_PRED_WORDS + LARS_PRED_MARKS;
+            for (int i = tid; i < 768; i += 256) {
+                const unsigned int x = (unsigned)i & 255u, v2 = mk[2 * (i >> 8)], v98 = mk[2 * (i >> 8) + 1];
+                s_lutw[i] = ((unsigned int)t[i] << 24) | (x < v2 ? 1u : 0u) | (x <= v2 ? 1u << 6 : 0u) | (x < v98 ? 1u << 12 : 0u) |
+                            (x <= v98 ? 1u << 18 : 0u);
+            }
+            for (int i = tid; i < 12 * CK_COPIES; i += 256) s_ck[i] = 0;
         } else {
             const uint8_t *t = P.wb_table + tile * 768;
             for (int i = tid; i < 768; i += 256) s_lut[i] = t[i];
@@ -323,6 +324,11 @@
     if (WB || STATS >= 2) __syncthreads();
 
     auto wb_map = [&](unsigned int v, int c) -> unsigned int {
+        if (CK) {
+            const unsigned int e = s_lutw[c * 256 + v];
+            ck[c] += e;
+            return e >> 24;
+        }
         if (!U16) return s_lut[c * 256 + v];
         const double y = ((double)v - s_par[2 * c]) * s_par[2 * c + 1];
         int g = (int)y;
@@ -390,6 +396,7 @@
 #pragma unroll
             for (int i = 0; i < 12; ++i)
                 if (i % 3 == 2 || (i % 3 == 0 && need_r) || (i % 3 == 1 && need_g)) b[i] = wb_map(b[i], i % 3);
+            if (CK) asm("" : "+v"(ck[0]), "+v"(ck[1]), "+v"(ck[2]));
             if (owb && CH == 4) {
                 *reinterpret_cast<uint4 *>(owb + q * 16) = make_uint4(b[0] | (b[1] << 8) | (b[2] << 16), b[3] | (b[4] << 8) | (b[5] << 16),
                                                                       b[6] | (b[7] << 8) | (b[8] << 16), b[9] | (b[10] << 8) | (b[11] << 16));
@@ -425,6 +432,15 @@
     const long long nsteps = (nquads + 64 * RUN - 1) / (64 * RUN);
     const long long wstride = (long long)gx * 4;
     const unsigned int lane = (unsigned int)tid & 63u;
+    auto ck_flush = [&]() {
+#pragma unroll
+        for (int c = 0; c < 3; ++c) {
+#pragma unroll
+            for (int k = 0; k < 4; ++k) atomicAdd(&s_ck[(c * 4 + k) * CK_COPIES + lane], (ck[c] >> (6 * k)) & 63u);
+            ck[c] = 0u;
+        }
+    };
+    static_assert(RUN % 8 == 0 || !CK, "the packed counters are emptied every eight quads");
     for (long long st = (long long)bx * 4 + (tid >> 6); st < nsteps; st += wstride) {
         const long long q0 = st * (64 * RUN) + lane;
         unsigned int w[RUN][NW];
@@ -435,12 +451,14 @@
 #pragma unroll
             for (int j = 0; j < RUN; ++j) {
                 do_quad(q0 + 64 * j, w[j]);
+                if (CK && (j & 7) == 7) ck_flush();
                 __builtin_amdgcn_sched_barrier(0);
             }
         } else {
             for (int j = 0; j < RUN; ++j) {
                 const long long q = q0 + 64 * j;
                 if (q < nquads) { load_quad(q, w[0]); do_quad(q, w[0]); }
+                if (CK && (j & 7) == 7) ck_flush();
             }
         }
     }
@@ -460,6 +478,16 @@
         if ((MASK & 1u) && oc0) reinterpret_cast<unsigned int *>(oc0)[i] = lut0[cmap_index(a)];
         if ((MASK & 2u) && oc1) reinterpret_cast<unsigned int *>(oc1)[i] = lut1[cmap_index(bq)];
         if ((MASK & 4u) && oc2) reinterpret_cast<unsigned int *>(oc2)[i] = lut2[cmap_index(c)];
+    }
+
+    if (CK) {
+        ck_flush();
+        __syncthreads();
+        if (tid < 12) {
+            unsigned int v = 0;
+            for (int c = 0; c < CK_COPIES; ++c) v += s_ck[tid * CK_COPIES + c];
+            if (v) atomicAdd(&P.pred[tile * LARS_PRED_WORDS + LARS_PRED_COUNTS + tid], v);
+        }
     }
 
     if (STATS >= 1) {
@@ -672,10 +700,10 @@
 template <typename PIX, unsigned MASK, bool WB, int CH, int POLICY>
 static void launch_fast_stats(int stats_mode, dim3 grid, hipStream_t s, const FusedParams &P)
 {
-    if (stats_mode == 0) hipLaunchKernelGGL((k_fused_u8c3<PIX, MASK, WB, 0, CH, POLICY>), grid, dim3(256), 0, s, P);
-    else if (stats_mode == 1) hipLaunchKernelGGL((k_fused_u8c3<PIX, MASK, WB, 1, CH, POLICY>), grid, dim3(256), 0, s, P);
-    else if (stats_mode == 3) hipLaunchKernelGGL((k_fused_u8c3<PIX, MASK, WB, 3, CH, POLICY>), grid, dim3(256), 0, s, P);
-    else hipLaunchKernelGGL((k_fused_u8c3<PIX, MASK, WB, 2, CH, POLICY>), grid, dim3(256), 0, s, P);
+    if (stats_mode == 0) hipLaunchKernelGGL((k_fused_u8c3<PIX, MASK, WB, 0, CH, 0, POLICY>), grid, dim3(256), 0, s, P);
+    else if (stats_mode == 1) hipLaunchKernelGGL((k_fused_u8c3<PIX, MASK, WB, 1, CH, 0, POLICY>), grid, dim3(256), 0, s, P);
+    else if (stats_mode == 3) hipLaunchKernelGGL((k_fused_u8c3<PIX, MASK, WB, 3, CH, 0, POLICY>), grid, dim3(256), 0, s, P);
+    else hipLaunchKernelGGL((k_fused_u8c3<PIX, MASK, WB, 2, CH, 0, POLICY>), grid, dim3(256), 0, s, P);
 }
 template <typename PIX, unsigned MASK, int CH, int POLICY>
 static void launch_fast_wb(bool wb, int stats_mode, dim3 grid, hipStream_t s, const FusedParams &P)
@@ -687,7 +715,7 @@
 static void launch_fast_policy(unsigned mask, bool wb, int stats_mode, dim3 grid, hipStream_t s, const FusedParams &P)
 {
     switch (mask) {
-    case 0u: hipLaunchKernelGGL((k_fused_u8c3<PIX, 0u, true, 0, CH, POLICY>), grid, dim3(256), 0, s, P); break;
+    case 0u: hipLaunchKernelGGL((k_fused_u8c3<PIX, 0u, true, 0, CH, 0, POLICY>), grid, dim3(256), 0, s, P); break;
     case 1u: launch_fast_wb<PIX, 1u, CH, POLICY>(wb, stats_mode, grid, s, P); break;
     case 2u: launch_fast_wb<PIX, 2u, CH, POLICY>(wb, stats_mode, grid, s, P); break;
     case 4u: launch_fast_wb<PIX, 4u, CH, POLICY>(wb, stats_mode, grid, s, P); break;
@@ -699,6 +727,23 @@
 {
     if (stream_loads_nt(default_nt)) launch_fast_policy<PIX, CH, LOAD_NT>(mask, wb, stats_mode, grid, s, P);
     else launch_fast_policy<PIX, CH, LOAD_PLAIN>(mask, wb, stats_mode, grid, s, P);
+}
+
+static void fused_params(const lars_fused_args *a, unsigned mask, FusedParams &P)
+{
+    P.tiles = a->tiles; P.npix = a->npix; P.channels = a->channels; P.wb_table = a->wb_table;
+    for (int k = 0; k < 3; ++k) {
+        const bool on = (mask >> k) & 1u;
+        P.out_index[k] = on ? a->out_index[k] : nullptr;
+        P.out_rgba[k] = on ? a->out_rgba[k] : nullptr;
+        P.cmap_lut[k] = a->cmap_lut[k];
+    }
+    P.out_wb = a->out_wb; P.stats = a->stats; P.mask = mask; P.sel_hist = nullptr; P.sel_win = nullptr; P.sel_win_hist = nullptr; P.sel_below = nullptr;
+    P.pred = nullptr;
+    P.flags = (a->flags & 7u) | (tuning().nt_stores ? 0x20000000u : 0u);
+#ifdef LARS_LAB_LAYOUT
+    P.out_tile_stride = a->npix * (tuning().out_stride_planes > 1 ? tuning().out_stride_planes : 1);
+#endif
 }
 
 extern "C" int lars_d_fused(const lars_fused_args *a)
@@ -720,18 +765,7 @@
     hipStream_t s = pick_stream(c, a->stream);
 
     FusedParams P;
-    P.tiles = a->tiles; P.npix = a->npix; P.channels = a->channels; P.wb_table = a->wb_table;
-    for (int k = 0; k < 3; ++k) {
-        const bool on = (mask >> k) & 1u;
-        P.out_index[k] = on ? a->out_index[k] : nullptr;
-        P.out_rgba[k] = on ? a->out_rgba[k] : nullptr;
-        P.cmap_lut[k] = a->cmap_lut[k];
-    }
-    P.out_wb = a->out_wb; P.stats = a->stats; P.mask = mask; P.sel_hist = nullptr; P.sel_win = nullptr; P.sel_win_hist = nullptr; P.sel_below = nullptr;
-    P.flags = (a->flags & 7u) | (tuning().nt_stores ? 0x20000000u : 0u);
-#ifdef LARS_LAB_LAYOUT
-    P.out_tile_stride = a->npix * (tuning().out_stride_planes > 1 ? tuning().out_stride_planes : 1);
-#endif
+    fused_params(a, mask, P);
 
     const long long nrec = a->ntiles * 3;
     const bool raw = (a->flags & LARS_F_RAW) != 0;
@@ -785,6 +819,61 @@
     return launch_check("lars_d_fused");
 }
 
+namespace lars {
+void wb_exact_gated_launch(const uint8_t *tiles, long long ntiles, long long npix, unsigned int *hist, uint8_t *table, double *pcts,
+                           int rgn_variant, const unsigned int *pred, unsigned int gate_mask, int blocks, hipStream_t s)
+{
+    long long want = tuning().blocks_per_tile > 0 ? tuning().blocks_per_tile : blocks;
+    const long long cap = (npix / 4 + 1023) / 1024;
+    if (want > cap) want = cap;
+    if (want < 1) want = 1;
+    chan_hist_v2_launch(tiles, npix, hist, dim3((unsigned)want, (unsigned)ntiles), s, 3, pred, gate_mask);
+    hipLaunchKernelGGL((k_wb_table<256>), dim3(3, (unsigned)ntiles), dim3(256), 0, s, hist, npix, table, pcts, rgn_variant, pred, gate_mask);
+}
+}
+
+template <int CHECK>
+static void launch_checked(dim3 grid, hipStream_t s, const FusedParams &P)
+{
+    if (stream_loads_nt(true)) hipLaunchKernelGGL((k_fused_u8c3<uint8_t, 7u, true, 1, 3, CHECK, LOAD_NT>), grid, dim3(256), 0, s, P);
+    else hipLaunchKernelGGL((k_fused_u8c3<uint8_t, 7u, true, 1, 3, CHECK, LOAD_PLAIN>), grid, dim3(256), 0, s, P);
+}
+
+extern "C" int lars_d_fused_checked(const lars_fused_args *a, uint32_t *pred, uint32_t *hist, double *percentiles, int rgn_variant)
+{
+    ThreadCtx *c;
+    LARS_TRY(ensure_ctx(&c));
+    if (!a || !pred || !hist || !percentiles || !a->tiles || a->ntiles <= 0 || a->ntiles > 65535 || a->npix <= 0)
+        return fail(LARS_ERR_INVALID, "lars_d_fused_checked: bad arguments");
+    const bool planes = a->out_index[0] && a->out_index[1] && a->out_index[2];
+    bool aligned = (reinterpret_cast<uintptr_t>(a->tiles) & 3) == 0 && (!a->out_wb || (reinterpret_cast<uintptr_t>(a->out_wb) & 3) == 0);
+    for (int k = 0; k < 3; ++k) {
+        aligned = aligned && (reinterpret_cast<uintptr_t>(a->out_index[k]) & 15) == 0 && (reinterpret_cast<uintptr_t>(a->out_rgba[k]) & 15) == 0;
+        if (a->out_rgba[k] && !a->cmap_lut[k]) return fail(LARS_ERR_INVALID, "lars_d_fused_checked: out_rgba needs cmap_lut");
+    }
+    if (a->dtype != LARS_U8 || a->channels != 3 || a->index_mask != LARS_MASK_ALL || !a->wb_table || !a->stats || !planes ||
+        (a->flags & (LARS_F_STATS | LARS_F_HIST | LARS_F_SUMSQ)) != LARS_F_STATS || !aligned || (a->ntiles > 1 && (a->npix & 3)) ||
+        (long long)a->npix * 3 >= (1ll << 30))
+        return fail(LARS_ERR_INVALID, "lars_d_fused_checked: serves uint8 RGNir tiles (4-byte aligned, under 2^30 bytes each), all three index "
+                                      "planes, basic statistics");
+    hipStream_t s = pick_stream(c, a->stream);
+    FusedParams P;
+    fused_params(a, LARS_MASK_ALL, P);
+    P.pred = pred;
+    const long long nrec = a->ntiles * 3;
+    const bool raw = (a->flags & LARS_F_RAW) != 0;
+    if (!raw) stats_init_launch(a->stats, nrec, LARS_MASK_ALL, s);
+    const dim3 grid(blocks_per_tile(a->npix / 4 + 1, a->ntiles, 256, 32768), (unsigned)a->ntiles);
+    launch_checked<1>(grid, s, P);
+    wb_check_launch(pred, a->ntiles, a->npix, a->stats, s);
+    wb_exact_gated_launch(static_cast<const uint8_t *>(a->tiles), a->ntiles, a->npix, hist, const_cast<uint8_t *>(a->wb_table), percentiles,
+                          rgn_variant, pred, 1u << LARS_PRED_REPAIRED, 16, s);
+    launch_checked<2>(grid, s, P);
+    tuning().last_fused_kernel = 1;
+    if (!raw) stats_finalize_launch(a->stats, nrec, LARS_MASK_ALL, (long long)a->npix, s);
+    return launch_check("lars_d_fused_checked");
+}
+
 extern "C" int lars_d_stats_begin(lars_stats *stats, int64_t ntiles, uint32_t index_mask, void *stream)
 {
     ThreadCtx *c;
diff --git a/lars_image_processing_amd/csrc/fused_v2.hip b/lars_image_processing_amd/csrc/fused_v2.hip
--- a/lars_image_processing_amd/csrc/fused_v2.hip
+++ b/lars_image_processing_amd/csrc/fused_v2.hip
@@ -27,8 +27,10 @@
 
 template <int CH, int POLICY = LOAD_PLAIN>
 __global__ __launch_bounds__(1024) void k_chan_hist_u8c3_v2(const uint8_t *__restrict__ tiles, long long npix,
-                                                            unsigned int *__restrict__ hist)
-{
+                                                            unsigned int *__restrict__ hist, const unsigned int *__restrict__ gate,
+                                                            unsigned int gate_mask)
+{
+    if (!pred_gate(gate, blockIdx.y, gate_mask)) return;
     __shared__ unsigned int s_h[3 * 256 * 32];
     const int tid = threadIdx.x;
     for (int i = tid; i < 3 * 256 * 32; i += 1024) s_h[i] = 0;
@@ -515,13 +517,14 @@
     });
 }
 
-void chan_hist_v2_launch(const uint8_t *tiles, long long npix, unsigned int *hist, dim3 grid, hipStream_t s, int channels)
+void chan_hist_v2_launch(const uint8_t *tiles, long long npix, unsigned int *hist, dim3 grid, hipStream_t s, int channels,
+                         const unsigned int *gate, unsigned int gate_mask)
 {
     const bool nt = stream_loads_nt(true);
-    if (channels == 4 && nt) hipLaunchKernelGGL((k_chan_hist_u8c3_v2<4, LOAD_NT>), grid, dim3(1024), 0, s, tiles, npix, hist);
-    else if (channels == 4) hipLaunchKernelGGL((k_chan_hist_u8c3_v2<4, LOAD_PLAIN>), grid, dim3(1024), 0, s, tiles, npix, hist);
-    else if (nt) hipLaunchKernelGGL((k_chan_hist_u8c3_v2<3, LOAD_NT>), grid, dim3(1024), 0, s, tiles, npix, hist);
-    else hipLaunchKernelGGL((k_chan_hist_u8c3_v2<3, LOAD_PLAIN>), grid, dim3(1024), 0, s, tiles, npix, hist);
+    if (channels == 4 && nt) hipLaunchKernelGGL((k_chan_hist_u8c3_v2<4, LOAD_NT>), grid, dim3(1024), 0, s, tiles, npix, hist, gate, gate_mask);
+    else if (channels == 4) hipLaunchKernelGGL((k_chan_hist_u8c3_v2<4, LOAD_PLAIN>), grid, dim3(1024), 0, s, tiles, npix, hist, gate, gate_mask);
+    else if (nt) hipLaunchKernelGGL((k_chan_hist_u8c3_v2<3, LOAD_NT>), grid, dim3(1024), 0, s, tiles, npix, hist, gate, gate_mask);
+    else hipLaunchKernelGGL((k_chan_hist_u8c3_v2<3, LOAD_PLAIN>), grid, dim3(1024), 0, s, tiles, npix, hist, gate, gate_mask);
 }
 
 int quot_check_launch(unsigned int max_den, unsigned long long *mismatches_dev, unsigned int *first_bad_dev, hipStream_t s)
diff --git a/lars_image_processing_amd/csrc/runtime.cpp b/lars_image_processing_amd/csrc/runtime.cpp
--- a/lars_image_processing_amd/csrc/runtime.cpp
+++ b/lars_image_processing_amd/csrc/runtime.cpp
@@ -118,6 +118,7 @@
     {"jpeg_subseq_bits", &Tuning::jpeg_subseq_bits, Knob::SET, [](int v) { return v >= 32 && v <= 65536; }, "32 .. 65536"},
     {"tiff_strip_bytes", &Tuning::tiff_strip_bytes, Knob::SET, [](int v) { return v >= 1 && v <= (1 << 30); }, "1 .. 1073741824"},
     {"deflate_matching", &Tuning::deflate_matching, Knob::SET, [](int v) { return v == 0 || v == 1; }, "0 or 1"},
+    {"wb_predict", &Tuning::wb_predict, Knob::SET, [](int v) { return v >= 0 && v <= 3; }, "0 .. 3"},
     {"zone_split_pixels", &Tuning::zone_split_pixels, Knob::SET, [](int v) { return v >= 64 && v <= (1 << 30); }, "64 .. 1073741824"},
     {"last_fused_kernel", &Tuning::last_fused_kernel, Knob::READ_ONLY, nullptr, nullptr},
     {"jpeg_last_rounds", &Tuning::jpeg_last_rounds, Knob::READ_ONLY, nullptr, nullptr},
diff --git a/lars_image_processing_amd/csrc/wb_predict.hip b/lars_image_processing_amd/csrc/wb_predict.hip
--- /dev/null
+++ b/lars_image_processing_amd/csrc/wb_predict.hip
@@ -0,0 +1,196 @@
+#include <vector>
+
+#include "common.h"
+#include "device_common.h"
+#include "wg_device.h"
+
+namespace lars {
+
+__host__ __device__ inline unsigned int wb_sample_hash(unsigned int s)
+{
+    unsigned int x = s * 0x9E3779B9u + 0x7F4A7C15u;
+    x ^= x >> 16; x *= 0x7FEB352Du; x ^= x >> 15; x *= 0x846CA68Bu; x ^= x >> 16;
+    return x;
+}
+__host__ __device__ inline long long wb_sample_strata(long long npix, int frac_log2) { return (npix >> 8) >> frac_log2; }
+
+__global__ __launch_bounds__(256) void k_wb_sample(const uint8_t *__restrict__ tiles, long long npix, int frac_log2,
+                                                   unsigned int *__restrict__ hist)
+{
+    __shared__ unsigned int s_h[4][3 * 256];
+    const int tid = threadIdx.x, wave = tid >> 6, lane = tid & 63;
+    for (int i = tid; i < 4 * 768; i += 256) (&s_h[0][0])[i] = 0;
+    __syncthreads();
+
+    const long long tile = blockIdx.y;
+    const uint8_t *base = tiles + tile * npix * 3;
+    const long long nstrata = wb_sample_strata(npix, frac_log2);
+    const unsigned int fmask = (1u << frac_log2) - 1u;
+    unsigned int *h = s_h[wave];
+    const long long stride = (long long)gridDim.x * 4;
+    for (long long s0 = (long long)blockIdx.x * 4 + wave; s0 < nstrata; s0 += 4 * stride) {
+        unsigned int w[4][3];
+#pragma unroll
+        for (int j = 0; j < 4; ++j) {
+            const long long s = s0 + j * stride;
+            if (s < nstrata) {
+                const long long seg = (s << frac_log2) + (wb_sample_hash((unsigned int)s) & fmask);
+                const unsigned int *p = reinterpret_cast<const unsigned int *>(base + (seg * 64 + lane) * 12);
+                w[j][0] = p[0]; w[j][1] = p[1]; w[j][2] = p[2];
+            }
+        }
+#pragma unroll
+        for (int j = 0; j < 4; ++j) {
+            if (s0 + j * stride < nstrata) {
+                const unsigned int w0 = w[j][0], w1 = w[j][1], w2 = w[j][2];
+                atomicAdd(&h[0 * 256 + (w0 & 0xFF)], 1u);
+                atomicAdd(&h[1 * 256 + ((w0 >> 8) & 0xFF)], 1u);
+                atomicAdd(&h[2 * 256 + ((w0 >> 16) & 0xFF)], 1u);
+                atomicAdd(&h[0 * 256 + (w0 >> 24)], 1u);
+                atomicAdd(&h[1 * 256 + (w1 & 0xFF)], 1u);
+                atomicAdd(&h[2 * 256 + ((w1 >> 8) & 0xFF)], 1u);
+                atomicAdd(&h[0 * 256 + ((w1 >> 16) & 0xFF)], 1u);
+                atomicAdd(&h[1 * 256 + (w1 >> 24)], 1u);
+                atomicAdd(&h[2 * 256 + (w2 & 0xFF)], 1u);
+                atomicAdd(&h[0 * 256 + ((w2 >> 8) & 0xFF)], 1u);
+                atomicAdd(&h[1 * 256 + ((w2 >> 16) & 0xFF)], 1u);
+                atomicAdd(&h[2 * 256 + (w2 >> 24)], 1u);
+            }
+        }
+    }
+    __syncthreads();
+    unsigned int *gh = hist + tile * 768;
+    for (int i = tid; i < 768; i += 256) {
+        const unsigned int v = s_h[0][i] + s_h[1][i] + s_h[2][i] + s_h[3][i];
+        if (v) atomicAdd(&gh[i], v);
+    }
+}
+
+__global__ __launch_bounds__(256) void k_wb_predict(const unsigned int *__restrict__ shist, long long npix, long long m, double ksigma,
+                                                    int mode, long long floor_pix, int rgn_variant, unsigned int *__restrict__ pred,
+                                                    uint8_t *__restrict__ table, double *__restrict__ pcts)
+{
+    __shared__ unsigned long long s_scan[4];
+    __shared__ unsigned int s_mark[6];
+    __shared__ unsigned int s_state;
+    const int tid = threadIdx.x;
+    const long long tile = blockIdx.x;
+    if (tid < 6) s_mark[tid] = 0xFFFFFFFFu;
+    __syncthreads();
+    for (int c = 0; c < 3; ++c) {
+        const unsigned long long cnt = shist[(tile * 3 + c) * 256 + tid];
+        const unsigned long long before = wg_exscan<256>(cnt, s_scan);
+        for (int k = 0; k < 2 && m > 0; ++k) {
+            long long lo, hi;
+            double t;
+            wb_mark_ranks(m, k, lo, hi, t);
+            if ((unsigned long long)lo >= before && (unsigned long long)hi < before + cnt) {
+                const double q = (k == 0 ? 2.0 : 98.0) / 100.0;
+                const double centre = q * (double)m;
+                const double need = ksigma * sqrt(q * (1.0 - q) * (double)m);
+                if (centre - (double)before >= need && (double)(before + cnt) - centre >= need) s_mark[c * 2 + k] = (unsigned)tid;
+            }
+        }
+    }
+    __syncthreads();
+    if (tid == 0) {
+        bool ok = mode != 0 && (mode >= 2 || npix >= floor_pix);
+        for (int i = 0; i < 6; ++i) ok = ok && s_mark[i] != 0xFFFFFFFFu;
+        for (int c = 0; c < 3; ++c) ok = ok && s_mark[2 * c] != s_mark[2 * c + 1];
+        if (ok && mode == 3)
+            for (int i = 0; i < 6; ++i) s_mark[i] = s_mark[i] < 255u ? s_mark[i] + 1u : 254u;
+        s_state = ok ? LARS_PRED_PREDICTED : LARS_PRED_EXACT;
+    }
+    __syncthreads();
+    const bool predicted = s_state == LARS_PRED_PREDICTED;
+    unsigned int *rec = pred + tile * LARS_PRED_WORDS;
+    if (tid < LARS_PRED_WORDS)
+        rec[tid] = tid == 0 ? s_state : (predicted && tid >= LARS_PRED_MARKS && tid < LARS_PRED_MARKS + 6) ? s_mark[tid - LARS_PRED_MARKS] : 0u;
+    if (!predicted) return;
+    if (tid < 6) pcts[tile * 6 + tid] = (double)s_mark[tid];
+    for (int c = 0; c < 3; ++c)
+        wb_table_row_u8(table + (tile * 3 + c) * 256, tid, (double)s_mark[2 * c], (double)s_mark[2 * c + 1], rgn_variant);
+}
+
+__global__ __launch_bounds__(64) void k_wb_check(unsigned int *__restrict__ pred, long long npix, lars_stats *__restrict__ stats)
+{
+    const long long tile = blockIdx.x;
+    unsigned int *rec = pred + tile * LARS_PRED_WORDS;
+    if (rec[0] != LARS_PRED_PREDICTED) return;
+    const int tid = threadIdx.x;
+    bool ok = true;
+    if (tid < 6) {
+        const int c = tid >> 1, k = tid & 1;
+        long long lo, hi;
+        double t;
+        wb_mark_ranks(npix, k, lo, hi, t);
+        const long long below = rec[LARS_PRED_COUNTS + 4 * c + 2 * k], upto = rec[LARS_PRED_COUNTS + 4 * c + 2 * k + 1];
+        ok = below <= lo && upto > hi;
+    }
+    const bool all_ok = __all(ok);
+    if (tid == 0) rec[0] = all_ok ? LARS_PRED_CONFIRMED : LARS_PRED_REPAIRED;
+    if (!all_ok && tid < 3) stats_rec_init(reinterpret_cast<StatsAccView *>(stats + tile * 3 + tid), tid);
+}
+
+void wb_check_launch(unsigned int *pred, long long ntiles, long long npix, lars_stats *stats, hipStream_t s)
+{
+    hipLaunchKernelGGL(k_wb_check, dim3((unsigned)ntiles), dim3(64), 0, s, pred, npix, stats);
+}
+
+}
+
+using namespace lars;
+
+extern "C" size_t lars_wb_predict_bytes(int64_t ntiles)
+{
+    return ntiles > 0 ? (size_t)ntiles * LARS_PRED_WORDS * sizeof(uint32_t) : 0;
+}
+
+extern "C" int64_t lars_wb_predict_floor_pixels(void) { return LARS_WB_PREDICT_FLOOR_PIXELS; }
+
+extern "C" int64_t lars_wb_predict_sample_segment(int64_t npix, int frac_log2, int64_t s)
+{
+    if (npix <= 0 || frac_log2 < 0 || frac_log2 > 16 || s < 0 || s >= wb_sample_strata(npix, frac_log2)) return -1;
+    return (s << frac_log2) + (wb_sample_hash((unsigned int)s) & ((1u << frac_log2) - 1u));
+}
+
+extern "C" int lars_d_wb_predict(const void *tiles, int64_t ntiles, int64_t npix, int frac_log2, double ksigma, int rgn_variant,
+                                 uint32_t *sample_hist, uint32_t *pred, uint32_t *hist, uint8_t *table, double *percentiles, void *stream)
+{
+    ThreadCtx *c;
+    LARS_TRY(ensure_ctx(&c));
+    if (!tiles || !sample_hist || !pred || !hist || !table || !percentiles || ntiles <= 0 || ntiles > 65535 || npix <= 0 ||
+        frac_log2 < 0 || frac_log2 > 16 || !(ksigma >= 0.0))
+        return fail(LARS_ERR_INVALID, "lars_d_wb_predict: bad arguments");
+    if ((reinterpret_cast<uintptr_t>(tiles) & 3) || (ntiles > 1 && (npix & 3)) || (long long)npix * 3 >= (1ll << 30))
+        return fail(LARS_ERR_INVALID, "lars_d_wb_predict: serves uint8 RGNir tiles, 4-byte aligned, under 2^30 bytes each");
+    hipStream_t s = pick_stream(c, stream);
+    const int mode = tuning().wb_predict;
+    const long long nstrata = wb_sample_strata(npix, frac_log2);
+    LARS_HIP_TRY(hipMemsetAsync(sample_hist, 0, (size_t)ntiles * 768 * sizeof(uint32_t), s));
+    LARS_HIP_TRY(hipMemsetAsync(hist, 0, (size_t)ntiles * 768 * sizeof(uint32_t), s));
+    if (nstrata > 0 && mode != 0) {
+        long long want = (2048 + ntiles - 1) / ntiles;
+        const long long cap = (nstrata + 3) / 4;
+        if (want > cap) want = cap;
+        hipLaunchKernelGGL(k_wb_sample, dim3((unsigned)want, (unsigned)ntiles), dim3(256), 0, s, static_cast<const uint8_t *>(tiles),
+                           (long long)npix, frac_log2, sample_hist);
+    }
+    hipLaunchKernelGGL(k_wb_predict, dim3((unsigned)ntiles), dim3(256), 0, s, sample_hist, (long long)npix, nstrata * 256, ksigma, mode,
+                       (long long)LARS_WB_PREDICT_FLOOR_PIXELS, rgn_variant, pred, table, percentiles);
+    wb_exact_gated_launch(static_cast<const uint8_t *>(tiles), ntiles, npix, hist, table, percentiles, rgn_variant, pred,
+                          1u << LARS_PRED_EXACT, 64, s);
+    return launch_check("lars_d_wb_predict");
+}
+
+extern "C" int lars_wb_predict_report(const uint32_t *pred, int64_t ntiles, uint32_t *states, uint32_t *marks)
+{
+    if (!pred || ntiles <= 0 || !states || !marks) return fail(LARS_ERR_INVALID, "lars_wb_predict_report: bad arguments");
+    std::vector<uint32_t> w((size_t)ntiles * LARS_PRED_WORDS);
+    LARS_HIP_TRY(hipMemcpy(w.data(), pred, w.size() * sizeof(uint32_t), hipMemcpyDeviceToHost));
+    for (int64_t t = 0; t < ntiles; ++t) {
+        states[t] = w[t * LARS_PRED_WORDS];
+        for (int i = 0; i < 6; ++i) marks[t * 6 + i] = w[t * LARS_PRED_WORDS + LARS_PRED_MARKS + i];
+    }
+    return LARS_OK;
+}
```

Measured after the change: 375,300 (median of 6 runs). 4.0% higher.
